# DrorT/demucs

Measured on AMD Instinct MI355X. Metric: real-time factor (audio-sec/wall-sec) htdemucs 4-stem 44.1kHz stereo, 1/8 GPU, higher is better.
Workload: dtype f32

## Files before the change

### demucs_amd/_lib.py

```python
from __future__ import annotations

import ctypes as C
import os
import threading

_HERE = os.path.dirname(os.path.abspath(__file__))
LIB_PATH = os.environ.get("DEMUCS_AMD_LIB") or os.path.join(_HERE, "libdemucs_amd.so")

MI_OK = 0


class MiTensorDesc(C.Structure):
    _fields_ = [("name", C.c_char_p), ("data", C.c_void_p), ("numel", C.c_int64)]


class MiConfig(C.Structure):
    _fields_ = [("n_sources", C.c_int32), ("segment_length", C.c_int32), ("max_batch", C.c_int32),
                ("dtype", C.c_int32)]


class MiProfileRow(C.Structure):
    _fields_ = [("name", C.c_char * 48), ("launches", C.c_int64), ("ms", C.c_double), ("flops", C.c_double),
                ("bytes", C.c_double)]


class MiConvDesc(C.Structure):
    _fields_ = [
        ("wt", C.c_void_p), ("M", C.c_int32), ("Mpad", C.c_int32), ("K", C.c_int32), ("Kpad", C.c_int32),
        ("ktab", C.c_void_p),
        ("x", C.c_void_p), ("x_bstride", C.c_int64),
        ("B", C.c_int32), ("D1", C.c_int32), ("D2", C.c_int32), ("O1", C.c_int32), ("O2", C.c_int32),
        ("S1", C.c_int32), ("S2", C.c_int32),
        ("pro", C.c_int32), ("pro_stats", C.c_void_p), ("pro_w", C.c_void_p), ("pro_b", C.c_void_p),
        ("row_mode", C.c_int32),
        ("epi", C.c_int32), ("flags", C.c_int32),
        ("bias", C.c_void_p), ("scale", C.c_void_p), ("res", C.c_void_p), ("emb", C.c_void_p),
        ("y", C.c_void_p), ("y_bstride", C.c_int64), ("y_cstride", C.c_int64),
        ("stats", C.c_void_p), ("gn_stats", C.c_void_p), ("gn_w", C.c_void_p), ("gn_b", C.c_void_p),
        ("out_len", C.c_int32), ("tile_m", C.c_int32), ("plain", C.c_int32), ("half", C.c_int32),
        ("o2_valid", C.c_int32), ("ktab_len", C.c_int32), ("sink", C.c_void_p), ("wx", C.c_void_p), ("tr_stride", C.c_int32), ("tr_pad", C.c_int32), ("x_ld", C.c_int32), ("x_ld_pad", C.c_int32), ("wh", C.c_void_p),
        ("xh", C.c_void_p), ("xh_n", C.c_int64), ("yh", C.c_void_p), ("yh_n", C.c_int64),
        ("wtap", C.c_void_p), ("ntaps", C.c_int32), ("tap_k2", C.c_int32), ("tap_pad1", C.c_int32), ("tap_pad2", C.c_int32),
        ("tap_dil1", C.c_int32), ("tap_dil2", C.c_int32), ("yh_pq", C.c_int64),
        ("dma_rows", C.c_int32), ("dma_rows_pad", C.c_int32),
        ("dma_time", C.c_int32), ("dma_time_pad", C.c_int32),
    ]


SIGNATURES = {
    "mi_model_create": (C.c_int, [C.POINTER(MiConfig), C.POINTER(MiTensorDesc), C.c_size_t, C.POINTER(C.c_void_p)]),
    "mi_model_destroy": (None, [C.c_void_p]),
    "mi_model_forward": (C.c_int, [C.c_void_p, C.c_void_p, C.c_void_p, C.c_int32, C.c_void_p]),
    "mi_model_forward_core": (C.c_int, [C.c_void_p, C.c_void_p, C.c_void_p, C.c_void_p, C.c_void_p, C.c_int32, C.c_void_p]),
    "mi_model_tap": (C.c_int, [C.c_void_p, C.c_char_p, C.c_void_p, C.c_int32, C.POINTER(C.c_int64), C.c_void_p]),
    "mi_hmodel_create": (C.c_int, [C.POINTER(MiConfig), C.POINTER(MiTensorDesc), C.c_size_t, C.POINTER(C.c_void_p)]),
    "mi_hmodel_destroy": (None, [C.c_void_p]),
    "mi_hmodel_forward": (C.c_int, [C.c_void_p, C.c_void_p, C.c_void_p, C.c_int32, C.c_int32, C.c_void_p]),
    "mi_hmodel_tap": (C.c_int, [C.c_void_p, C.c_char_p, C.c_void_p, C.c_int32, C.POINTER(C.c_int64), C.c_void_p]),
    "mi_hmodel_device_bytes": (C.c_int64, [C.c_void_p]),
    "mi_hmodel_status": (C.c_int, [C.c_void_p, C.c_void_p]),
    "mi_set_two_streams": (C.c_int, [C.c_int32]),
    "mi_set_split_bf16": (C.c_int, [C.c_int32]),
    "mi_set_istft_fused": (C.c_int, [C.c_int32]),
    "mi_set_transpose_tiles": (C.c_int, [C.c_int32]),
    "mi_profile_begin": (C.c_int, [C.c_void_p]),
    "mi_profile_end": (C.c_int, [C.c_void_p, C.POINTER(MiProfileRow), C.c_int32, C.POINTER(C.c_int32), C.c_void_p]),
    "mi_model_device_bytes": (C.c_int64, [C.c_void_p]),
    "mi_segments_gather": (C.c_int, [C.c_void_p, C.c_int64, C.c_int32, C.c_void_p, C.c_int32, C.c_int32, C.c_void_p,
                                     C.c_int64, C.c_void_p]),
    "mi_ola_accumulate": (C.c_int, [C.c_void_p, C.c_int64, C.c_int32, C.c_void_p, C.c_int32, C.c_int64, C.c_void_p, C.c_void_p,
                                    C.c_void_p, C.c_int32, C.c_int64, C.c_int64, C.c_void_p, C.c_int32, C.c_void_p]),
    "mi_ola_finish": (C.c_int, [C.c_void_p, C.c_int64, C.c_int32, C.c_int64, C.c_void_p, C.c_void_p, C.c_int32,
                                C.c_int32, C.c_void_p, C.c_void_p]),
    "mi_segments_gather_packed": (C.c_int, [C.c_void_p, C.c_int64, C.c_int32, C.c_void_p, C.c_int32, C.c_int32, C.c_void_p,
                                            C.c_int64, C.c_void_p]),
    "mi_ola_accumulate_packed": (C.c_int, [C.c_void_p, C.c_int64, C.c_int32, C.c_void_p, C.c_int32, C.c_int64, C.c_void_p, C.c_int32,
                                           C.c_void_p, C.c_int32, C.c_void_p, C.c_int64, C.c_void_p]),
    "mi_ola_finish_packed": (C.c_int, [C.c_void_p, C.c_int64, C.c_int32, C.c_void_p, C.c_int32, C.c_void_p, C.c_int32, C.c_void_p,
                                       C.c_int64, C.c_void_p]),
    "mi_stream_emit": (C.c_int, [C.c_void_p, C.c_int64, C.c_int32, C.c_int32, C.c_void_p, C.c_int32, C.c_void_p, C.c_int32,
                                 C.c_void_p, C.c_int64, C.c_void_p, C.c_int32, C.c_int32, C.c_int32, C.c_void_p, C.c_int64,
                                 C.c_void_p, C.c_int64, C.c_void_p]),
    "mi_streams_emit": (C.c_int, [C.c_void_p, C.c_int64, C.c_int32, C.c_int32, C.c_void_p, C.c_int32, C.c_int64, C.c_void_p,
                                  C.c_int32, C.c_void_p, C.c_int32, C.c_void_p, C.c_int64, C.c_void_p, C.c_int32, C.c_int32,
                                  C.c_int32, C.c_void_p, C.c_int32, C.c_void_p, C.c_int64, C.c_void_p]),
    "mi_streams_append": (C.c_int, [C.c_void_p, C.c_int64, C.c_int32, C.c_void_p, C.c_int32, C.c_int64, C.c_void_p, C.c_int32,
                                    C.c_void_p]),
    "mi_streams_convert_append": (C.c_int, [C.c_void_p, C.c_int64, C.c_int32, C.c_void_p, C.c_int32, C.c_int64, C.c_void_p, C.c_int64,
                                            C.c_void_p, C.c_int64, C.c_void_p, C.c_int32, C.c_int32, C.c_void_p]),
    "mi_pcm_planar": (C.c_int, [C.c_void_p, C.c_int32, C.c_int32, C.c_int64, C.c_int32, C.c_void_p, C.c_void_p, C.c_void_p]),
    "mi_streams_append_pcm": (C.c_int, [C.c_void_p, C.c_int64, C.c_int32, C.c_void_p, C.c_int32, C.c_int64, C.c_void_p, C.c_int32,
                                        C.c_void_p]),
    "mi_streams_convert_append_pcm": (C.c_int, [C.c_void_p, C.c_int64, C.c_int32, C.c_void_p, C.c_int32, C.c_int64, C.c_void_p,
                                                C.c_int64, C.c_void_p, C.c_int64, C.c_void_p, C.c_int32, C.c_int32, C.c_void_p]),
    "mi_streams_compact": (C.c_int, [C.c_void_p, C.c_int64, C.c_void_p, C.c_int64, C.c_void_p, C.c_int32, C.c_int64, C.c_void_p]),
    "mi_mono_stats_scratch_bytes": (C.c_int32, []),
    "mi_mono_stats": (C.c_int, [C.c_void_p, C.c_int32, C.c_int64, C.c_void_p, C.c_void_p, C.c_void_p]),
    "mi_mono_stats_state_bytes": (C.c_int32, []),
    "mi_mono_stats_update": (C.c_int, [C.c_void_p, C.c_int32, C.c_int32, C.c_int64, C.c_int32, C.c_int64, C.c_void_p, C.c_void_p]),
    "mi_mono_stats_finish": (C.c_int, [C.c_void_p, C.c_int64, C.c_void_p, C.c_void_p, C.c_void_p]),
    "mi_sdr_state_bytes": (C.c_int64, [C.c_int32]),
    "mi_sdr_scratch_bytes": (C.c_int64, [C.c_int32]),
    "mi_sdr_update": (C.c_int, [C.c_void_p, C.c_int32, C.c_int32, C.c_int64, C.c_void_p, C.c_int64, C.c_int32, C.c_int32, C.c_int64,
                                C.c_int64, C.c_void_p, C.c_void_p]),
    "mi_sdr_finish": (C.c_int, [C.c_void_p, C.c_int32, C.c_void_p, C.c_void_p, C.c_void_p]),
    "mi_sdr": (C.c_int, [C.c_void_p, C.c_void_p, C.c_int32, C.c_int32, C.c_int32, C.c_int64, C.c_void_p, C.c_void_p, C.c_void_p,
                         C.c_void_p]),
    "mi_track_affine": (C.c_int, [C.c_void_p, C.c_int64, C.c_void_p, C.c_int32, C.c_void_p]),
    "mi_prevent_clip": (C.c_int, [C.c_void_p, C.c_int64, C.c_int32, C.c_void_p, C.c_void_p, C.c_void_p]),
    "mi_two_stems": (C.c_int, [C.c_void_p, C.c_int32, C.c_int32, C.c_void_p, C.c_int32, C.c_int64, C.c_void_p, C.c_void_p]),
    "mi_deliver_peaks": (C.c_int, [C.c_void_p, C.c_int32, C.c_int64, C.c_int32, C.c_int32, C.c_void_p, C.c_int32, C.c_int64, C.c_void_p]),
    "mi_deliver_pcm": (C.c_int, [C.c_void_p, C.c_int32, C.c_int64, C.c_int32, C.c_int32, C.c_void_p, C.c_int32, C.c_void_p, C.c_int64,
                                 C.c_void_p]),
    "mi_deliver_resample_pcm": (C.c_int, [C.c_void_p, C.c_int32, C.c_int64, C.c_int32, C.c_int32, C.c_void_p, C.c_int64, C.c_void_p,
                                          C.c_int64, C.c_int32, C.c_void_p, C.c_int64, C.c_void_p]),
    "mi_deliver_peaks_update": (C.c_int, [C.c_void_p, C.c_int32, C.c_int64, C.c_int32, C.c_int32, C.c_void_p, C.c_int32, C.c_void_p]),
    "mi_deliver_mix_pcm": (C.c_int, [C.c_void_p, C.c_int32, C.c_int64, C.c_int32, C.c_int32, C.c_void_p, C.c_int32, C.c_void_p, C.c_int64,
                                     C.c_void_p]),
    "mi_deliver_mix_peaks": (C.c_int, [C.c_void_p, C.c_int32, C.c_int64, C.c_int32, C.c_int32, C.c_void_p, C.c_int32, C.c_int64,
                                       C.c_void_p]),
    "mi_deliver_mix_peaks_update": (C.c_int, [C.c_void_p, C.c_int32, C.c_int64, C.c_int32, C.c_int32, C.c_void_p, C.c_int32, C.c_void_p]),
    "mi_deliver_mix_auto_pcm": (C.c_int, [C.c_void_p, C.c_int64, C.c_int32, C.c_int64, C.c_int32, C.c_int32, C.c_void_p, C.c_int32,
                                          C.c_void_p, C.c_int64, C.c_void_p]),
    "mi_deliver_mix_auto_peaks": (C.c_int, [C.c_void_p, C.c_int64, C.c_int32, C.c_int64, C.c_int32, C.c_int32, C.c_void_p, C.c_int32,
                                            C.c_int64, C.c_void_p]),
    "mi_loudness_update": (C.c_int, [C.c_void_p, C.c_int32, C.c_int64, C.c_int64, C.c_int32, C.c_int32, C.POINTER(C.c_double), C.c_int64,
                                     C.c_int64, C.c_void_p, C.c_int64, C.c_void_p, C.c_int64, C.c_void_p, C.c_int64, C.c_void_p]),
    "mi_deliver_resample_peaks": (C.c_int, [C.c_void_p, C.c_int32, C.c_int64, C.c_int32, C.c_int32, C.c_void_p, C.c_int64, C.c_void_p,
                                            C.c_int64, C.c_int32, C.c_void_p, C.c_void_p, C.c_int32, C.c_void_p]),
    "mi_deliver_resample_pcm_peaks": (C.c_int, [C.c_void_p, C.c_int32, C.c_int64, C.c_int32, C.c_int32, C.c_void_p, C.c_int64,
                                                C.c_void_p, C.c_int64, C.c_int32, C.c_void_p, C.c_int64, C.c_void_p, C.c_void_p,
                                                C.c_int32, C.c_void_p]),
    "mi_stft_cac": (C.c_int, [C.c_void_p, C.c_int32, C.c_int32, C.c_void_p, C.c_void_p]),
    "mi_istft_cac": (C.c_int, [C.c_void_p, C.c_int32, C.c_int32, C.c_int32, C.c_void_p, C.c_void_p]),
    "mi_stft_norm": (C.c_int, [C.c_void_p, C.c_int32, C.c_int32, C.c_void_p, C.c_int32, C.c_void_p, C.c_void_p, C.c_void_p]),
    "mi_istft_full": (C.c_int, [C.c_void_p, C.c_int32, C.c_int32, C.c_int32, C.c_int32, C.c_void_p, C.c_void_p, C.c_int32, C.c_void_p,
                                C.c_void_p, C.c_void_p]),
    "mi_item_norm": (C.c_int, [C.c_void_p, C.c_int32, C.c_int64, C.c_void_p, C.c_void_p, C.c_void_p, C.c_void_p]),
    "mi_item_denorm": (C.c_int, [C.c_void_p, C.c_int32, C.c_int64, C.c_void_p, C.c_void_p, C.c_void_p]),
    "mi_conv_forward": (C.c_int, [C.POINTER(MiConvDesc), C.c_void_p]),
    "mi_resample_frac": (C.c_int, [C.c_void_p, C.c_int32, C.c_int64, C.c_void_p, C.c_int32, C.c_int32, C.c_int32, C.c_void_p, C.c_int64,
                                   C.c_void_p]),
    "mi_conv_pack_split": (C.c_int, [C.c_void_p, C.c_int32, C.c_int32, C.c_int32, C.c_void_p, C.c_void_p]),
    "mi_conv_pack_half": (C.c_int, [C.c_void_p, C.c_int32, C.c_int32, C.c_int32, C.c_void_p, C.c_void_p]),
    "mi_f32_to_image": (C.c_int, [C.c_void_p, C.c_int32, C.c_int32, C.c_int64, C.c_int32, C.c_void_p, C.c_void_p]),
    "mi_conv_pack_tap": (C.c_int, [C.c_void_p, C.c_int32, C.c_int32, C.c_int32, C.c_int32, C.c_void_p, C.c_void_p]),
    "mi_attention": (C.c_int, [C.c_void_p, C.c_void_p, C.c_void_p, C.c_void_p, C.c_int32, C.c_int32, C.c_int32,
                               C.c_int32, C.c_int64, C.c_int64, C.c_int64, C.c_int32, C.c_void_p]),
    "mi_attention_split": (C.c_int, [C.c_void_p, C.c_void_p, C.c_void_p, C.c_void_p, C.c_int32, C.c_int32, C.c_int32,
                                     C.c_int32, C.c_int64, C.c_int64, C.c_int64, C.c_void_p]),
    "mi_attention_heads": (C.c_int, [C.c_void_p, C.c_void_p, C.c_void_p, C.c_void_p, C.c_int32, C.c_int32, C.c_int32, C.c_int32,
                                     C.c_int32, C.c_int32, C.c_int32, C.c_void_p]),
    "mi_attention_heads_image": (C.c_int, [C.c_void_p, C.c_void_p, C.c_void_p, C.c_void_p, C.c_int64, C.c_int32, C.c_int32, C.c_int32,
                                           C.c_int32, C.c_int32, C.c_int32, C.c_int32, C.c_void_p]),
    "mi_attention_image": (C.c_int, [C.c_void_p, C.c_void_p, C.c_void_p, C.c_void_p, C.c_int64, C.c_int32, C.c_int32, C.c_int32,
                                     C.c_int32, C.c_int64, C.c_int64, C.c_int32, C.c_void_p]),
    "mi_lstm_seq": (C.c_int, [C.c_void_p, C.c_void_p, C.c_int32, C.c_int32, C.c_int32, C.c_void_p, C.c_int32, C.c_void_p]),
    "mi_gn_gelu": (C.c_int, [C.c_void_p, C.c_int32, C.c_int32, C.c_int32, C.c_int32, C.c_int32, C.c_int32, C.c_void_p, C.c_void_p,
                             C.c_void_p, C.c_void_p]),
    "mi_gram_order": (C.c_int32, [C.c_int32]),
    "mi_gn_gelu_gram": (C.c_int, [C.c_void_p, C.c_int32, C.c_int32, C.c_int32, C.c_int32, C.c_int32, C.c_int32, C.c_int32, C.c_void_p,
                                  C.c_void_p, C.c_void_p, C.c_void_p, C.c_int32, C.c_void_p]),
    "mi_dconv_gn_gelu_gram": (C.c_int, [C.c_void_p, C.c_int32, C.c_int32, C.c_int32, C.c_int32, C.c_int32, C.c_int32, C.c_int32,
                                        C.c_void_p, C.c_void_p, C.c_void_p, C.c_void_p, C.c_int32, C.c_void_p]),
    "mi_gram_finalize": (C.c_int, [C.c_void_p, C.c_int32, C.c_int32, C.c_int32, C.c_void_p, C.c_void_p, C.c_double, C.c_double,
                                   C.c_double, C.c_double, C.c_float, C.c_void_p, C.c_void_p]),
    "mi_layernorm_cf": (C.c_int, [C.c_void_p, C.c_int32, C.c_int32, C.c_int32, C.c_void_p, C.c_void_p, C.c_void_p,
                                  C.c_void_p, C.c_void_p]),
    "mi_token_norm": (C.c_int, [C.c_int32, C.c_void_p, C.c_int32, C.c_int32, C.c_int32, C.c_void_p, C.c_void_p, C.c_void_p, C.c_void_p,
                                C.c_void_p, C.c_void_p, C.c_void_p, C.c_int64, C.c_int32, C.c_void_p]),
    "mi_local_attn": (C.c_int, [C.c_void_p, C.c_int32, C.c_int32, C.c_int32, C.c_int32, C.c_void_p, C.c_int32, C.c_void_p]),
    "mi_group_norm_apply": (C.c_int, [C.c_void_p, C.c_int32, C.c_int32, C.c_int32, C.c_int32, C.c_int32, C.c_int32, C.c_void_p,
                                      C.c_void_p, C.c_int32, C.c_int32, C.c_void_p, C.c_void_p, C.c_int32, C.c_void_p, C.c_int32,
                                      C.c_int32, C.c_int32, C.c_int32, C.c_void_p, C.c_void_p, C.c_void_p]),
    "mi_blstm_unfold": (C.c_int, [C.c_void_p, C.c_int32, C.c_int32, C.c_int32, C.c_int32, C.c_int32, C.c_int32, C.c_void_p, C.c_void_p]),
    "mi_blstm_restitch": (C.c_int, [C.c_void_p, C.c_int32, C.c_int32, C.c_int32, C.c_int32, C.c_int32, C.c_int32, C.c_void_p,
                                    C.c_void_p, C.c_void_p]),
    "mi_row_affine_pitch": (C.c_int, [C.c_void_p, C.c_int32, C.c_int32, C.c_int32, C.c_int32, C.c_void_p, C.c_void_p, C.c_void_p]),
    "mi_dconv_row": (C.c_int, [C.c_void_p, C.c_void_p, C.c_int32, C.c_int32, C.c_int32, C.c_int32, C.c_void_p, C.c_int32, C.c_void_p]),
    "mi_dconv_time_layer": (C.c_int, [C.c_void_p, C.c_void_p, C.c_int32, C.c_int32, C.c_int32, C.c_int32, C.c_int32, C.c_void_p,
                                      C.c_void_p, C.c_void_p, C.c_void_p, C.c_void_p, C.c_void_p]),
    "mi_debug_set_post_launch_hook": (None, [C.c_void_p]),
    "mi_debug_last_conv_route": (C.c_int, []),
    "mi_debug_last_conv_tile": (C.c_int, []),
    "mi_debug_conv_staged": (C.c_int, []),
    "mi_debug_conv_route_launches": (C.c_int64, [C.c_int32, C.c_int32]),
    "mi_debug_conv_route": (C.c_int, [C.POINTER(MiConvDesc), C.POINTER(C.c_int)]),
    "mi_debug_switches": (C.c_int, [C.c_char_p, C.c_int32]),
    "mi_last_error": (C.c_char_p, []),
    "mi_version": (C.c_char_p, []),
}

_lib = None
_lock = threading.Lock()


class EngineError(RuntimeError):
    """A libdemucs_amd call returned a non-zero status (the reference convention for this path
# ... 30 lines not shown
```

### demucs_amd/csrc/api.hip

```cpp
#include <new>

#include "hmodel.h"
#include "model.h"

namespace mi {

post_launch_hook_t g_post_launch_hook = nullptr;
int g_last_conv_route = -1;
long long g_conv_route_launches[16][8] = {};
int g_last_conv_tile = -1;

char *last_error_buf() {
    static thread_local char buf[1024] = "";
    return buf;
}

int set_error(int code, const char *fmt, ...) {
    va_list ap;
    va_start(ap, fmt);
    vsnprintf(last_error_buf(), 1024, fmt, ap);
    va_end(ap);
    return code;
}

struct Tables {
    FftTables t{};
    bool ready = false;
};
static int get_tables(FftTables *out) {
    static Tables tb;
    if (!tb.ready) {
        const FftHostTables h = fft_host_tables();
        float *dw, *de; float2 *dt;
        MI_HIP(hipMalloc((void **)&dw, 4096 * 4)); MI_HIP(hipMalloc((void **)&dt, h.twiddle.size() * 8)); MI_HIP(hipMalloc((void **)&de, 1024 * 4));
        MI_HIP(hipMemcpy(dw, h.window.data(), 4096 * 4, hipMemcpyHostToDevice));
        MI_HIP(hipMemcpy(dt, h.twiddle.data(), h.twiddle.size() * 8, hipMemcpyHostToDevice));
        MI_HIP(hipMemcpy(de, h.envelope.data(), 1024 * 4, hipMemcpyHostToDevice));
        tb.t = FftTables{dw, dt, de};
        tb.ready = true;
    }
    *out = tb.t;
    return MI_OK;
}

static size_t dconv_layer_floats(int C) { const size_t h = C / 8; return h * C * 3 + 3 * h + 2 * C * h + 6 * (size_t)C + C; }
struct DConvTestLayer {
    std::vector<void *> bufs;
    DConvTimeLayer l{};
    ~DConvTestLayer() { for (void *p : bufs) (void)hipFree(p); }
    template <typename T> int up(const T *h, size_t n, const T **out) {
        void *p = nullptr;
        MI_HIP(hipMalloc(&p, n * sizeof(T)));
        bufs.push_back(p);
        MI_HIP(hipMemcpy(p, h, n * sizeof(T), hipMemcpyHostToDevice));
        *out = (const T *)p;
        return MI_OK;
    }
    int init(int C, const float *w) {
        const int h = C / 8;
        const float *w0 = w, *b0 = w0 + (size_t)h * C * 3, *g1w = b0 + h, *g1b = g1w + h, *w3 = g1b + h, *b3 = w3 + (size_t)2 * C * h,
                    *g2w = b3 + 2 * C, *g2b = g2w + 2 * C, *ls = g2b + 2 * C;
        const DConvHostPack p = dconv_pack_host(C, h, w0, b0, g1w, g1b, w3, b3);
        MI_TRY(up(p.w0.data(), p.w0.size(), &l.w.w0)); MI_TRY(up(p.b0.data(), p.b0.size(), &l.w.b0));
        MI_TRY(up(p.g1w.data(), p.g1w.size(), &l.w.g1w)); MI_TRY(up(p.g1b.data(), p.g1b.size(), &l.w.g1b));
        MI_TRY(up(p.w3.data(), p.w3.size(), &l.w.w3));
        MI_TRY(up(b3, (size_t)2 * C, &l.w.b3)); MI_TRY(up(g2w, (size_t)2 * C, &l.w.g2w)); MI_TRY(up(g2b, (size_t)2 * C, &l.w.g2b));
        MI_TRY(up(ls, (size_t)C, &l.w.ls));
        MI_TRY(up(p.gram_a.data(), p.gram_a.size(), &l.gram_a)); MI_TRY(up(p.gram_v.data(), p.gram_v.size(), &l.gram_v));
        MI_TRY(up(p.gram_c.data(), p.gram_c.size(), &l.gram_c)); MI_TRY(up(p.gram_e1.data(), p.gram_e1.size(), &l.gram_e1));
        MI_TRY(up(p.gram_e2.data(), p.gram_e2.size(), &l.gram_e2));
        l.sum_b3 = p.sum_b3; l.sum_b3sq = p.sum_b3sq;
        return MI_OK;
    }
};

struct TestScratch {
    std::vector<void *> bufs;
    ~TestScratch() { for (void *p : bufs) (void)hipFree(p); }
    template <typename T> int get(size_t n, T **out) {
        void *p = nullptr;
        MI_HIP(hipMalloc(&p, std::max<size_t>(n, 1) * sizeof(T)));
        bufs.push_back(p);
        *out = (T *)p;
        return MI_OK;
    }
};
static int finish_entry(int r, hipStream_t st, const char *who) {
    const hipError_t e = hipStreamSynchronize(st);
    if (e != hipSuccess && r == MI_OK) r = set_error(MI_EHIP, "%s: hipStreamSynchronize: %s", who, hipGetErrorString(e));
    return r;
}

static int stft_entry(const char *who, const float *mix_dev, int B, int L, float *x_dev, int x_pitch, float *norm_dev, float *denorm_dev,
                      hipStream_t st) {
    FftTables tb;
    MI_TRY(get_tables(&tb));
    const int T = (L + 1023) / 1024;
    TestScratch ws;
    float *zt = nullptr; double *stats = nullptr;
    MI_TRY(ws.get((size_t)B * T * 4 * 2048, &zt));
    MI_TRY(ws.get((size_t)2 * kStatSlots * B, &stats));
    MI_HIP(hipMemsetAsync(stats, 0, sizeof(double) * 2 * kStatSlots * B, st));
    int r = launch_stft_frames(mix_dev, B, L, tb, zt, stats, st);
    if (r == MI_OK && norm_dev) r = launch_finalize_stats(stats, B, 4.0 * 2048 * T, 1e-5f, 1, (float2 *)norm_dev, (float2 *)denorm_dev, st);
    if (r == MI_OK) r = launch_cac_transpose(zt, B, T, (const float2 *)norm_dev, x_dev, st, x_pitch);
    return finish_entry(r, st, who);
}

static const char *const kKindNames[2] = {"htdemucs", "hdemucs"};
template <typename Engine>
static Engine *engine_of(void *handle, EngineKind want, const char *entry) {
    EngineCore *core = static_cast<EngineCore *>(handle);
    if (core->kind != want) {
        set_error(MI_EINVAL, "%s: the handle belongs to the %s engine, this entry takes one of the %s engine", entry, kKindNames[core->kind], kKindNames[want]);
        return nullptr;
    }
    return static_cast<Engine *>(core);
}
constexpr size_t kConvSlack = 128;
int g_conv_staged = 0;
static bool conv_reads_slack(int route) { return route == MI_ROUTE_DMATAP || route == MI_ROUTE_TAP_X6 || route == MI_ROUTE_TIME_X6; }
static bool conv_owns_slack(const float *x, size_t bytes) {
    hipDeviceptr_t base = nullptr;
    size_t size = 0;
    if (hipMemGetAddressRange(&base, &size, (hipDeviceptr_t)x) != hipSuccess) {
        (void)hipGetLastError();
        return false;
    }
    const uintptr_t lo = (uintptr_t)base, hi = lo + size, p = (uintptr_t)x;
    return p >= lo + kConvSlack && p + bytes + kConvSlack <= hi;
}
static int conv_forward_staged(const mi_conv_desc &din, size_t bytes, hipStream_t st) {
    TestScratch ws;
    unsigned char *buf = nullptr;
    MI_TRY(ws.get(bytes + 2 * kConvSlack, &buf));
    MI_HIP(hipMemsetAsync(buf, 0, bytes + 2 * kConvSlack, st));
    MI_HIP(hipMemcpyAsync(buf + kConvSlack, din.x, bytes, hipMemcpyDeviceToDevice, st));
    mi_conv_desc d = din;
    d.x = reinterpret_cast<const float *>(buf + kConvSlack);
    ++g_conv_staged;
    return finish_entry(launch_conv(d, st), st, "mi_conv_forward");
}

static Model *as_model(void *handle, const char *entry) { return engine_of<Model>(handle, ENGINE_HTDEMUCS, entry); }
static HModel *as_hmodel(void *handle, const char *entry) { return engine_of<HModel>(handle, ENGINE_HDEMUCS, entry); }

}

using namespace mi;

extern "C" {

const char *mi_last_error(void) { return last_error_buf(); }
void mi_debug_set_post_launch_hook(void (*hook)(void *stream)) { g_post_launch_hook = hook; }
int mi_debug_last_conv_route(void) { return g_last_conv_route; }
int mi_debug_last_conv_tile(void) { return g_last_conv_tile; }
int mi_debug_conv_staged(void) { return g_conv_staged; }
int64_t mi_debug_conv_route_launches(int32_t route, int32_t epi) {
    if (route < 0 || route >= 16 || epi >= 8) return -1;
    int64_t n = 0;
    for (int e = 0; e < 8; ++e)
        if (epi < 0 || e == epi) n += mi::g_conv_route_launches[route][e];
    return n;
}
int mi_debug_conv_route(const struct mi_conv_desc *desc, int *tile) {
    if (!desc) return -1;
    if (conv_check_tile_m(*desc) != MI_OK) return -1;
    const ConvRoute r = conv_route(*desc);
    if (tile) *tile = r.tile;
    return r.route;
}
const char *mi_version(void) { return "demucs_amd 0.1 gfx950"; }

int mi_model_create(const mi_config *cfg, const mi_tensor_desc *weights, size_t n_weights, void **handle) {
    if (!cfg || !weights || !handle) return set_error(MI_EINVAL, "mi_model_create: null argument");
    *handle = nullptr;
    Model *m = new (std::nothrow) Model();
    if (!m) return set_error(MI_ENOMEM, "mi_model_create: host allocation failed");
    const int r = m->init(*cfg, weights, n_weights);
    if (r != MI_OK) { delete m; return r; }
    *handle = static_cast<EngineCore *>(m);
    return MI_OK;
}

void mi_model_destroy(void *handle) {
    if (!handle) return;
    Model *m = as_model(handle, "mi_model_destroy");
    if (!m) return;
    (void)hipDeviceSynchronize();
    delete m;
}

int mi_model_forward(void *handle, const float *mix_dev, float *out_dev, int32_t B, void *stream) {
    if (!handle) return set_error(MI_EINVAL, "mi_model_forward: null handle");
    Model *m = as_model(handle, "mi_model_forward");
    return m ? m->forward(mix_dev, out_dev, B, (hipStream_t)stream) : MI_EINVAL;
}

int mi_model_tap(void *handle, const char *name, float *dst_dev, int32_t B, int64_t *numel_per_item, void *stream) {
    if (!handle || !name || !numel_per_item) return set_error(MI_EINVAL, "mi_model_tap: null argument");
    Model *m = as_model(handle, "mi_model_tap");
    if (!m) return MI_EINVAL;
    const float *src = nullptr;
    const float **ptr_dev = &src;
    const std::string n(name);
    const int64_t T = m->T, Tf = 8 * T, Tt = m->Lt[4];
    static const int ch[4] = {48, 96, 192, 384}, fr[4] = {512, 128, 32, 8};
    *ptr_dev = nullptr;
    if (n == "x0") { *ptr_dev = m->w_x0; *numel_per_item = 4 * 2048 * T; }
    else if (n == "xt0") { *ptr_dev = m->w_xt0; *numel_per_item = 2 * (int64_t)m->SL; }
    else if (n == "yspec") { *ptr_dev = m->w_yspec; *numel_per_item = 4 * (int64_t)m->S * 2048 * T; }
    else if (n == "ytime") { *ptr_dev = m->w_ytime; *numel_per_item = 2 * (int64_t)m->S * m->SL; }
    else if (n == "tr_f") { *ptr_dev = m->w_tr_x[0][1]; *numel_per_item = 512 * Tf; }
    else if (n == "tr_t") { *ptr_dev = m->w_tr_x[1][1]; *numel_per_item = 512 * Tt; }
    else if (n.size() == 4 && n.compare(0, 3, "enc") == 0 && n[3] >= '0' && n[3] <= '3') {
        const int i = n[3] - '0'; *ptr_dev = m->w_skip[i]; *numel_per_item = (int64_t)ch[i] * fr[i] * T;
    } else if (n.size() == 5 && n.compare(0, 4, "tenc") == 0 && n[4] >= '0' && n[4] <= '3') {
        const int i = n[4] - '0'; *ptr_dev = m->w_skip_t[i]; *numel_per_item = (int64_t)ch[i] * m->Lp[i + 1];
    }
    if (!*ptr_dev) return set_error(MI_EINVAL, "mi_model_tap: unknown tap '%s'", name);
    if (dst_dev) {
        MI_REQUIRE(B >= 1 && B <= m->cfg.max_batch, "mi_model_tap: batch %d out of range", B);
        MI_HIP(hipMemcpyAsync(dst_dev, src, sizeof(float) * (size_t)B * *numel_per_item, hipMemcpyDeviceToDevice, (hipStream_t)stream));
    }
    return MI_OK;
}

int mi_model_forward_core(void *handle, const float *mix_dev, const float *mag_dev, float *spec_out_dev, float *time_out_dev,
                          int32_t B, void *stream) {
    if (!handle) return set_error(MI_EINVAL, "mi_model_forward_core: null handle");
    Model *m = as_model(handle, "mi_model_forward_core");
    return m ? m->forward_core(mix_dev, mag_dev, spec_out_dev, time_out_dev, B, (hipStream_t)stream) : MI_EINVAL;
}

int mi_hmodel_create(const mi_config *cfg, const mi_tensor_desc *weights, size_t n_weights, void **handle) {
    if (!cfg || !weights || !handle) return set_error(MI_EINVAL, "mi_hmodel_create: null argument");
    *handle = nullptr;
    HModel *m = new (std::nothrow) HModel();
    if (!m) return set_error(MI_ENOMEM, "mi_hmodel_create: host allocation failed");
    const int r = m->hinit(*cfg, weights, n_weights);
    if (r != MI_OK) { delete m; return r; }
    *handle = static_cast<EngineCore *>(m);
    return MI_OK;
}

void mi_hmodel_destroy(void *handle) {
    if (!handle) return;
    HModel *m = as_hmodel(handle, "mi_hmodel_destroy");
    if (!m) return;
    (void)hipDeviceSynchronize();
    delete m;
}

int mi_hmodel_forward(void *handle, const float *mix_dev, float *out_dev, int32_t B, int32_t length, void *stream) {
    if (!handle) return set_error(MI_EINVAL, "mi_hmodel_forward: null handle");
    HModel *m = as_hmodel(handle, "mi_hmodel_forward");
    return m ? m->hforward(mix_dev, out_dev, B, length, (hipStream_t)stream) : MI_EINVAL;
}

int mi_hmodel_tap(void *handle, const char *name, float *dst_dev, int32_t B, int64_t *numel_per_item, void *stream) {
    if (!handle || !name || !numel_per_item) return set_error(MI_EINVAL, "mi_hmodel_tap: null argument");
    HModel *m = as_hmodel(handle, "mi_hmodel_tap");
    if (!m) return MI_EINVAL;
    auto it = m->taps.find(name);
    if (it == m->taps.end()) return set_error(MI_EINVAL, "mi_hmodel_tap: unknown tap '%s'", name);
    *numel_per_item = it->second.second;
    if (dst_dev) {
        MI_REQUIRE(B >= 1 && B <= m->cfg.max_batch, "mi_hmodel_tap: batch %d out of range", B);
        MI_HIP(hipMemcpyAsync(dst_dev, it->second.first, sizeof(float) * (size_t)B * it->second.second, hipMemcpyDeviceToDevice, (hipStream_t)stream));
    }
    return MI_OK;
}

int mi_hmodel_status(void *handle, void *stream) {
// ... 355 lines not shown
int mi_deliver_resample_pcm_peaks(const int64_t *table_dev, int32_t n_rows, int64_t max_groups, int32_t n_sources, int32_t channels,
                                  const float *bank_dev, int64_t bank_capacity, float *hist_dev, int64_t hist_capacity, int32_t lds_floats,
                                  void *dst_dev, int64_t dst_capacity, const int32_t *slots_dev, const void *peaks_dev, int32_t n_peaks,
                                  void *stream) {
    MI_REQUIRE(table_dev && dst_dev && n_rows > 0 && n_rows <= 65535 && max_groups >= 1 && max_groups <= INT32_MAX && n_sources > 0 &&
               channels > 0 && bank_capacity >= 0 && (bank_capacity == 0 || bank_dev) && hist_capacity >= 0 &&
               (hist_capacity == 0 || hist_dev) && lds_floats >= 1 && lds_floats <= MI_RATE_LDS_FLOATS && dst_capacity >= 0 &&
               slots_dev && n_peaks >= 0 && (n_peaks == 0 || peaks_dev), "mi_deliver_resample_pcm_peaks: bad argument");
    MI_REQUIRE(((uintptr_t)dst_dev & 3) == 0, "mi_deliver_resample_pcm_peaks: dst_dev must be 4-byte aligned");
    return launch_deliver_resample_pcm_peaks(table_dev, n_rows, max_groups, n_sources, channels, bank_dev, bank_capacity, hist_dev,
                                             hist_capacity, lds_floats, (unsigned char *)dst_dev, dst_capacity, slots_dev,
                                             (const unsigned *)peaks_dev, n_peaks, (hipStream_t)stream);
}

int mi_deliver_mix_pcm(const int64_t *table_dev, int32_t n_rows, int64_t max_n, int32_t n_sources, int32_t channels,
                       const void *peaks_dev, int32_t n_peaks, void *dst_dev, int64_t dst_capacity, void *stream) {
    MI_REQUIRE(table_dev && dst_dev && n_rows > 0 && n_rows <= 65535 && max_n >= 1 && max_n <= (int64_t)INT32_MAX * 1024 &&
               n_sources > 0 && n_sources <= MI_MIX_MAX_SOURCES && channels > 0 && n_peaks >= 0 && (n_peaks == 0 || peaks_dev) &&
               dst_capacity >= 0, "mi_deliver_mix_pcm: bad argument");
    MI_REQUIRE(((uintptr_t)dst_dev & 3) == 0, "mi_deliver_mix_pcm: dst_dev must be 4-byte aligned");
    return launch_deliver_mix_pcm(table_dev, n_rows, max_n, n_sources, channels, (const unsigned *)peaks_dev, n_peaks,
                                  (unsigned char *)dst_dev, dst_capacity, (hipStream_t)stream);
}

int mi_deliver_mix_peaks(const int64_t *table_dev, int32_t n_rows, int64_t max_n, int32_t n_sources, int32_t channels, void *peaks_dev,
                         int32_t n_peaks, int64_t dst_capacity, void *stream) {
    MI_REQUIRE(table_dev && peaks_dev && n_rows > 0 && n_rows <= 65535 && max_n >= 1 && max_n <= (int64_t)INT32_MAX * 1024 &&
               n_sources > 0 && n_sources <= MI_MIX_MAX_SOURCES && channels > 0 && n_peaks > 0 && dst_capacity >= 0,
               "mi_deliver_mix_peaks: bad argument");
    return launch_deliver_mix_peaks(table_dev, n_rows, max_n, n_sources, channels, (unsigned *)peaks_dev, n_peaks, dst_capacity,
                                    (hipStream_t)stream);
}

int mi_deliver_mix_peaks_update(const int64_t *table_dev, int32_t n_rows, int64_t max_n, int32_t n_sources, int32_t channels,
                                void *peaks_dev, int32_t n_peaks, void *stream) {
    MI_REQUIRE(table_dev && peaks_dev && n_rows > 0 && n_rows <= 65535 && max_n >= 1 && max_n <= (int64_t)INT32_MAX * 1024 &&
               n_sources > 0 && n_sources <= MI_MIX_MAX_SOURCES && channels > 0 && n_peaks > 0, "mi_deliver_mix_peaks_update: bad argument");
    return launch_deliver_mix_peaks_update(table_dev, n_rows, max_n, n_sources, channels, (unsigned *)peaks_dev, n_peaks,
                                           (hipStream_t)stream);
}

int mi_deliver_mix_auto_pcm(const int64_t *table_dev, int64_t table_len, int32_t n_rows, int64_t max_n, int32_t n_sources,
                            int32_t channels, const void *peaks_dev, int32_t n_peaks, void *dst_dev, int64_t dst_capacity, void *stream) {
    MI_REQUIRE(table_dev && dst_dev && n_rows > 0 && n_rows <= 65535 && table_len <= INT32_MAX &&
               table_len >= (int64_t)n_rows * MI_AUTO_COLS && max_n >= 1 && max_n <= (int64_t)INT32_MAX * 1024 && n_sources > 0 &&
               n_sources <= MI_MIX_MAX_SOURCES && channels > 0 && n_peaks >= 0 && (n_peaks == 0 || peaks_dev) && dst_capacity >= 0,
               "mi_deliver_mix_auto_pcm: bad argument");
    MI_REQUIRE(((uintptr_t)dst_dev & 3) == 0, "mi_deliver_mix_auto_pcm: dst_dev must be 4-byte aligned");
    return launch_deliver_mix_auto_pcm(table_dev, table_len, n_rows, max_n, n_sources, channels, (const unsigned *)peaks_dev, n_peaks,
                                       (unsigned char *)dst_dev, dst_capacity, (hipStream_t)stream);
}

int mi_deliver_mix_auto_peaks(const int64_t *table_dev, int64_t table_len, int32_t n_rows, int64_t max_n, int32_t n_sources,
                              int32_t channels, void *peaks_dev, int32_t n_peaks, int64_t dst_capacity, void *stream) {
    MI_REQUIRE(table_dev && peaks_dev && n_rows > 0 && n_rows <= 65535 && table_len <= INT32_MAX &&
               table_len >= (int64_t)n_rows * MI_AUTO_COLS && max_n >= 1 && max_n <= (int64_t)INT32_MAX * 1024 && n_sources > 0 &&
               n_sources <= MI_MIX_MAX_SOURCES && channels > 0 && n_peaks > 0 && dst_capacity >= 0,
               "mi_deliver_mix_auto_peaks: bad argument");
    return launch_deliver_mix_auto_peaks(table_dev, table_len, n_rows, max_n, n_sources, channels, (unsigned *)peaks_dev, n_peaks,
                                         dst_capacity, (hipStream_t)stream);
}

int mi_loudness_update(const int64_t *table_dev, int32_t n_rows, int64_t max_n, int64_t max_blocks, int32_t n_sources, int32_t channels,
                       const double *coef, int64_t hop, int64_t warm, float *hist_dev, int64_t hist_capacity, double *energies_dev,
                       int64_t energies_capacity, float *work_dev, int64_t work_capacity, void *stream) {
    MI_REQUIRE(table_dev && coef && energies_dev && work_dev && n_rows > 0 && n_rows <= 65535 && max_n >= 1 &&
               max_n <= (int64_t)INT32_MAX * 256 && max_blocks >= 0 && max_blocks <= (int64_t)INT32_MAX * 64 && n_sources > 0 &&
               n_sources <= MI_MIX_MAX_SOURCES && channels > 0 && channels <= 65535 && hist_capacity >= 0 &&
               (hist_dev || hist_capacity == 0) && energies_capacity >= 0 && work_capacity >= 0,
               "mi_loudness_update: bad argument");
    if (hop < 1 || warm < 0) return MI_OK;
    return launch_loudness_update(table_dev, n_rows, max_n, max_blocks, n_sources, channels, coef, hop, warm, hist_dev, hist_capacity,
                                  energies_dev, energies_capacity, work_dev, work_capacity, (hipStream_t)stream);
}

int mi_stft_cac(const float *mix_dev, int32_t B, int32_t L, float *cac_dev, void *stream) {
    MI_REQUIRE(mix_dev && cac_dev && B > 0 && B <= 16383 && L >= 1, "mi_stft_cac: bad argument");
    return stft_entry("mi_stft_cac", mix_dev, B, L, cac_dev, 0, nullptr, nullptr, (hipStream_t)stream);
}

int mi_stft_norm(const float *mix_dev, int32_t B, int32_t L, float *x_dev, int32_t x_pitch, float *norm_dev, float *denorm_dev, void *stream) {
    MI_REQUIRE(mix_dev && x_dev && norm_dev && denorm_dev, "mi_stft_norm: null argument");
    MI_REQUIRE(B >= 1 && B <= 16383, "mi_stft_norm: B = %d outside [1, 16383] (the transpose's grid holds 4 B planes)", B);
    MI_REQUIRE(L >= 1, "mi_stft_norm: L = %d, at least one sample", L);
    const int T = (L + 1023) / 1024;
    MI_REQUIRE(x_pitch == 0 || x_pitch >= T, "mi_stft_norm: row pitch %d below T = %d", x_pitch, T);
    return stft_entry("mi_stft_norm", mix_dev, B, L, x_dev, x_pitch, norm_dev, denorm_dev, (hipStream_t)stream);
}

int mi_istft_full(const float *y_dev, int32_t B, int32_t S, int32_t L, int32_t y_pitch, const float *denorm_f_dev, const float *xt_dev,
                  int32_t xt_pitch, const float *denorm_t_dev, float *wav_dev, void *stream) {
    MI_REQUIRE(y_dev && wav_dev, "mi_istft_full: null argument");
    MI_REQUIRE(B >= 1 && S >= 1 && (int64_t)B * S <= 16383, "mi_istft_full: B = %d, S = %d: 1 <= B S <= 16383 (the transpose's grid holds 4 B S planes)",
               B, S);
    MI_REQUIRE(L >= 1, "mi_istft_full: L = %d, at least one sample", L);
    const int T = (L + 1023) / 1024;
    MI_REQUIRE(y_pitch == 0 || y_pitch >= T, "mi_istft_full: spectrogram row pitch %d below T = %d", y_pitch, T);
    MI_REQUIRE((xt_dev != nullptr) == (denorm_t_dev != nullptr), "mi_istft_full: xt_dev and denorm_t_dev go together");
    MI_REQUIRE(xt_pitch == 0 || xt_pitch >= L, "mi_istft_full: time-branch row pitch %d below L = %d", xt_pitch, L);
    FftTables tb;
    MI_TRY(get_tables(&tb));
    TestScratch ws;
    float *yt = nullptr, *fr = nullptr;
    MI_TRY(ws.get((size_t)B * S * T * 4 * 2048, &yt));
    MI_TRY(ws.get((size_t)B * S * T * 2 * 4096, &fr));
    hipStream_t st = (hipStream_t)stream;
    const int r = launch_istft(y_dev, B, S, L, (const float2 *)denorm_f_dev, xt_dev, (const float2 *)denorm_t_dev, tb, yt, fr, wav_dev, st,
                               xt_pitch, y_pitch);
    return finish_entry(r, st, "mi_istft_full");
}

int mi_istft_cac(const float *x_dev, int32_t B, int32_t S, int32_t L, float *wav_dev, void *stream) {
    MI_REQUIRE(x_dev && wav_dev && B > 0 && S > 0 && (int64_t)B * S <= 16383 && L >= 1, "mi_istft_cac: bad argument");
    return mi_istft_full(x_dev, B, S, L, 0, nullptr, nullptr, 0, nullptr, wav_dev, stream);
}

int mi_item_norm(const float *x_dev, int32_t rows, int64_t count, float *y_dev, float *norm_dev, float *denorm_dev, void *stream) {
    MI_REQUIRE(x_dev && y_dev && norm_dev && denorm_dev, "mi_item_norm: null argument");
    MI_REQUIRE(rows >= 1 && rows <= 65535, "mi_item_norm: rows = %d outside [1, 65535] (the grid's y range)", rows);
    MI_REQUIRE(count >= 2, "mi_item_norm: count = %lld: the unbiased std divides by count - 1", (long long)count);
    TestScratch ws;
    double *stats = nullptr;
    MI_TRY(ws.get((size_t)2 * kStatSlots * rows, &stats));
    hipStream_t st = (hipStream_t)stream;
    MI_HIP(hipMemsetAsync(stats, 0, sizeof(double) * 2 * kStatSlots * rows, st));
    int r = launch_row_stats(x_dev, rows, count, count, stats, st);
    if (r == MI_OK) r = launch_finalize_stats(stats, rows, (double)count, 1e-5f, 1, (float2 *)norm_dev, (float2 *)denorm_dev, st);
    if (r == MI_OK) r = launch_row_affine(x_dev, rows, count, (const float2 *)norm_dev, y_dev, st);
    return finish_entry(r, st, "mi_item_norm");
}

int mi_item_denorm(const float *x_dev, int32_t rows, int64_t count, const float *denorm_dev, float *y_dev, void *stream) {
    MI_REQUIRE(x_dev && denorm_dev && y_dev, "mi_item_denorm: null argument");
    MI_REQUIRE(rows >= 1 && rows <= 65535 && count >= 1, "mi_item_denorm: rows = %d outside [1, 65535] or count = %lld < 1", rows, (long long)count);
    return launch_row_denorm(x_dev, rows, count, (const float2 *)denorm_dev, y_dev, (hipStream_t)stream);
}

int mi_conv_forward(const struct mi_conv_desc *desc, void *stream) {
    MI_REQUIRE(desc, "mi_conv_forward: null descriptor");
    if (desc->x && desc->B > 0 && desc->x_bstride > 0 && conv_check_tile_m(*desc) == MI_OK && conv_reads_slack(conv_route(*desc).route)) {
        const size_t bytes = (size_t)desc->B * (size_t)desc->x_bstride * sizeof(float);
        if (!conv_owns_slack(desc->x, bytes)) return conv_forward_staged(*desc, bytes, (hipStream_t)stream);
    }
    return launch_conv(*desc, (hipStream_t)stream);
}

int mi_resample_frac(const float *x_dev, int32_t rows, int64_t length, const float *table_dev, int32_t old_sr, int32_t new_sr,
                     int32_t width, float *y_dev, int64_t out_length, void *stream) {
    MI_REQUIRE(x_dev && table_dev && y_dev && old_sr > 0 && new_sr > 0 && width > 0, "mi_resample_frac: bad argument");
    return launch_resample_frac(x_dev, rows, length, table_dev, old_sr, new_sr, width, y_dev, out_length, (hipStream_t)stream);
}

int mi_conv_pack_split(const float *wt_dev, int32_t Kpad, int32_t Mpad, int32_t tile_m, void *wx_dev, void *stream) {
    MI_REQUIRE(wt_dev && wx_dev && Kpad > 0 && Mpad > 0 && (conv_x6_supported(tile_m) || tile_m == 192), "mi_conv_pack_split: bad argument");
    MI_REQUIRE(tile_m != 192 || Mpad % 192 == 0, "mi_conv_pack_split: tile_m 192 needs Mpad %% 192 == 0 (Mpad %d)", Mpad);
    return launch_pack_split(wt_dev, Kpad, Mpad, tile_m == 192 ? 96 : tile_m, wx_dev, (hipStream_t)stream);
}

int mi_conv_pack_tap(const float *wt_dev, int32_t Mpad, int32_t Cin, int32_t ntaps, int32_t dtype, void *wtap_dev, void *stream) {
    MI_REQUIRE(wt_dev && wtap_dev && Mpad > 0 && Cin > 0 && ntaps > 0, "mi_conv_pack_tap: bad argument");
    return launch_pack_tap(wt_dev, Mpad, Cin, ntaps, dtype, wtap_dev, (hipStream_t)stream);
}

int mi_f32_to_image(const float *x_dev, int32_t B, int32_t C, int64_t P, int32_t dtype, void *img_dev, void *stream) {
    MI_REQUIRE(x_dev && img_dev && B > 0 && C > 0 && P > 0, "mi_f32_to_image: bad argument");
    return launch_f32_to_image(x_dev, B, C, P, dtype, img_dev, (hipStream_t)stream);
}

int mi_conv_pack_half(const float *wt_dev, int32_t Kpad, int32_t Mpad, int32_t dtype, void *wh_dev, void *stream) {
    MI_REQUIRE(wt_dev && wh_dev && Kpad > 0 && Mpad > 0, "mi_conv_pack_half: bad argument");
    return launch_pack_half(wt_dev, Kpad, Mpad, dtype, wh_dev, (hipStream_t)stream);
}

int mi_attention(const float *q_dev, const float *k_dev, const float *v_dev, float *o_dev, int32_t B, int32_t heads, int32_t Tq,
                 int32_t Tk, int64_t q_batch_stride, int64_t kv_batch_stride, int64_t o_batch_stride, int32_t dtype, void *stream) {
    MI_REQUIRE(q_dev && k_dev && v_dev && o_dev && B > 0 && heads > 0 && Tq > 0 && Tk > 0, "mi_attention: bad argument");
    return launch_attention(q_dev, k_dev, v_dev, o_dev, B, heads, Tq, Tk, q_batch_stride, kv_batch_stride, o_batch_stride, dtype,
                            (hipStream_t)stream);
}

int mi_attention_split(const float *q_dev, const float *k_dev, const float *v_dev, float *o_dev, int32_t B, int32_t heads, int32_t Tq,
                       int32_t Tk, int64_t q_batch_stride, int64_t kv_batch_stride, int64_t o_batch_stride, void *stream) {
    MI_REQUIRE(q_dev && k_dev && v_dev && o_dev && B > 0 && heads > 0 && Tq > 0 && Tk > 0, "mi_attention_split: bad argument");
    return launch_attention_x6(q_dev, k_dev, v_dev, o_dev, B, heads, Tq, Tk, q_batch_stride, kv_batch_stride, o_batch_stride,
                               (hipStream_t)stream);
}

int mi_attention_heads(const void *q_dev, const void *k_dev, const void *v_dev, float *o_dev, int32_t B, int32_t heads, int32_t Tq, int32_t Tk,
                       int32_t Tq_pitch, int32_t Tk_pitch, int32_t dtype, void *stream) {
    MI_REQUIRE(q_dev && k_dev && v_dev && o_dev && B > 0 && heads > 0 && Tq > 0 && Tk > 0, "mi_attention_heads: bad argument");
    const void *zero = conv_zero_page();
    MI_REQUIRE(zero, "mi_attention_heads: could not allocate the zero page");
    return launch_attention_heads(q_dev, k_dev, v_dev, zero, B, heads, Tq, Tk, Tq_pitch, Tk_pitch, dtype, nullptr, 0, o_dev,
                                  (int64_t)heads * 64 * Tq, (hipStream_t)stream);
}

int mi_attention_heads_image(const void *q_dev, const void *k_dev, const void *v_dev, void *img_dev, int64_t n_img, int32_t B, int32_t heads,
                             int32_t Tq, int32_t Tk, int32_t Tq_pitch, int32_t Tk_pitch, int32_t dtype, void *stream) {
    MI_REQUIRE(q_dev && k_dev && v_dev && img_dev && B > 0 && heads > 0 && Tq > 0 && Tk > 0, "mi_attention_heads_image: bad argument");
    const void *zero = conv_zero_page();
    MI_REQUIRE(zero, "mi_attention_heads_image: could not allocate the zero page");
    return launch_attention_heads(q_dev, k_dev, v_dev, zero, B, heads, Tq, Tk, Tq_pitch, Tk_pitch, dtype, img_dev, n_img, nullptr, 0,
                                  (hipStream_t)stream);
}

int mi_attention_image(const float *q_dev, const float *k_dev, const float *v_dev, void *img_dev, int64_t n_img, int32_t B,
                       int32_t heads, int32_t Tq, int32_t Tk, int64_t q_batch_stride, int64_t kv_batch_stride, int32_t dtype,
                       void *stream) {
    MI_REQUIRE(q_dev && k_dev && v_dev && img_dev && B > 0 && heads > 0 && Tq > 0 && Tk > 0, "mi_attention_image: bad argument");
    MI_REQUIRE(dtype == MI_DTYPE_BF16 || dtype == MI_DTYPE_F16, "mi_attention_image: dtype %d is not a half mode", dtype);
    return launch_attention(q_dev, k_dev, v_dev, nullptr, B, heads, Tq, Tk, q_batch_stride, kv_batch_stride, 0, dtype,
                            (hipStream_t)stream, img_dev, n_img);
}

int mi_gn_gelu(float *x_dev, int32_t B, int32_t C, int32_t C_alloc, int32_t D1, int32_t D2, int32_t row_mode, const float *stats_dev,
               const float *w_dev, const float *b_dev, void *stream) {
    MI_REQUIRE(x_dev && stats_dev && w_dev && b_dev && B > 0 && C > 0 && D1 > 0 && D2 > 0, "mi_gn_gelu: bad argument");
    MI_REQUIRE(C_alloc >= C, "mi_gn_gelu: C_alloc < C");
    return launch_gn_gelu(x_dev, B, C, C_alloc, D1, D2, row_mode, (const float2 *)stats_dev, w_dev, b_dev, (hipStream_t)stream);
}

int32_t mi_gram_order(int32_t h) { return gram_hp(h); }

int mi_lstm_seq(const float *gx_dev, const float *whh_host, int32_t N, int32_t H, int32_t W, float *out_dev, int32_t mode, void *stream) {
    MI_REQUIRE(mode == 0 || mode == 1 || mode == 2, "mi_lstm_seq: mode 0 (one launch per step), 1 (persistent kernel) or 2 (generic small kernel)");
    hipStream_t st = (hipStream_t)stream;
    if (mode == 2) {
        MI_REQUIRE(gx_dev && whh_host && out_dev && N > 0 && N <= 65535 && W > 0 && H >= 1 && H <= 64,
                   "mi_lstm_seq: bad argument (mode 2 needs 1 <= H <= 64)");
        const size_t bytes = (size_t)2 * 4 * H * H * sizeof(float);
        float *wn = nullptr;
        MI_HIP(hipMalloc((void **)&wn, bytes));
        int rs = MI_OK;
        if (hipMemcpyAsync(wn, whh_host, bytes, hipMemcpyHostToDevice, st) != hipSuccess) rs = set_error(MI_EHIP, "mi_lstm_seq: hipMemcpyAsync failed");
        if (rs == MI_OK) rs = launch_lstm_small(gx_dev, wn, N, H, W, out_dev, st);
        const hipError_t es = hipStreamSynchronize(st);
        if (es != hipSuccess && rs == MI_OK) rs = set_error(MI_EHIP, "mi_lstm_seq: hipStreamSynchronize: %s", hipGetErrorString(es));
        (void)hipFree(wn);
        return rs;
    }
    MI_REQUIRE(gx_dev && whh_host && out_dev && N > 0 && W > 0 && (H == 192 || H == 384), "mi_lstm_seq: bad argument (H must be 192 or 384)");
    std::vector<float> packed((size_t)2 * 4 * H * H);
    pack_lstm_whh(whh_host, H, packed.data());
    float *wd = nullptr, *state = nullptr;
    void *scratch = nullptr;
    unsigned *flag = nullptr;
    int r = MI_OK;
    auto fail = [&](hipError_t e, const char *what) { if (e != hipSuccess && r == MI_OK) r = set_error(MI_EHIP, "mi_lstm_seq: %s: %s", what, hipGetErrorString(e)); };
    fail(hipMalloc((void **)&wd, packed.size() * sizeof(float)), "hipMalloc");
    fail(hipMalloc((void **)&state, (size_t)6 * N * H * sizeof(float)), "hipMalloc");
    fail(hipMalloc(&scratch, lstm_persist_scratch_bytes()), "hipMalloc");
    fail(hipHostMalloc((void **)&flag, 64, hipHostMallocMapped), "hipHostMalloc");
    if (r == MI_OK) {
        *flag = 0;
        fail(hipMemcpyAsync(wd, packed.data(), packed.size() * sizeof(float), hipMemcpyHostToDevice, st), "hipMemcpyAsync");
        if (r == MI_OK) r = mode ? launch_lstm_persist(gx_dev, wd, N, H, W, out_dev, scratch, flag, st) : launch_lstm_seq(gx_dev, wd, N, H, W, out_dev, state, st);
        fail(hipStreamSynchronize(st), "hipStreamSynchronize");
        if (r == MI_OK && *(volatile unsigned *)flag) r = set_error(MI_EHIP, "mi_lstm_seq: the persistent kernel timed out waiting for its hidden-state exchange");
        if (r == MI_OK && mode && switches().lstm_debug) {
                        unsigned dbg[16] = {};
            (void)hipMemcpy(dbg, (char *)scratch + lstm_persist_ctl_offset(), sizeof(dbg), hipMemcpyDeviceToHost);
            fprintf(stderr, "[lstm] H %d N %d W %d: block 0 / wave 1 spent %.1f us gathering h in %u poll passes (%.2f us, %.2f passes per step); "
                    "%s stores\n", H, N, W, dbg[2] * 0.01, dbg[3], dbg[2] * 0.01 / std::max(1, W - 1), (double)dbg[3] / std::max(1, W - 1),
                    dbg[4] ? "same-XCD plain" : "write-through");
            fprintf(stderr, "[lstm]   shader cycles per step: gather %.0f, issue + products %.0f, LDS write + barrier %.0f, gate stage %.0f; whole step %.0f\n",
                    (double)dbg[8] / W, (double)dbg[9] / W, (double)dbg[10] / W, (double)dbg[11] / W, (double)dbg[12] / W);
        }
    }
    if (wd) (void)hipFree(wd);
    if (state) (void)hipFree(state);
    if (scratch) (void)hipFree(scratch);
    if (flag) (void)hipHostFree(flag);
    return r;
}

int mi_gn_gelu_gram(float *x_dev, int32_t B, int32_t h, int32_t C_alloc, int32_t D1, int32_t D2, int32_t pitch, int32_t row_mode,
                    const float *stats_dev, const float *w_dev, const float *b_dev, double *gram_dev, int32_t slots, void *stream) {
    MI_REQUIRE(x_dev && stats_dev && w_dev && b_dev && gram_dev && B > 0 && h > 0 && D1 > 0 && D2 > 0 && slots > 0, "mi_gn_gelu_gram: bad argument");
    MI_REQUIRE(C_alloc >= h && pitch >= D2, "mi_gn_gelu_gram: C_alloc < h or pitch < D2");
    return launch_gn_gelu_gram(x_dev, B, h, C_alloc, D1, D2, pitch, row_mode, (const float2 *)stats_dev, w_dev, b_dev, gram_dev, slots,
                               false, (hipStream_t)stream);
}

int mi_dconv_gn_gelu_gram(float *x_dev, int32_t B, int32_t h, int32_t C_alloc, int32_t D1, int32_t D2, int32_t pitch, int32_t row_mode,
                          const float *stats_dev, const float *w_dev, const float *b_dev, double *gram_dev, int32_t slots, void *stream) {
    MI_REQUIRE(x_dev && stats_dev && w_dev && b_dev && gram_dev && B > 0 && h > 0 && D1 > 0 && D2 > 0 && slots > 0, "mi_dconv_gn_gelu_gram: bad argument");
    MI_REQUIRE(C_alloc >= h && C_alloc <= gram_hp(h) && pitch >= D2, "mi_dconv_gn_gelu_gram: C_alloc outside [h, mi_gram_order(h)] or pitch < D2");
    return launch_gn_gelu_gram(x_dev, B, h, C_alloc, D1, D2, pitch, row_mode, (const float2 *)stats_dev, w_dev, b_dev, gram_dev, slots,
                               true, (hipStream_t)stream);
}

int mi_gram_finalize(double *gram_dev, int32_t rows, int32_t h, int32_t slots, const double *wt_dev, const double *ct_dev, double sum_b,
                     double sum_bsq, double cols, double count, float eps, float *stats_out_dev, void *stream) {
    MI_REQUIRE(gram_dev && wt_dev && ct_dev && stats_out_dev && rows > 0 && h > 0 && slots > 0 && count > 0.0, "mi_gram_finalize: bad argument");
    return launch_gram_finalize(gram_dev, rows, h, slots, wt_dev, ct_dev, sum_b, sum_bsq, cols, count, eps, (float2 *)stats_out_dev,
                                (hipStream_t)stream);
}

int mi_layernorm_cf(const float *x_dev, int32_t B, int32_t C, int32_t T, const float *w_dev, const float *b_dev,
                    const float *add_dev, float *y_dev, void *stream) {
    MI_REQUIRE(x_dev && w_dev && b_dev && y_dev, "mi_layernorm_cf: null argument");
    return launch_layernorm_cf(x_dev, B, C, T, w_dev, b_dev, add_dev, y_dev, nullptr, (hipStream_t)stream);
}

int mi_token_norm(int32_t mode, const float *x_dev, int32_t B, int32_t C, int32_t T, const float *w_dev, const float *b_dev,
                  const float *pe_dev, const float *gstat_dev, float *y_dev, float *ostat_dev, void *img_dev, int64_t img_n,
                  int32_t img_dtype, void *stream) {
// ... 104 lines not shown
```

### demucs_amd/csrc/conv_route.hip

```cpp
#include "common.h"
#include "kernels.h"

namespace mi {

int g_split_bf16 = 1;

int conv_pick_tile(int M) {
    if (M <= 32) return 32;
    if (M <= 64) return 64;
    if (M % 128 == 0) return 128;
    if (M % 96 == 0) return 96;
    if (M <= 96) return 96;
    return 128;
}

static bool under_filled(const mi_conv_desc &d, int tile = 128) {
    return (int64_t)(d.Mpad / tile) * ceil_div((int64_t)d.B * d.O1 * d.O2, BN) < 200;
}

static bool dmatap_eligible(const mi_conv_desc &d, int tile, bool has_image, bool split = false) {
    const bool off = switches().no_dma_tap;
    const int ld = d.x_ld ? d.x_ld : d.D2;
    if (switches().no_dma_dconv && d.epi == MI_EPI_BIAS_STATS) return false;
    const int dil = d.tap_dil2 ? d.tap_dil2 : 1;
    const bool kind = (d.epi == MI_EPI_GLU && (tile == 96 || tile == 128) && (d.ntaps == 9 || d.ntaps == 3) && dil == 1) ||
                      (d.epi == MI_EPI_BIAS_STATS && (tile == 32 || tile == 64) && d.ntaps == 3 && (dil == 1 || dil == 2) && d.flags == 0);
    return !off && !d.half && (split ? has_image && d.epi == MI_EPI_GLU : !has_image) && kind && d.tap_k2 == 3 && d.Mpad % tile == 0 &&
           d.K % d.ntaps == 0 && d.S1 == 1 && d.S2 == 1 && d.O1 == d.D1 && d.O2 == ld && ld % 4 == 0 && d.tap_pad2 == dil &&
           d.tap_pad1 == (d.ntaps / 3 - 1) / 2 && !(d.flags & (MI_FLAG_IMG | MI_FLAG_IMG4)) && d.x_bstride == (int64_t)(d.K / d.ntaps) * d.D1 * ld;
}
static bool dmarow_eligible(const mi_conv_desc &d, int tile, bool plain, bool has_image, bool split = false) {
    const bool off = switches().no_dma_rows;
    const int ld = d.x_ld ? d.x_ld : d.D2;
    const int lf = d.flags & (MI_FLAG_GELU | MI_FLAG_SCALE | MI_FLAG_RES | MI_FLAG_LN | MI_FLAG_STATS | MI_FLAG_IMG | MI_FLAG_IMG4 | MI_FLAG_HEADS);
    const bool epi_ok = (d.epi == MI_EPI_LINEAR && lf == MI_FLAG_GELU && !plain) || d.epi == MI_EPI_CONVTR ||
                        ((d.epi == MI_EPI_GLU || d.epi == MI_EPI_GN_GLU) && plain && tile == 128 && !(d.flags & (MI_FLAG_IMG | MI_FLAG_IMG4)));
    if (split && (d.epi == MI_EPI_GN_GLU || tile == 64)) return false;
    return !off && !d.half && (split ? has_image : !has_image) && d.ktab && epi_ok && (plain || d.dma_rows) && (tile == 64 || tile == 96 || tile == 128) &&
           d.Mpad % tile == 0 && d.S2 == 1 && d.O2 == ld && ld % 4 == 0 && ((uintptr_t)d.x & 3) == 0 && ((uintptr_t)d.ktab & 63) == 0 &&
           (d.epi == MI_EPI_CONVTR || tile != 64 || d.epi == MI_EPI_LINEAR);
}

static bool dmatime_eligible(const mi_conv_desc &d, int tile, bool plain, bool has_image) {
    const int ld = d.x_ld ? d.x_ld : d.D2, o2v = d.o2_valid ? d.o2_valid : d.O2;
    const int lf = d.flags & (MI_FLAG_GELU | MI_FLAG_SCALE | MI_FLAG_RES | MI_FLAG_LN | MI_FLAG_STATS | MI_FLAG_IMG | MI_FLAG_IMG4 | MI_FLAG_HEADS);
    const bool tr = d.epi == MI_EPI_CONVTR && !(d.flags & (MI_FLAG_TR_FREQ | MI_FLAG_IMG)) && d.K % 2 == 0 && d.S2 == 1 && d.O2 % 4 == 0 &&
                    d.o2_valid == d.D2 + 1 && d.o2_valid <= d.O2 && d.x_bstride == (int64_t)(d.K / 2) * ld;
    const bool enc = d.epi == MI_EPI_LINEAR && lf == MI_FLAG_GELU && d.K % 8 == 0 && d.S2 == 4 && 4 * (int64_t)o2v <= (int64_t)d.D2 + 3 &&
                     d.x_bstride == (int64_t)(d.K / 8) * ld;
    return d.dma_time && !d.half && has_image && !plain && (tr || enc) && (tile == 96 || tile == 128) && d.Mpad % tile == 0 && d.D1 == 1 &&
           d.O1 == 1 && d.S1 == 1 && ld >= d.D2 && ((uintptr_t)d.x & 3) == 0;
}

int conv_check_tile_m(const mi_conv_desc &d) {
    MI_REQUIRE(d.tile_m != 192 || (d.M > 0 && d.M % 192 == 0 && d.Mpad == d.M), "conv: tile_m 192 needs M %% 192 == 0 and no M padding (M %d, Mpad %d)", d.M, d.Mpad);
    return MI_OK;
}

static bool conv_plain(const mi_conv_desc &d) {
    const int64_t P = (int64_t)d.O1 * d.O2;
    return d.plain && (d.xh || (d.K == d.Kpad && P % 4 == 0 && d.x_bstride % 4 == 0 && ((uintptr_t)d.x & 15) == 0)) &&
           d.S1 == 1 && d.S2 == 1 && d.D1 == d.O1 && (d.x_ld ? d.x_ld : d.D2) == d.O2;
}

static bool half_img256_only(int f) { return f == (MI_FLAG_LN | MI_FLAG_HEADS) || f == (MI_FLAG_LN | MI_FLAG_GELU | MI_FLAG_IMG); }
static int half_linear_flags(const mi_conv_desc &d) {
    return d.flags & (MI_FLAG_GELU | MI_FLAG_SCALE | MI_FLAG_RES | MI_FLAG_LN | MI_FLAG_IMG | MI_FLAG_HEADS | MI_FLAG_STATS);
}

int conv_validate(const mi_conv_desc &d) {
    MI_TRY(conv_check_tile_m(d));
    MI_REQUIRE((int64_t)d.Mpad * d.y_cstride < (1ll << 31), "conv: output channel stride too large for 32-bit row offsets");
    MI_REQUIRE(d.Kpad % BK == 0 && d.Kpad >= BK, "conv: Kpad %d must be a positive multiple of %d", d.Kpad, BK);
    MI_REQUIRE(d.Mpad % 4 == 0, "conv: Mpad %d must be a multiple of 4", d.Mpad);
    MI_REQUIRE(d.O2 >= 32 || d.row_mode == 0 || (d.epi != MI_EPI_BIAS_STATS && d.epi != MI_EPI_STATS_ONLY),
               "conv: statistics epilogue with rows (b, o1) (row_mode 1) needs O2 >= 32");
    MI_REQUIRE(d.pro == 0, "conv: the fused GroupNorm+GELU prologue was replaced by launch_gn_gelu");
    MI_REQUIRE(!(d.flags & MI_FLAG_IMG4) || (d.epi == MI_EPI_GLU && d.half && d.yh && d.yh_pq > 0 && d.yh_n >= (int64_t)d.B * d.yh_pq && d.M % 32 == 0 &&
                                             ((uintptr_t)d.yh & 15) == 0),
               "conv: MI_FLAG_IMG4 needs a half-mode GLU layer with M %% 32 == 0 and an aligned phase image of >= B * yh_pq positions per plane");
    MI_REQUIRE(!(d.flags & MI_FLAG_STATS) || (d.epi == MI_EPI_LINEAR && d.stats && d.O2 >= 32 && d.row_mode == 0),
               "conv: MI_FLAG_STATS needs a LINEAR layer, a statistics buffer and O2 >= 32");
    MI_REQUIRE(!(d.flags & MI_FLAG_LN) || (d.pro_stats && d.scale && d.epi == MI_EPI_LINEAR), "conv: MI_FLAG_LN needs pro_stats and scale");
    const int64_t P = (int64_t)d.O1 * d.O2;
    MI_REQUIRE(!(d.flags & MI_FLAG_IMG) || d.epi == MI_EPI_CONVTR ||
               (d.half && d.yh && d.epi == MI_EPI_LINEAR && d.M % 8 == 0 && d.yh_n >= (int64_t)d.B * P && ((uintptr_t)d.yh & 15) == 0) ||
               (d.half && d.yh && d.epi == MI_EPI_GLU && d.M % 32 == 0 && !(d.flags & (MI_FLAG_IMG4 | MI_FLAG_EMB)) && d.yh_n >= (int64_t)d.B * P &&
                ((uintptr_t)d.yh & 15) == 0),
               "conv: MI_FLAG_IMG needs a half-precision LINEAR layer with M %% 8 == 0 (or GLU layer with M %% 32 == 0) and an aligned "
               "output image of >= B * P columns");
    MI_REQUIRE(d.epi != MI_EPI_CONVTR || ((int64_t)d.Mpad * d.y_cstride < (1ll << 30) && (d.tr_stride == 0 || d.tr_stride == 2 || d.tr_stride == 4) &&
                                          d.M % (d.tr_stride == 2 ? 2 : 4) == 0),
               "conv: transposed conv needs stride 2 or 4, M a multiple of it and 30-bit output offsets per item");
    {
        const int f = d.flags & (MI_FLAG_GELU | MI_FLAG_RES | MI_FLAG_IMG);
        MI_REQUIRE(d.epi != MI_EPI_CONVTR || f == 0 || (d.tr_stride != 2 && (f == (MI_FLAG_GELU | MI_FLAG_RES) || f == (MI_FLAG_GELU | MI_FLAG_RES | MI_FLAG_IMG))),
                   "conv: transposed conv epilogue supports no flags, GELU|RES or GELU|RES|IMG (stride 2: no flags), got %d", d.flags);
    }
    MI_REQUIRE(!(d.flags & MI_FLAG_IMG) || d.epi != MI_EPI_CONVTR ||
               (d.half && d.yh && d.yh_n >= (int64_t)d.B * d.y_cstride && ((uintptr_t)d.yh & 15) == 0),
               "conv: MI_FLAG_IMG on a transposed conv needs a half mode and an output image of >= B * y_cstride positions");
    MI_REQUIRE(!d.wtap || (d.half && d.xh), "conv: tap-ordered weights need a half mode and an operand-image input");
    MI_REQUIRE(d.wtap || !(d.flags & MI_FLAG_HEADS) || (d.half && d.yh && d.epi == MI_EPI_LINEAR && d.M % 512 == 0 && d.O1 == 1 && d.yh_n >= d.O2 &&
                                                        ((uintptr_t)d.yh & 15) == 0 && !(d.flags & MI_FLAG_IMG)),
               "conv: MI_FLAG_HEADS needs a half-precision LINEAR layer on tokens (O1 = 1) with M %% 512 == 0 and an aligned output");
    MI_REQUIRE(!d.xh || d.half, "conv: an operand-image input needs a half-precision layer");
    if (d.xh && !d.wtap) {
        const int f = half_linear_flags(d);
        MI_REQUIRE(d.epi == MI_EPI_LINEAR && conv_plain(d), "conv: an operand-image input needs a plain LINEAR layer");
        MI_REQUIRE(f == (MI_FLAG_SCALE | MI_FLAG_RES) || f == (MI_FLAG_SCALE | MI_FLAG_RES | MI_FLAG_STATS) || half_img256_only(f),
                   "conv: an operand-image input is not instantiated for LINEAR flags %d", d.flags);
    }
    return MI_OK;
}

bool conv_stats_per_item(const mi_conv_desc &d) {
    return (d.epi == MI_EPI_BIAS_STATS || d.epi == MI_EPI_STATS_ONLY) && d.row_mode == 0 && d.B > 2 && (int64_t)d.O1 * d.O2 < 32;
}

ConvRoute conv_route(const mi_conv_desc &d) {
    const bool image = d.wx && g_split_bf16;
    const Switches &sw = switches();
    const int tile = d.tile_m && d.tile_m != 192 ? d.tile_m : conv_pick_tile(d.M);
    const bool plain = conv_plain(d);
    if (d.wtap) return {MI_ROUTE_TAP_HALF, tile, plain};
    if (d.half && d.xh) {
        const int f = half_linear_flags(d);
        const bool wide = d.Mpad % 256 == 0;
        if (half_img256_only(f) || (f == (MI_FLAG_SCALE | MI_FLAG_RES) && sw.img256 && wide)) return {MI_ROUTE_HALF_IMG256, 256, plain};
        return {MI_ROUTE_HALF_IMG, wide ? 256 : 128, plain};
    }
    if (d.half) return {MI_ROUTE_HALF, sw.half_tile256 && plain && tile == 128 && d.epi == MI_EPI_LINEAR && d.Mpad % 256 == 0 ? 256 : tile, plain};
    const bool t192 = d.tile_m == 192 && image;
    const bool small = sw.small_tile && tile == 128 && !t192 && under_filled(d), small_linear = small && plain && d.epi == MI_EPI_LINEAR;
    const int lf = d.flags & (MI_FLAG_GELU | MI_FLAG_SCALE | MI_FLAG_RES | MI_FLAG_LN | MI_FLAG_STATS);
    auto split_tile = [&](int ntaps) {
        if (!t192) return small ? 64 : tile;
        const bool filled = !(sw.small_tile && under_filled(d, 192));
        return filled && conv_x6_tile192(d.epi, d.epi == MI_EPI_LINEAR ? lf : 0, plain, ntaps) ? 192 : 96;
    };
    if (!plain && !sw.x6_plain_only && dmatap_eligible(d, tile, image, true)) return {MI_ROUTE_TAP_X6, split_tile(d.ntaps), plain};
    if (!sw.x6_plain_only && dmarow_eligible(d, tile, plain, image, true)) return {MI_ROUTE_ROWS_X6, split_tile(kRowTaps), plain};
    if (!sw.x6_plain_only && dmatime_eligible(d, tile, plain, image))
        return {MI_ROUTE_TIME_X6, split_tile(d.epi == MI_EPI_CONVTR ? kTimeTr : kTimeEnc), plain};
    const int ktile = small && !plain && d.epi == MI_EPI_GLU && d.Mpad % 96 == 0 ? 96 : tile;
    if (!plain && dmatap_eligible(d, ktile, image)) return {MI_ROUTE_DMATAP, ktile, plain};
    if (dmarow_eligible(d, tile, plain, image)) return {MI_ROUTE_DMAROW, tile, plain};
    if (image && conv_x6_supported(tile) && (!sw.x6_plain_only || plain)) return {MI_ROUTE_X6, t192 ? split_tile(0) : small_linear ? 64 : tile, plain};
    const int ntile = small_linear && d.Mpad % 64 == 0 ? 64 : tile;
    const bool dma = plain && ntile == 128 && d.epi == MI_EPI_LINEAR && !sw.no_dma;
    return {dma ? MI_ROUTE_DMA : MI_ROUTE_TABLE, ntile, plain, sw.mgroups};
}

}
```

### demucs_amd/csrc/engine_core.h

```cpp
#pragma once
#include <algorithm>
#include <cstring>
#include <map>
#include <string>
#include <vector>

#include "common.h"
#include "gemm_conv.h"
#include "kernels.h"

namespace mi {

extern int g_two_streams;

struct DeviceArena {
    int64_t bytes = 0;
    DeviceArena() = default;
    DeviceArena(const DeviceArena &) = delete;
    DeviceArena &operator=(const DeviceArena &) = delete;
    int alloc(void **p, size_t n);
    void release(void *p);
    ~DeviceArena();

   private:
    std::map<void *, size_t> sizes;
};

struct PackedConv {
    float *wt = nullptr, *bias = nullptr;
    void *wx = nullptr;
    void *wh = nullptr;
    void *wtap = nullptr;
    int ntaps = 0;
    int M = 0, Mpad = 0, K = 0, Kpad = 0, tile = 0, half = 0;
};

struct DConvLayerW {
    PackedConv conv3, conv1;
    mi_ktab_entry *ktab3 = nullptr, *ktab1 = nullptr;
    float *gn1_w = nullptr, *gn1_b = nullptr, *gn2_w = nullptr, *gn2_b = nullptr, *ls = nullptr;
    double *gram_wt = nullptr, *gram_ct = nullptr, sum_b = 0.0, sum_bsq = 0.0;
};
struct DConvW {
    DConvLayerW l[2];
    int h = 0;
    bool has_row = false;
    DConvRowLayer row[2];
    bool has_time = false;
    DConvTimeLayer tl[2];
};

struct ProfRow {
    int cls = 0;
    char name[48] = "";
    long long launches = 0;
    double ms = 0.0, flops = 0.0, bytes = 0.0;
};
struct Profiler {
    bool on = false;
    struct Pending { int cls; hipEvent_t a, b; double flops, bytes; long long launches = 1; };
    std::vector<Pending> pending;
    std::vector<hipEvent_t> pool;
    ProfRow rows[128];
    hipEvent_t get();
    template <typename Fn>
    int timed(int cls, const char *name, double flops, double bytes, hipStream_t st, Fn &&fn, long long launches = 1) {
        if (!on) return fn();
        Pending p{cls, get(), get(), flops, bytes, launches};
        MI_HIP(hipEventRecord(p.a, st));
        const int r = fn();
        MI_HIP(hipEventRecord(p.b, st));
        pending.push_back(p);
        if (name) snprintf(rows[cls].name, sizeof(rows[cls].name), "%s", name);
        return r;
    }
    void begin();
    int end(hipStream_t st);
    ~Profiler();
};

enum SplitScope {
    SPLIT_OPT_IN,
    SPLIT_DEFAULT,
    SPLIT_ROWS,
    SPLIT_TIME,
};

struct WeightTable {
    std::map<std::string, std::pair<const float *, int64_t>> t;
    int get(const std::string &name, int64_t numel, const float **out) const {
        auto it = t.find(name);
        if (it == t.end()) return set_error(MI_EWEIGHT, "missing tensor '%s'", name.c_str());
        if (it->second.second != numel)
            return set_error(MI_EWEIGHT, "tensor '%s' has %lld elements, expected %lld", name.c_str(),
                             (long long)it->second.second, (long long)numel);
        *out = it->second.first;
        return MI_OK;
    }
};

static inline int round_up(int v, int m) { return (v + m - 1) / m * m; }

struct Gather {
    int Cin, K1, K2, dil1, dil2, pad1, pad2;
    int64_t chan_stride;
    int D2;
};

static inline std::vector<mi_ktab_entry> build_ktab(const Gather &g, int Kpad) {
    std::vector<mi_ktab_entry> tab(Kpad);
    const int K = g.Cin * g.K1 * g.K2;
    for (int k = 0; k < Kpad; ++k) {
        mi_ktab_entry e;
        if (k < K) {
            const int ci = k / (g.K1 * g.K2), r = k % (g.K1 * g.K2), k1 = r / g.K2, k2 = r % g.K2;
            e.d1 = k1 * g.dil1 - g.pad1;
            e.d2 = k2 * g.dil2 - g.pad2;
            e.off = (int32_t)(ci * g.chan_stride + (int64_t)e.d1 * g.D2 + e.d2);
            e.ci = ci;
        } else {
            e.d1 = -(1 << 29); e.d2 = -(1 << 29); e.off = 0; e.ci = 0;
        }
        tab[k] = e;
    }
    return tab;
}

struct Geo {
    int B, D1, D2;
    int row_mode;
    int ld;
    int pitch() const { return ld ? ld : D2; }
};

static inline mi_conv_desc base_desc(const PackedConv &pc, const mi_ktab_entry *ktab, const float *x, int64_t x_bs, const Geo &g) {
    mi_conv_desc d;
    memset(&d, 0, sizeof(d));
    d.wt = pc.wt; d.M = pc.M; d.Mpad = pc.Mpad; d.K = pc.K; d.Kpad = pc.Kpad; d.ktab = ktab; d.bias = pc.bias; d.tile_m = pc.tile; d.wx = pc.wx;
    d.wh = pc.wh; d.half = pc.wh ? pc.half : 0; d.ktab_len = round_up(pc.Kpad, 32);
    d.x = x; d.x_bstride = x_bs; d.B = g.B; d.D1 = g.D1; d.D2 = g.D2; d.O1 = g.D1; d.O2 = g.pitch(); d.S1 = 1; d.S2 = 1;
    d.o2_valid = g.pitch() != g.D2 ? g.D2 : 0;
    d.x_ld = g.pitch() != g.D2 ? g.pitch() : 0;
    d.row_mode = g.row_mode;
    return d;
}

enum EngineKind { ENGINE_HTDEMUCS, ENGINE_HDEMUCS };

struct EngineCore {
    const EngineKind kind;
    mi_config cfg{};
    Profiler prof;
    int conv(const mi_conv_desc &d, hipStream_t st);
    DeviceArena weights;
    FftTables fft{};

    hipStream_t side_st = nullptr;
    hipEvent_t ev_main = nullptr, ev_side = nullptr;
    int side_streams();

   protected:
    explicit EngineCore(EngineKind k) : kind(k) {}
    ~EngineCore();
    template <typename T> int upload(const std::vector<T> &h, T **dptr) {
        void *p = nullptr;
        MI_TRY(weights.alloc(&p, std::max<size_t>(h.size(), 1) * sizeof(T)));
        MI_HIP(hipMemcpy(p, h.data(), h.size() * sizeof(T), hipMemcpyHostToDevice));
        *dptr = (T *)p;
        return MI_OK;
    }
    int upload_fft_tables();
    int pack_split(PackedConv *pc, SplitScope scope);
    int pack_half(PackedConv *pc);
    int pack_conv(const float *W, const float *bias, int M, int K, bool glu, PackedConv *pc, int ntaps = 0, SplitScope scope = SPLIT_OPT_IN);
    int pack_tap(PackedConv *pc, int ntaps);
    int pack_enc_tap(const float *W, int Cin, PackedConv *pc);
    int pack_convtr(const float *W, const float *bias, int Cin, int Cout, PackedConv *pc, int stride = 4, SplitScope scope = SPLIT_OPT_IN);
    int pack_vec(const float *v, int n, int npad, bool glu, float **out);
    int pack_linear_ln(const float *W, const float *bias, const float *ln_w, const float *ln_b, int M, int K, PackedConv *pc,
                       float **c1, SplitScope scope);
    int make_ktab(const Gather &g, int Kpad, mi_ktab_entry **out);
    int load_dconv(const WeightTable &wt, const std::string &prefix, int C, int64_t chan_stride, int D2, bool freq, DConvW *dw, int comp = 8);
    double *dconv_gram = nullptr;
    double *dconv_gram2 = nullptr;
    size_t dconv_gram2_bytes = 0;
    bool dconv_tap_dma = false;
    int run_dconv(const DConvW &w, int C, const Geo &g, float *x, float *tmp, float *hidden, double *stats, float2 *st1, float2 *st2,
                  hipStream_t st, double *gram2 = nullptr, size_t gram2_cap = 0);
};

}
```

### demucs_amd/csrc/engine_core.hip

```cpp
#include <cmath>
#include <string>
#include <vector>

#include "engine_core.h"

namespace mi {

int DeviceArena::alloc(void **p, size_t n) {
    n = (n + 255) & ~(size_t)255;
    hipError_t e = hipMalloc(p, n);
    if (e != hipSuccess) return set_error(MI_ENOMEM, "hipMalloc(%zu) failed: %s", n, hipGetErrorString(e));
    sizes[*p] = n;
    bytes += (int64_t)n;
    return MI_OK;
}
void DeviceArena::release(void *p) {
    auto it = sizes.find(p);
    if (it == sizes.end()) return;
    (void)hipFree(p);
    bytes -= (int64_t)it->second;
    sizes.erase(it);
}
DeviceArena::~DeviceArena() {
    for (auto &a : sizes) (void)hipFree(a.first);
}

int EngineCore::upload_fft_tables() {
    const FftHostTables h = fft_host_tables();
    float *dw, *de; float2 *dt;
    MI_TRY(upload(h.window, &dw)); MI_TRY(upload(h.twiddle, &dt)); MI_TRY(upload(h.envelope, &de));
    fft = FftTables{dw, dt, de};
    return MI_OK;
}

EngineCore::~EngineCore() {
    if (side_st) (void)hipStreamDestroy(side_st);
    if (ev_main) (void)hipEventDestroy(ev_main);
    if (ev_side) (void)hipEventDestroy(ev_side);
}

int g_two_streams = 1;

int EngineCore::side_streams() {
    if (side_st) return MI_OK;
    const int prio = switches().side_prio;
    if (prio) {
        int least = 0, greatest = 0;
        MI_HIP(hipDeviceGetStreamPriorityRange(&least, &greatest));
        MI_HIP(hipStreamCreateWithPriority(&side_st, hipStreamNonBlocking, prio < 0 ? least : greatest));
    } else
        MI_HIP(hipStreamCreateWithFlags(&side_st, hipStreamNonBlocking));
    MI_HIP(hipEventCreateWithFlags(&ev_main, hipEventDisableTiming));
    MI_HIP(hipEventCreateWithFlags(&ev_side, hipEventDisableTiming));
    return MI_OK;
}

hipEvent_t Profiler::get() {
    if (!pool.empty()) { hipEvent_t e = pool.back(); pool.pop_back(); return e; }
    hipEvent_t e;
    (void)hipEventCreate(&e);
    return e;
}
void Profiler::begin() {
    for (auto &r : rows) r = ProfRow();
    on = true;
}
int Profiler::end(hipStream_t st) {
    on = false;
    MI_HIP(hipStreamSynchronize(st));
    for (auto &p : pending) {
        float ms = 0.f;
        MI_HIP(hipEventElapsedTime(&ms, p.a, p.b));
        ProfRow &r = rows[p.cls];
        r.cls = p.cls; r.launches += p.launches; r.ms += ms; r.flops += p.flops; r.bytes += p.bytes;
        pool.push_back(p.a); pool.push_back(p.b);
    }
    pending.clear();
    return MI_OK;
}
Profiler::~Profiler() {
    for (auto &p : pending) { (void)hipEventDestroy(p.a); (void)hipEventDestroy(p.b); }
    for (auto e : pool) (void)hipEventDestroy(e);
}

static const char *kEpiNames[6] = {"linear", "glu", "bias_stats", "stats_only", "gn_glu", "convtr"};

int EngineCore::conv(const mi_conv_desc &d, hipStream_t st) {
    if (!prof.on) return launch_conv(d, st);
    const int route = conv_route(d).route;
    const int tile = d.tile_m && d.tile_m != 192 ? d.tile_m : conv_pick_tile(d.M), ti = tile == 32 ? 0 : tile == 64 ? 1 : tile == 96 ? 2 : 3;
    const bool tap_x6 = route == MI_ROUTE_TAP_X6, rows_x6 = route == MI_ROUTE_ROWS_X6, time_x6 = route == MI_ROUTE_TIME_X6;
    const int cls = tap_x6    ? 105 + (d.ntaps == 9 ? 2 : 0) + (tile == 128 ? 1 : 0)
                    : rows_x6 ? 109 + (d.epi == MI_EPI_CONVTR ? 4 : d.epi == MI_EPI_GLU ? 2 : 0) + (tile == 128 ? 1 : 0)
                              : (route >= MI_ROUTE_X6 && !time_x6 ? 48 : 0) + d.epi * 8 + ti * 2 + (d.plain ? 1 : 0);
    const double N = (double)d.B * d.O1 * d.O2;
    const double in_bytes = 4.0 * (double)d.B * (double)d.x_bstride;
    double out_rows = d.M;
    if (d.epi == MI_EPI_GLU || d.epi == MI_EPI_GN_GLU) out_rows = d.M / 2;
    if (d.epi == MI_EPI_CONVTR) out_rows = d.M;
    if (d.epi == MI_EPI_STATS_ONLY) out_rows = 0;
    double bytes = in_bytes + 4.0 * out_rows * N + 4.0 * (double)d.M * d.K;
    if (d.flags & MI_FLAG_RES || d.epi == MI_EPI_GN_GLU) bytes += 4.0 * out_rows * N;
    char name[sizeof(ProfRow::name)];
    const bool unnamed = !prof.rows[cls].name[0];
    if (unnamed && tap_x6)
        snprintf(name, sizeof(name), "conv_tap_x6<%s,tile%d,taps%d>", kEpiNames[d.epi], tile, d.ntaps);
    else if (unnamed && rows_x6)
        snprintf(name, sizeof(name), "conv_rows_x6<%s,tile%d>", kEpiNames[d.epi], tile);
    else if (unnamed)
        snprintf(name, sizeof(name), "conv_gemm%s<%s,tile%d%s>", d.half == MI_DTYPE_BF16 ? "_bf16" : d.half == MI_DTYPE_F16 ? "_f16" : cls >= 48 ? "_x6" : "",
                 kEpiNames[d.epi], tile, d.plain ? ",1x1" : "");
    return prof.timed(cls, unnamed ? name : nullptr, 2.0 * d.M * (double)d.K * N, bytes, st, [&] { return launch_conv(d, st); });
}

int EngineCore::pack_split(PackedConv *pc, SplitScope scope) {
    const Switches &sw = switches();
    const bool in_default = scope == SPLIT_DEFAULT || scope == SPLIT_TIME || (scope == SPLIT_ROWS && !sw.no_dma_rows);
    const bool want = sw.x6_scope == 2 || (sw.x6_scope == 1 && in_default && cfg.dtype == MI_DTYPE_F32);
    if (!want || !conv_x6_supported(pc->tile)) return MI_OK;
    const bool t192 = pc->M % 192 == 0 && pc->Mpad == pc->M;
    MI_TRY(weights.alloc(&pc->wx, (size_t)6 * pc->Kpad * pc->Mpad));
    MI_TRY(launch_pack_split(pc->wt, pc->Kpad, pc->Mpad, t192 ? 96 : pc->tile, pc->wx, nullptr));
    MI_HIP(hipStreamSynchronize(nullptr));
    if (t192) pc->tile = 192;
    return MI_OK;
}

int EngineCore::pack_half(PackedConv *pc) {
    if (cfg.dtype == MI_DTYPE_F32) return MI_OK;
    const int Kh = round_up(pc->Kpad, 32);
    MI_TRY(weights.alloc(&pc->wh, (size_t)2 * Kh * pc->Mpad));
    pc->half = cfg.dtype;
    MI_TRY(launch_pack_half(pc->wt, pc->Kpad, pc->Mpad, cfg.dtype, pc->wh, nullptr));
    MI_HIP(hipStreamSynchronize(nullptr));
    return MI_OK;
}

int EngineCore::pack_tap(PackedConv *pc, int ntaps) {
    if (cfg.dtype == MI_DTYPE_F32 || switches().no_tap_image || ntaps < 2 || pc->K % ntaps || (pc->K / ntaps) % 8) return MI_OK;
    const int Cin = pc->K / ntaps;
    MI_TRY(weights.alloc(&pc->wtap, (size_t)16 * conv_tap_pairs_pad(Cin, ntaps) * pc->Mpad));
    pc->ntaps = ntaps;
    MI_TRY(launch_pack_tap(pc->wt, pc->Mpad, Cin, ntaps, cfg.dtype, pc->wtap, nullptr));
    MI_HIP(hipStreamSynchronize(nullptr));
    return MI_OK;
}

int EngineCore::pack_enc_tap(const float *W , int Cin, PackedConv *pc) {
    if (cfg.dtype == MI_DTYPE_F32 || switches().no_enc_image || switches().no_tap_image || Cin % 8) return MI_OK;
    const int M = pc->M, K = 8 * Cin;
    std::vector<float> wt((size_t)K * pc->Mpad, 0.f);
    for (int m = 0; m < M; ++m)
        for (int ci = 0; ci < Cin; ++ci)
            for (int rho = 0; rho < 4; ++rho)
                for (int j = 0; j < 2; ++j) {
                    const int tau = 4 * (j - (rho >= 2)) + rho + 2, ce = ((ci >> 3) * 4 + rho) * 8 + (ci & 7);
                    wt[(size_t)(ce * 2 + j) * pc->Mpad + m] = W[((size_t)m * Cin + ci) * 8 + tau];
                }
    float *tmp = nullptr;
    MI_HIP(hipMalloc((void **)&tmp, wt.size() * sizeof(float)));
    MI_HIP(hipMemcpy(tmp, wt.data(), wt.size() * sizeof(float), hipMemcpyHostToDevice));
    int r = weights.alloc(&pc->wtap, (size_t)16 * conv_tap_pairs_pad(4 * Cin, 2) * pc->Mpad);
    if (r == MI_OK) r = launch_pack_tap(tmp, pc->Mpad, 4 * Cin, 2, cfg.dtype, pc->wtap, nullptr);
    (void)hipStreamSynchronize(nullptr);
    (void)hipFree(tmp);
    if (r == MI_OK) pc->ntaps = 2;
    return r;
}

int EngineCore::pack_conv(const float *W, const float *bias, int M, int K, bool glu, PackedConv *pc, int ntaps, SplitScope scope) {
    const int tile = conv_pick_tile(M);
    pc->M = M; pc->K = K; pc->Mpad = round_up(M, tile); pc->Kpad = round_up(K, 16); pc->tile = tile;
    std::vector<float> wt((size_t)pc->Kpad * pc->Mpad, 0.f), b(pc->Mpad, 0.f);
    for (int m = 0; m < M; ++m) {
        const int src = glu ? ((m & 1) ? (m >> 1) + M / 2 : (m >> 1)) : m;
        for (int k = 0; k < K; ++k) wt[(size_t)k * pc->Mpad + m] = W[(size_t)src * K + k];
        b[m] = bias ? bias[src] : 0.f;
    }
    MI_TRY(upload(wt, &pc->wt));
    MI_TRY(upload(b, &pc->bias));
    MI_TRY(pack_half(pc));
    MI_TRY(pack_tap(pc, ntaps));
    return pack_split(pc, scope);
}

int EngineCore::pack_convtr(const float *W, const float *bias, int Cin, int Cout, PackedConv *pc, int stride, SplitScope scope) {
    const int M = stride * Cout, K = 2 * Cin, ks = 2 * stride;
    const int tile = conv_pick_tile(M);
    pc->M = M; pc->K = K; pc->Mpad = round_up(M, tile); pc->Kpad = round_up(K, 16); pc->tile = tile;
    std::vector<float> wt((size_t)pc->Kpad * pc->Mpad, 0.f), b(pc->Mpad, 0.f);
    for (int ci = 0; ci < Cin; ++ci)
        for (int co = 0; co < Cout; ++co)
            for (int r = 0; r < stride; ++r)
                for (int j = 0; j < 2; ++j)
                    wt[(size_t)(2 * ci + j) * pc->Mpad + stride * co + r] = W[((size_t)ci * Cout + co) * ks + r + stride * j];
    for (int co = 0; co < Cout; ++co)
        for (int r = 0; r < stride; ++r) b[stride * co + r] = bias[co];
    MI_TRY(upload(wt, &pc->wt));
    MI_TRY(upload(b, &pc->bias));
    MI_TRY(pack_half(pc));
    MI_TRY(pack_tap(pc, 2));
    return pack_split(pc, scope);
}

int EngineCore::pack_linear_ln(const float *W, const float *bias, const float *ln_w, const float *ln_b, int M, int K, PackedConv *pc,
                               float **c1, SplitScope scope) {
    std::vector<float> wf((size_t)M * K), c2(M), c1h(M);
    for (int m = 0; m < M; ++m) {
        double s1 = 0.0, s2 = bias ? (double)bias[m] : 0.0;
        for (int k = 0; k < K; ++k) {
            const float wp = W[(size_t)m * K + k] * ln_w[k];
            wf[(size_t)m * K + k] = wp;
            s1 += (double)wp;
            s2 += (double)W[(size_t)m * K + k] * (double)ln_b[k];
        }
        c1h[m] = (float)s1; c2[m] = (float)s2;
    }
    MI_TRY(pack_conv(wf.data(), c2.data(), M, K, false, pc, 0, scope));
    return pack_vec(c1h.data(), M, pc->Mpad, false, c1);
}

int EngineCore::pack_vec(const float *v, int n, int npad, bool glu, float **out) {
    std::vector<float> h(npad, 0.f);
    for (int m = 0; m < n; ++m) h[m] = v[glu ? ((m & 1) ? (m >> 1) + n / 2 : (m >> 1)) : m];
    return upload(h, out);
}

int EngineCore::make_ktab(const Gather &g, int Kpad, mi_ktab_entry **out) {
    return upload(build_ktab(g, round_up(Kpad, 32)), out);
}

int EngineCore::load_dconv(const WeightTable &wt, const std::string &prefix, int C, int64_t chan_stride, int D2, bool freq, DConvW *dw, int comp) {
    const int h = C / comp;
    dw->h = h;
    dw->has_row = comp == 8 && freq && dconv_row_supported(C, D2);
    dw->has_time = comp == 8 && !freq && !switches().no_dconv_time && dconv_time_supported(C, D2);
    for (int d = 0; d < 2; ++d) {
        DConvLayerW &l = dw->l[d];
        const std::string p = prefix + ".dconv.layers." + std::to_string(d);
        const float *w0, *b0, *g1w, *g1b, *w3, *b3, *g2w, *g2b, *ls;
        MI_TRY(wt.get(p + ".0.weight", (int64_t)h * C * 3, &w0));
        MI_TRY(wt.get(p + ".0.bias", h, &b0));
        MI_TRY(wt.get(p + ".1.weight", h, &g1w));
        MI_TRY(wt.get(p + ".1.bias", h, &g1b));
        MI_TRY(wt.get(p + ".3.weight", (int64_t)2 * C * h, &w3));
        MI_TRY(wt.get(p + ".3.bias", 2 * C, &b3));
        MI_TRY(wt.get(p + ".4.weight", 2 * C, &g2w));
        MI_TRY(wt.get(p + ".4.bias", 2 * C, &g2b));
        MI_TRY(wt.get(p + ".6.scale", C, &ls));
        MI_TRY(pack_conv(w0, b0, h, 3 * C, false, &l.conv3));
        const int dil = 1 << d;
        MI_TRY(make_ktab(Gather{C, 1, 3, 1, dil, 0, dil, chan_stride, D2}, l.conv3.Kpad, &l.ktab3));
        const int hp = round_up(h, 16);
        std::vector<float> w3p((size_t)2 * C * hp, 0.f);
        for (int m = 0; m < 2 * C; ++m)
            for (int k = 0; k < h; ++k) w3p[(size_t)m * hp + k] = w3[(size_t)m * h + k];
        MI_TRY(pack_conv(w3p.data(), b3, 2 * C, hp, true, &l.conv1));
        MI_TRY(make_ktab(Gather{hp, 1, 1, 1, 1, 0, 0, chan_stride, D2}, l.conv1.Kpad, &l.ktab1));
        MI_TRY(pack_vec(g1w, h, h, false, &l.gn1_w));
        MI_TRY(pack_vec(g1b, h, h, false, &l.gn1_b));
        MI_TRY(pack_vec(g2w, 2 * C, l.conv1.Mpad, true, &l.gn2_w));
        MI_TRY(pack_vec(g2b, 2 * C, l.conv1.Mpad, true, &l.gn2_b));
        MI_TRY(pack_vec(ls, C, C, false, &l.ls));
        {
            const int HP = gram_hp(h);
            std::vector<double> gw((size_t)HP * HP, 0.0), gc(HP, 0.0);
            double sb = 0.0, sbq = 0.0;
            for (int m = 0; m < 2 * C; ++m) { sb += (double)b3[m]; sbq += (double)b3[m] * (double)b3[m]; }
            for (int i = 0; i < h; ++i) {
                for (int k = 0; k < h; ++k) {
                    if ((k >> 5) < (i >> 5)) continue;
                    double a = 0.0;
                    for (int m = 0; m < 2 * C; ++m) a += (double)w3[(size_t)m * h + i] * (double)w3[(size_t)m * h + k];
                    gw[(size_t)i * HP + k] = (k >> 5) > (i >> 5) ? 2.0 * a : a;
                }
                double v = 0.0, c1 = 0.0;
                for (int m = 0; m < 2 * C; ++m) { v += 2.0 * (double)w3[(size_t)m * h + i] * (double)b3[m]; c1 += (double)w3[(size_t)m * h + i]; }
                gw[(size_t)i * HP + h] = v;
                gc[i] = c1;
            }
            MI_TRY(upload(gw, &l.gram_wt)); MI_TRY(upload(gc, &l.gram_ct));
            l.sum_b = sb; l.sum_bsq = sbq;
        }
        if (dw->has_row || dw->has_time) {
            const DConvHostPack pk = dconv_pack_host(C, h, w0, b0, g1w, g1b, w3, b3);
            float *p0, *p1, *p2, *p3, *p4, *p5, *p6, *p7;
            MI_TRY(upload(pk.w0, &p0)); MI_TRY(upload(pk.b0, &p1)); MI_TRY(upload(pk.g1w, &p2)); MI_TRY(upload(pk.g1b, &p3));
            MI_TRY(upload(pk.w3, &p4));
            MI_TRY(pack_vec(b3, 2 * C, 2 * C, false, &p5)); MI_TRY(pack_vec(g2w, 2 * C, 2 * C, false, &p6));
            MI_TRY(pack_vec(g2b, 2 * C, 2 * C, false, &p7));
            dw->row[d] = DConvRowLayer{p0, p1, p2, p3, p4, p5, p6, p7, l.ls};
            double *da, *dv, *dc, *de1, *de2;
            MI_TRY(upload(pk.gram_a, &da)); MI_TRY(upload(pk.gram_v, &dv)); MI_TRY(upload(pk.gram_c, &dc));
            MI_TRY(upload(pk.gram_e1, &de1)); MI_TRY(upload(pk.gram_e2, &de2));
            dw->tl[d] = DConvTimeLayer{dw->row[d], da, dv, dc, de1, de2, pk.sum_b3, pk.sum_b3sq};
        }
    }
    return MI_OK;
}

int EngineCore::run_dconv(const DConvW &w, int C, const Geo &g, float *x, float *tmp, float *hidden, double *stats, float2 *st1,
                          float2 *st2, hipStream_t st, double *gram2, size_t gram2_cap) {
    if (!gram2) { gram2 = dconv_gram2; gram2_cap = dconv_gram2_bytes; }
    const int h = w.h, hp = round_up(h, 16);
    const int64_t P = (int64_t)g.D1 * g.pitch();
    const int rows = g.row_mode ? g.B * g.D1 : g.B;
    if (w.has_row && g.row_mode == 1) {
        DConvRowArgs a{{w.tl[0], w.tl[1]}, x, x, g.D1, g.D2};
        return prof.timed(101, "dconv_row_kernel", 2.0 * 2.0 * (3.0 * C * h + 2.0 * 2 * C * h) * (double)rows * g.D2,
                          2.0 * 4.0 * C * (double)rows * g.D2, st, [&] { return launch_dconv_row(a, C, rows, switches().dconv_row_lds, st); });
    }
    if (w.has_time && g.row_mode == 0 && g.D1 == 1) {
        MI_REQUIRE(dconv_gram, "dconv: the engine set no Gram buffer for the time kernels");
        return prof.timed(102, "dconv_time_kernels", 2.0 * 2.0 * (3.0 * C * h + 2.0 * C * h) * (double)g.B * g.D2, 2.0 * 4.0 * C * (double)g.B * g.D2, st, [&] {
            float *s = x, *dd = tmp;
            for (int dlayer = 0; dlayer < 2; ++dlayer) {
                MI_TRY(launch_dconv_time_layer(w.tl[dlayer], C, 1 << dlayer, g.B, g.D2, g.pitch(), s, dd, hidden, stats, dconv_gram, st1, st2, st));
                std::swap(s, dd);
            }
            return (int)MI_OK;
        });
    }
    const double cnt_row = g.row_mode ? (double)g.D2 : (double)g.D1 * g.D2;
    float *src = x, *dst = tmp;
    for (int dlayer = 0; dlayer < 2; ++dlayer) {
        const DConvLayerW &l = w.l[dlayer];
        mi_conv_desc d = base_desc(l.conv3, l.ktab3, src, (int64_t)C * P, g);
        d.epi = MI_EPI_BIAS_STATS; d.y = hidden; d.y_bstride = (int64_t)hp * P; d.y_cstride = P; d.stats = stats;
        if (dconv_tap_dma) {
            d.ntaps = 3; d.tap_k2 = 3; d.tap_pad1 = 0; d.tap_pad2 = 1 << dlayer; d.tap_dil2 = 1 << dlayer;
        }
        MI_TRY(conv(d, st));
        MI_TRY(launch_finalize_stats(stats, rows, cnt_row * h, 1e-5f, 0, st1, nullptr, st));
        const int gslots = g.row_mode ? 1 : 8, HP = gram_hp(h);
        MI_REQUIRE((size_t)rows * gslots * HP * HP * sizeof(double) <= gram2_cap, "dconv: Gram accumulators need %zu bytes, workspace has %zu",
                   (size_t)rows * gslots * HP * HP * sizeof(double), gram2_cap);
        MI_TRY(launch_gn_gelu_gram(hidden, g.B, h, hp, g.D1, g.D2, g.pitch(), g.row_mode, st1, l.gn1_w, l.gn1_b, gram2, gslots, true, st));
        MI_TRY(launch_gram_finalize(gram2, rows, h, gslots, l.gram_wt, l.gram_ct, l.sum_b, l.sum_bsq, cnt_row, cnt_row * 2 * C, 1e-5f, st2, st));
        mi_conv_desc e = base_desc(l.conv1, l.ktab1, hidden, (int64_t)hp * P, g);
        e.plain = 1;
        e.epi = MI_EPI_GN_GLU; e.stats = nullptr; e.gn_stats = (const float *)st2; e.gn_w = l.gn2_w; e.gn_b = l.gn2_b;
        e.scale = l.ls; e.res = src; e.y = dst; e.y_bstride = (int64_t)C * P; e.y_cstride = P;
        MI_TRY(conv(e, st));
        std::swap(src, dst);
    }
    return MI_OK;
}

}
```

### demucs_amd/csrc/gemm_conv.h

```cpp
#pragma once
#include <stdint.h>

#ifdef __cplusplus
extern "C" {
#endif

enum mi_epilogue {
    MI_EPI_LINEAR = 0,
    MI_EPI_GLU = 1,
    MI_EPI_BIAS_STATS = 2,
    MI_EPI_STATS_ONLY = 3,
    MI_EPI_GN_GLU = 4,
    MI_EPI_CONVTR = 5
};

#define MI_FLAG_GELU 1
#define MI_FLAG_SCALE 2
#define MI_FLAG_RES 4
#define MI_FLAG_EMB 8
#define MI_FLAG_TR_FREQ 16
#define MI_FLAG_LN 32
#define MI_FLAG_IMG 64
#define MI_FLAG_HEADS 128
#define MI_FLAG_STATS 256
#define MI_FLAG_IMG4 512

#define MI_SINK_FLOATS 256
#define MI_ZERO_PAGE_FLOATS 64

typedef struct mi_ktab_entry {
    int32_t off;
    int32_t d1;
    int32_t d2;
    int32_t ci;
} mi_ktab_entry;

typedef struct mi_conv_desc {
    const float *wt;
    int32_t M, Mpad, K, Kpad;
    const mi_ktab_entry *ktab;
    const float *x;
    int64_t x_bstride;
    int32_t B, D1, D2, O1, O2, S1, S2;
    int32_t pro;
    const float *pro_stats;
    const float *pro_w, *pro_b;
    int32_t row_mode;
    int32_t epi, flags;
    const float *bias;
    const float *scale;
    const float *res;
    const float *emb;
    float *y;
    int64_t y_bstride, y_cstride;
    double *stats;
    const float *gn_stats;
    const float *gn_w, *gn_b;
    int32_t out_len;
    int32_t tile_m;
    int32_t plain;
    int32_t half;
    int32_t o2_valid;
    int32_t ktab_len;
    float *sink;
    const void *wx;
    int32_t tr_stride;
    int32_t tr_pad;
    int32_t x_ld;
    int32_t x_ld_pad;
    const void *wh;
    const void *xh;
    int64_t xh_n;
    void *yh;
    int64_t yh_n;
    const void *wtap;
    int32_t ntaps, tap_k2, tap_pad1, tap_pad2;
    int32_t tap_dil1, tap_dil2;
    int64_t yh_pq;
    int32_t dma_rows;
    int32_t dma_rows_pad;
    int32_t dma_time;
    int32_t dma_time_pad;
} mi_conv_desc;

#ifdef __cplusplus
}
#endif
```

### demucs_amd/csrc/gemm_conv.hip

```cpp
#include "gemm_loop.h"

namespace mi {

template <int WM, int WN, int TM, int TN, int EPI, int LFLAGS, bool PLAIN>
__global__ __launch_bounds__(256, (TM * TN == 4 ? 3 : 4)) void conv_gemm_kernel(const mi_conv_desc d, const int N, const int MT, const int Gm) {
    constexpr int BM = WM * TM * 32;
    static_assert(WN * TN * 32 == BN, "block N tile is 128");
    static_assert(WM * WN == 4, "4 waves");
    __shared__ float As[2][BK][BM];
    __shared__ float Bs[2][BK][BN];
    Wg w;
    if (!wg_tile<WN, BM>(d, MT, Gm, N, w)) return;
    const int tid = w.tid;

    constexpr int A_F4 = BK * BM / 4, A_FULL = A_F4 / 256, A_REM = A_F4 % 256;
    constexpr int A_SLOTS = A_FULL + (A_REM ? 1 : 0);
    static_assert(A_SLOTS <= 2, "A tile fits two float4 per thread");
    const int aidx0 = tid < A_F4 ? tid : 0, aidx1 = (tid + 256 < A_F4) ? tid + 256 : 0;
    const int ar0 = aidx0 / (BM / 4), ac0 = (aidx0 % (BM / 4)) * 4;
    const int ar1 = aidx1 / (BM / 4), ac1 = (aidx1 % (BM / 4)) * 4;
    const bool a_on0 = tid < A_F4, a_on1 = tid + 256 < A_F4;
    const float *ap0 = d.wt + (size_t)ar0 * d.Mpad + w.m0 + ac0;
    const float *ap1 = d.wt + (size_t)ar1 * d.Mpad + w.m0 + ac1;
    const size_t a_step = (size_t)BK * d.Mpad;
// ... 40 lines not shown
        if (A_SLOTS >= 2 && a_on1) *reinterpret_cast<float4 *>(&As[buf][ar1][ac1]) = areg1;           \
    } while (0)

    f32x16 acc[TM][TN];
    zero_acc(acc);

    const int nk = d.Kpad / BK;
    MI_LOAD_TILE(0);
    MI_STORE_TILE(0);
    __syncthreads();
    int cur = 0;
    for (int kt = 0; kt < nk; ++kt) {
        if (kt + 1 < nk) MI_LOAD_TILE(kt + 1);
        fp32_kstep<TM, TN, BM>(&As[cur][0][0], &Bs[cur][0][0], w, acc);
        if (kt + 1 < nk) MI_STORE_TILE(cur ^ 1);
        __syncthreads();
        cur ^= 1;
    }
#undef MI_LOAD_TILE
#undef MI_STORE_TILE

    conv_epilogue<TM, TN, EPI, LFLAGS>(d, acc, w.m0, w.n0, w.wm, w.wn, N, w.P, w.o2v);
}

template <int BM, int EPI, int LFLAGS, int NT, int DIL, bool ROWPAIRS>
__device__ __forceinline__ void conv_dma_body(const mi_conv_desc &d, const int N, const int MT, const int Gm) {
    constexpr int WM = BM == 128 ? 2 : 1, WN = 4 / WM, TM = BM / (32 * WM), TN = BN / (32 * WN);
    constexpr int SS = BK * (BM + BN);
    __shared__ __attribute__((aligned(16))) float smem[3 * SS];
    Wg w;
    if (!wg_tile<WN, BM>(d, MT, Gm, N, w)) return;
    const AImagePlan<BM, ROWPAIRS> A(d, w);
    BLoader<NT, DIL> B(d, w, N, (int64_t)d.D1 * (d.x_ld ? d.x_ld : d.D2));
    const auto brows = [&](int stage) { return smem + stage * SS + BK * BM + (4 * w.wave) * BN; };
    f32x16 acc[TM][TN];
    zero_acc(acc);
    dma_ring3(
        d.Kpad / BK, kBInFlight + A.in_flight(), [&](int kt) { B.prefetch(kt); },
        [&](int kt, int stage) {
            A.issue(kt, smem + stage * SS);
            B.issue(d, kt, brows(stage));
        },
        [&](int kt, int stage) {
            if constexpr (NT > 0) {
                B.fix(d, kt, brows(stage));
                asm volatile("s_waitcnt lgkmcnt(0)" ::: "memory");
            }
        },
        [&](int stage) { fp32_kstep<TM, TN, BM>(smem + stage * SS, smem + stage * SS + BK * BM, w, acc); });
    conv_epilogue<TM, TN, EPI, LFLAGS>(d, acc, w.m0, w.n0, w.wm, w.wn, N, w.P, w.o2v);
}

template <int EPI, int LFLAGS>
__global__ __launch_bounds__(256, 3) void conv_gemm_dma_kernel(const mi_conv_desc d, const int N, const int MT, const int Gm) {
    conv_dma_body<128, EPI, LFLAGS, 0, 1, true>(d, N, MT, Gm);
}

template <int BMT, int EPI, int NT, int DIL = 1>
__global__ __launch_bounds__(256, 3) void conv_gemm_dmatap_kernel(const mi_conv_desc d, const int N, const int MT, const int Gm) {
    conv_dma_body<BMT, EPI, 0, NT, DIL, true>(d, N, MT, Gm);
}

template <int EPI>
static int launch_dmatap(const mi_conv_desc &d, int tile, hipStream_t st) {
    ConvGeom g;
    MI_TRY(conv_geom(d, "conv: DMA tap route", tile, tile, g));
    if constexpr (EPI == MI_EPI_BIAS_STATS) {
        const bool d2 = d.tap_dil2 == 2;
        if (tile == 64 && d2) MI_LAUNCH_TILES((conv_gemm_dmatap_kernel<64, EPI, 3, 2>), d, g, 1, st);
        else if (tile == 64) MI_LAUNCH_TILES((conv_gemm_dmatap_kernel<64, EPI, 3, 1>), d, g, 1, st);
        else if (d2) MI_LAUNCH_TILES((conv_gemm_dmatap_kernel<32, EPI, 3, 2>), d, g, 1, st);
        else MI_LAUNCH_TILES((conv_gemm_dmatap_kernel<32, EPI, 3, 1>), d, g, 1, st);
    } else if (tile == 128 && d.ntaps == 9) MI_LAUNCH_TILES((conv_gemm_dmatap_kernel<128, EPI, 9>), d, g, 1, st);
    else if (tile == 128) MI_LAUNCH_TILES((conv_gemm_dmatap_kernel<128, EPI, 3>), d, g, 1, st);
    else if (d.ntaps == 9) MI_LAUNCH_TILES((conv_gemm_dmatap_kernel<96, EPI, 9>), d, g, 1, st);
    else MI_LAUNCH_TILES((conv_gemm_dmatap_kernel<96, EPI, 3>), d, g, 1, st);
    return MI_OK;
}

template <int BMT, int EPI, int LFLAGS>
__global__ __launch_bounds__(256, 3) void conv_gemm_dmarow_kernel(const mi_conv_desc d, const int N, const int MT, const int Gm) {
    conv_dma_body<BMT, EPI, LFLAGS, kRowTaps, 1, false>(d, N, MT, Gm);
}

template <int EPI, int LFLAGS>
static int launch_dmarow(const mi_conv_desc &d, int tile, hipStream_t st) {
    ConvGeom g;
    MI_TRY(conv_geom(d, "conv: DMA row route", tile, tile, g));
    if (tile == 128) MI_LAUNCH_TILES((conv_gemm_dmarow_kernel<128, EPI, LFLAGS>), d, g, 1, st);
    else if constexpr (EPI == MI_EPI_LINEAR || EPI == MI_EPI_CONVTR) {
        if (tile == 96) MI_LAUNCH_TILES((conv_gemm_dmarow_kernel<96, EPI, LFLAGS>), d, g, 1, st);
        else MI_LAUNCH_TILES((conv_gemm_dmarow_kernel<64, EPI, LFLAGS>), d, g, 1, st);
    } else return set_error(MI_EINVAL, "conv: DMA row route has no %d-row tile for epilogue %d", tile, EPI);
    return MI_OK;
}

template <int WM, int WN, int TM, int TN, int EPI, int LFLAGS, bool PLAIN>
static int launch_cfg(const mi_conv_desc &d, const ConvRoute &r, hipStream_t st) {
    constexpr int BM = WM * TM * 32;
    const bool dma = r.route == MI_ROUTE_DMA;
    ConvGeom g;
    MI_TRY(conv_geom(d, "conv", BM, BM, g));
    const int Gm = r.mgroups ? pick_m_groups(g.MT, (size_t)d.Kpad * d.Mpad * 4) : 1;
    if constexpr (PLAIN && BM == 128 && EPI == MI_EPI_LINEAR) {
        if (dma) {
            MI_LAUNCH_TILES((conv_gemm_dma_kernel<EPI, LFLAGS>), d, g, Gm, st);
            return MI_OK;
        }
    }
    MI_REQUIRE(!dma, "conv: the LDS-DMA linear tile takes a plain LINEAR layer on the 128-row tile");
    MI_LAUNCH_TILES((conv_gemm_kernel<WM, WN, TM, TN, EPI, LFLAGS, PLAIN>), d, g, Gm, st);
    return MI_OK;
}

template <int EPI, int LFLAGS, bool PLAIN>
static int launch_tile(const mi_conv_desc &d, const ConvRoute &r, hipStream_t st) {
    switch (r.tile) {
        case 128: return launch_cfg<2, 2, 2, 2, EPI, LFLAGS, PLAIN>(d, r, st);
        case 96: return launch_cfg<1, 4, 3, 1, EPI, LFLAGS, PLAIN>(d, r, st);
        case 64: return launch_cfg<1, 4, 2, 1, EPI, LFLAGS, PLAIN>(d, r, st);
        case 32: return launch_cfg<1, 4, 1, 1, EPI, LFLAGS, PLAIN>(d, r, st);
    }
    return set_error(MI_EINVAL, "conv: unsupported tile_m %d", r.tile);
}

static float *conv_sink() {
    static float *p = nullptr;
    if (!p) {
        if (hipMalloc((void **)&p, (MI_SINK_FLOATS + MI_ZERO_PAGE_FLOATS) * sizeof(float)) != hipSuccess) { p = nullptr; return nullptr; }
        (void)hipMemset(p, 0, (MI_SINK_FLOATS + MI_ZERO_PAGE_FLOATS) * sizeof(float));
    }
    return p;
}

const void *conv_zero_page() {
    float *p = conv_sink();
    return p ? p + MI_SINK_FLOATS : nullptr;
}

static int launch_routed(const mi_conv_desc &d, hipStream_t st) {
    const ConvRoute r = conv_route(d);
    const int image_tile = d.tile_m == 192 ? 96 : d.tile_m ? d.tile_m : conv_pick_tile(d.M);
    g_last_conv_route = r.route;
    g_last_conv_tile = r.tile;
    if ((unsigned)r.route < 16u && (unsigned)d.epi < 8u) ++g_conv_route_launches[r.route][d.epi];
    switch (r.route) {
        case MI_ROUTE_TAP_HALF: return launch_conv_tap(d, r.tile, st);
        case MI_ROUTE_HALF:
        case MI_ROUTE_HALF_IMG:
        case MI_ROUTE_HALF_IMG256: return launch_conv_half(d, r, st);
        case MI_ROUTE_TAP_X6: return launch_conv_tap_x6(d, r.tile, image_tile, st);
        case MI_ROUTE_ROWS_X6: return launch_conv_rows_x6(d, r.tile, image_tile, st);
        case MI_ROUTE_TIME_X6: return launch_conv_time_x6(d, r.tile, image_tile, st);
        case MI_ROUTE_X6: return launch_conv_x6(d, r.tile, image_tile, r.plain, st);
        case MI_ROUTE_DMATAP:
            return d.epi == MI_EPI_GLU ? launch_dmatap<MI_EPI_GLU>(d, r.tile, st) : launch_dmatap<MI_EPI_BIAS_STATS>(d, r.tile, st);
        case MI_ROUTE_DMAROW:
            switch (d.epi) {
                case MI_EPI_LINEAR: return launch_dmarow<MI_EPI_LINEAR, MI_FLAG_GELU>(d, r.tile, st);
                case MI_EPI_CONVTR: return launch_dmarow<MI_EPI_CONVTR, 0>(d, r.tile, st);
                case MI_EPI_GLU: return launch_dmarow<MI_EPI_GLU, 0>(d, r.tile, st);
                case MI_EPI_GN_GLU: return launch_dmarow<MI_EPI_GN_GLU, 0>(d, r.tile, st);
            }
            return set_error(MI_EINVAL, "conv: DMA row route has no epilogue %d", d.epi);
    }
    return dispatch_epilogue(d, [&](auto epi, auto lflags) {
        constexpr int E = decltype(epi)::value, F = decltype(lflags)::value;
        return r.plain ? launch_tile<E, F, true>(d, r, st) : launch_tile<E, F, false>(d, r, st);
    });
}

int launch_conv(const mi_conv_desc &din, hipStream_t st) {
    mi_conv_desc d = din;
    if (!d.sink) d.sink = conv_sink();
    MI_REQUIRE(d.sink && ((uintptr_t)d.sink & 15) == 0, "conv: the store sink could not be allocated or is not 16-byte aligned");
    MI_TRY(conv_validate(d));
    if (!conv_stats_per_item(d)) return launch_routed(d, st);
    mi_conv_desc e = d;
    e.B = 1;
    for (int b = 0; b < d.B; ++b) {
        e.x = d.x + (size_t)b * d.x_bstride;
        e.y = d.y ? d.y + (size_t)b * d.y_bstride : nullptr;
        e.res = d.res ? d.res + (size_t)b * d.y_bstride : nullptr;
        e.stats = d.stats ? d.stats + (size_t)b * kStatSlots * 2 : nullptr;
        MI_TRY(launch_routed(e, st));
    }
    return MI_OK;
}

}
```

### demucs_amd/csrc/gemm_x6.hip

```cpp
#include "gemm_loop.h"
#include "split_bf16.h"

namespace mi {

__global__ void pack_split_kernel(const float *__restrict__ wt, int Kpad, int Mpad, int BM, __bf16 *__restrict__ wx) {
    const size_t idx = blockIdx.x * (size_t)blockDim.x + threadIdx.x;
    if (idx >= (size_t)Kpad * Mpad) return;
    const int k = (int)(idx / Mpad), m = (int)(idx % Mpad);
    const int mt = m / BM, mi = m % BM, kt = k / BK, h = (k % BK) / 8, j = k % 8, nk = Kpad / BK;
    const float x = wt[idx];
    const __bf16 a = (__bf16)x;
    const float r = x - (float)a;
    const __bf16 b = (__bf16)r;
    const __bf16 c = (__bf16)(r - (float)b);
    __bf16 *img = wx + ((size_t)mt * nk + kt) * ((size_t)BM * 48);
    img[((0 * 2 + h) * BM + mi) * 8 + j] = a;
    img[((1 * 2 + h) * BM + mi) * 8 + j] = b;
    img[((2 * 2 + h) * BM + mi) * 8 + j] = c;
}

int launch_pack_split(const float *wt, int Kpad, int Mpad, int tile_m, void *wx, hipStream_t st) {
    MI_REQUIRE(Kpad % BK == 0 && Mpad % tile_m == 0, "pack_split: Kpad %d / Mpad %d do not fit tile %d", Kpad, Mpad, tile_m);
    const size_t n = (size_t)Kpad * Mpad;
    hipLaunchKernelGGL(pack_split_kernel, dim3((unsigned)((n + 255) / 256)), dim3(256), 0, st, wt, Kpad, Mpad, tile_m, (__bf16 *)wx);
    MI_CHECK_LAUNCH();
    return MI_OK;
}

template <int WM, int WN, int TM, int TN, int EPI, int LFLAGS, bool PLAIN, bool HALF_IMG, int NT>
__device__ __forceinline__ void conv_x6_body(const mi_conv_desc &d, const int N, const int MT, const int Gm) {
    constexpr int BM = WM * TM * 32;
    constexpr bool RAW = PLAIN || NT != 0;
    constexpr bool ROWS = NT == kRowTaps;
    static_assert(NT <= 0 || (!PLAIN && EPI == MI_EPI_GLU), "tap loader: GLU rewrite convs");
    static_assert(!ROWS || (!PLAIN && (EPI == MI_EPI_LINEAR || EPI == MI_EPI_CONVTR || EPI == MI_EPI_GLU)),
                  "row-tap loader: encoder / transposed convs, 1 x 1 + GLU rewrites");
    static_assert(NT != kTimeTr || (!PLAIN && EPI == MI_EPI_CONVTR), "time-axis two-tap loader: transposed convs");
    static_assert(NT != kTimeEnc || (!PLAIN && EPI == MI_EPI_LINEAR && LFLAGS == MI_FLAG_GELU), "time-axis strided loader: encoder convs");
    static_assert(NT >= kTimeEnc, "NT: taps, 0, kRowTaps, kTimeTr or kTimeEnc");
    static_assert(WN * TN * 32 == BN, "block N tile is 128");
    static_assert(WM * WN == 4, "4 waves");
    constexpr int A_BYTES = BM * 96, B_BYTES = BN * 96, STAGE = A_BYTES + B_BYTES;
    constexpr int A_CHUNKS = A_BYTES / 1024;
    static_assert(!HALF_IMG || BM == 64, "HALF_IMG: 64-row tile of a 128-row image");
    constexpr bool PAIR = BM == 192;
    static_assert(!PAIR || (WM == 2 && TM == 3), "192-row tile: two wave rows of 96 rows");
    constexpr int IMG_ROWS = PAIR ? 96 : BM, IMG_BYTES = IMG_ROWS * 96, IMG_CHUNKS = IMG_BYTES / 1024;
    constexpr int A_KSTEP = HALF_IMG ? 2 * A_BYTES : IMG_BYTES, A_CHUNK_STRIDE = HALF_IMG ? 2048 : 1024;
    __shared__ __attribute__((aligned(16))) unsigned char smem[2 * STAGE];
    __shared__ __attribute__((aligned(16))) float braw[RAW ? 2 * BK * BN : 4];

    agpr_anchor();
    Wg w;
    if (!wg_tile<WN, BM>(d, MT, Gm, N, w)) return;
    const int nk = d.Kpad / BK;

    const unsigned char *aimg = reinterpret_cast<const unsigned char *>(d.wx) + (size_t)(HALF_IMG ? w.mt >> 1 : PAIR ? 2 * w.mt : w.mt) * nk * A_KSTEP +
                                (HALF_IMG ? (w.mt & 1) * 1024 : 0) + w.lane * 16;
#define MI_A_DMA(kt, stage)                                                                                         \
    do {                                                                                                            \
        _Pragma("unroll") for (int c = 0; c < (A_CHUNKS + 3) / 4; ++c) {                                             \
            const int chunk = c * 4 + w.wave, img = PAIR ? chunk / IMG_CHUNKS : 0, ic = chunk - img * IMG_CHUNKS;      \
            if (chunk < A_CHUNKS)                                                                                   \
                lds_dma16_tracked(aimg + ((size_t)img * nk + (kt)) * A_KSTEP + ic * A_CHUNK_STRIDE,                    \
                                  smem + (stage) * STAGE + chunk * 1024);                                          \
        }                                                                                                           \
    } while (0)

    const int bn = w.tid & 127;
    const int bh = __builtin_amdgcn_readfirstlane(w.tid >> 7);
    const ColInfo lc = decompose(w.n0 + bn, N, w.P, d.O2, PLAIN ? d.O2 : w.o2v);
    const int i1b = lc.o1 * d.S1, i2b = lc.o2 * d.S2;
    const float *xcol = d.x + (size_t)lc.b * d.x_bstride + (PLAIN ? (size_t)lc.p : (size_t)i1b * (d.x_ld ? d.x_ld : d.D2) + i2b);
    const float *bp = lc.valid ? xcol + (size_t)(8 * bh) * w.P : d.sink + MI_SINK_FLOATS;
    const size_t b_row = lc.valid ? (size_t)w.P : 0, b_step = lc.valid ? (size_t)BK * w.P : 0;
    float breg[8];
    BLoader<NT> L(d, w, N, w.P);
    constexpr bool OWN_STAGE = NT == kTimeEnc;
#define MI_BRAW_DMA(kt, rs) L.issue(d, (kt), braw + (rs) * (BK * BN) + (OWN_STAGE ? 0 : 4 * w.wave) * BN)
#define MI_BRAW_FIX(kt, rs) L.fix(d, (kt), braw + (rs) * (BK * BN) + (OWN_STAGE ? 0 : 4 * w.wave) * BN)
#define MI_BRAW_READ(rs)                                                                                            \
    do {                                                                                                            \
        if constexpr (OWN_STAGE) {                                                                                  \
            L.read(braw + (rs) * (BK * BN), bn, bh, breg);                                                          \
        } else {                                                                                                    \
            _Pragma("unroll") for (int j = 0; j < 8; ++j) breg[j] = braw[(rs) * (BK * BN) + (8 * bh + j) * BN + bn]; \
        }                                                                                                           \
    } while (0)

#define MI_B_LOAD(kt)                                                                                               \
    do {                                                                                                            \
        if (PLAIN) {                                                                                                \
            _Pragma("unroll") for (int j = 0; j < 8; ++j) breg[j] = bp[(size_t)(kt) * b_step + j * b_row];           \
        } else {                                                                                                    \
            mi_ktab_entry ke[8];                                                                                    \
            _Pragma("unroll") for (int j = 0; j < 8; ++j) ke[j] = d.ktab[(kt) * BK + 8 * bh + j];                    \
            _Pragma("unroll") for (int j = 0; j < 8; ++j) {                                                          \
                bool ok;                                                                                            \
                const float v = gather_b(d, ke[j], xcol, i1b, i2b, lc.valid, ok);                                   \
                breg[j] = ok ? v : 0.f;                                                                             \
            }                                                                                                       \
        }                                                                                                           \
    } while (0)

#define MI_B_STORE(stage)                                                                                           \
    do {                                                                                                            \
        unsigned ph[4], pm[4], pl[4];                                                                               \
        _Pragma("unroll") for (int j = 0; j < 4; ++j) split3(breg[2 * j], breg[2 * j + 1], ph[j], pm[j], pl[j]);    \
        unsigned char *bs = smem + (stage) * STAGE + A_BYTES + (bh * BN + bn) * 16;                                 \
        *reinterpret_cast<uint4 *>(bs) = make_uint4(ph[0], ph[1], ph[2], ph[3]);                                    \
        *reinterpret_cast<uint4 *>(bs + 2 * BN * 16) = make_uint4(pm[0], pm[1], pm[2], pm[3]);                      \
        *reinterpret_cast<uint4 *>(bs + 4 * BN * 16) = make_uint4(pl[0], pl[1], pl[2], pl[3]);                      \
    } while (0)

    f32x16 acc[TM][TN];
    zero_acc(acc);

    constexpr int PA[6] = {2, 0, 1, 1, 0, 0}, PB[6] = {0, 2, 1, 0, 1, 0};
    MI_A_DMA(0, 0);
    if constexpr (RAW) {
        L.prefetch(0);
        MI_BRAW_DMA(0, 0);
        if (nk > 1) {
            L.prefetch(1);
            MI_BRAW_DMA(1, 1);
        }
        if (nk > 2) L.prefetch(2);
        asm volatile("s_waitcnt vmcnt(0)" ::: "memory");
        MI_BRAW_FIX(0, 0);
        if (nk > 1) MI_BRAW_FIX(1, 1);
        __syncthreads();
        MI_BRAW_READ(0);
    } else {
        MI_B_LOAD(0);
    }
    MI_B_STORE(0);
    asm volatile("s_waitcnt vmcnt(0)" ::: "memory");
    __syncthreads();
    int cur = 0;
    for (int kt = 0; kt < nk; ++kt) {
        const unsigned char *As = smem + cur * STAGE, *Bs = As + A_BYTES;
        bf16x8 af[TM][3], bf[TN][3];
#pragma unroll
        for (int p = 0; p < 3; ++p) {
#pragma unroll
            for (int a = 0; a < TM; ++a)
                af[a][p] = *reinterpret_cast<const bf16x8 *>(As + (PAIR ? w.wm * IMG_BYTES : 0) +
                                                             (((p * 2 + w.lh) * IMG_ROWS) + ((PAIR ? 0 : w.wm * TM) + a) * 32 + w.li) * 16);
#pragma unroll
            for (int b = 0; b < TN; ++b)
                bf[b][p] = *reinterpret_cast<const bf16x8 *>(Bs + (((p * 2 + w.lh) * BN) + (w.wn * TN + b) * 32 + w.li) * 16);
        }
        __builtin_amdgcn_sched_barrier(0);
        if (kt + 1 < nk) {
            MI_A_DMA(kt + 1, cur ^ 1);
            if constexpr (RAW) {
                if (kt + 2 < nk) MI_BRAW_DMA(kt + 2, kt & 1);
            } else {
                MI_B_LOAD(kt + 1);
            }
        }
        if constexpr (RAW) {
            MI_BRAW_READ((kt + 1) & 1);
        }
        __builtin_amdgcn_sched_barrier(0);
#pragma unroll
        for (int q = 0; q < 6; ++q)
#pragma unroll
            for (int a = 0; a < TM; ++a)
#pragma unroll
                for (int b = 0; b < TN; ++b)
                    acc[a][b] = __builtin_amdgcn_mfma_f32_32x32x16_bf16(af[a][PA[q]], bf[b][PB[q]], acc[a][b], 0, 0, 0);
        if (RAW || kt + 1 < nk) MI_B_STORE(cur ^ 1);
        if constexpr (RAW) {
#pragma unroll
            for (int i = 0; i < 6 * TM * TN; ++i) {
                __builtin_amdgcn_sched_group_barrier(0x008, 1, 0);
                __builtin_amdgcn_sched_group_barrier(0x002, (72 + 6 * TM * TN - 1) / (6 * TM * TN), 0);
            }
        }
        if constexpr (ROWS) {
            if (kt + 3 < nk) L.template prefetch<true>(kt + 3);
            else asm volatile("s_waitcnt vmcnt(0)" ::: "memory");
        } else {
            asm volatile("s_waitcnt vmcnt(0)" ::: "memory");
        }
        if (kt + 2 < nk) MI_BRAW_FIX(kt + 2, kt & 1);
        __syncthreads();
        cur ^= 1;
    }
#undef MI_A_DMA
#undef MI_B_LOAD
#undef MI_BRAW_DMA
#undef MI_BRAW_FIX
#undef MI_BRAW_READ
#undef MI_B_STORE

    conv_epilogue<TM, TN, EPI, LFLAGS>(d, acc, w.m0, w.n0, w.wm, w.wn, N, w.P, w.o2v);
}

template <int WM, int WN, int TM, int TN, int EPI, int LFLAGS, bool PLAIN, bool HALF_IMG = false>
__global__ __launch_bounds__(256, 2) void conv_gemm_x6_kernel(const mi_conv_desc d, const int N, const int MT, const int Gm) {
    conv_x6_body<WM, WN, TM, TN, EPI, LFLAGS, PLAIN, HALF_IMG, 0>(d, N, MT, Gm);
}

template <int WM, int WN, int TM, int TN, bool HALF_IMG, int NT>
__global__ __launch_bounds__(256, 2) void conv_tap_x6_kernel(const mi_conv_desc d, const int N, const int MT, const int Gm) {
    conv_x6_body<WM, WN, TM, TN, MI_EPI_GLU, 0, false, HALF_IMG, NT>(d, N, MT, Gm);
}

template <int WM, int WN, int TM, int TN, int EPI, int LFLAGS, bool HALF_IMG>
__global__ __launch_bounds__(256, 2) void conv_rows_x6_kernel(const mi_conv_desc d, const int N, const int MT, const int Gm) {
    conv_x6_body<WM, WN, TM, TN, EPI, LFLAGS, false, HALF_IMG, kRowTaps>(d, N, MT, Gm);
}

template <int WM, int WN, int TM, int TN, bool HALF_IMG>
__global__ __launch_bounds__(256, 2) void conv_time_tr_x6_kernel(const mi_conv_desc d, const int N, const int MT, const int Gm) {
    conv_x6_body<WM, WN, TM, TN, MI_EPI_CONVTR, 0, false, HALF_IMG, kTimeTr>(d, N, MT, Gm);
}

template <int WM, int WN, int TM, int TN, bool HALF_IMG>
__global__ __launch_bounds__(256, 2) void conv_time_enc_x6_kernel(const mi_conv_desc d, const int N, const int MT, const int Gm) {
    conv_x6_body<WM, WN, TM, TN, MI_EPI_LINEAR, MI_FLAG_GELU, false, HALF_IMG, kTimeEnc>(d, N, MT, Gm);
}

template <int WM, int WN, int TM, int TN, int EPI, int LFLAGS, bool PLAIN, bool HALF_IMG = false, int NTAPS = 0>
static int launch_cfg_x6(const mi_conv_desc &d, hipStream_t st) {
    constexpr int BM = WM * TM * 32;
    ConvGeom g;
    MI_TRY(conv_geom(d, "conv", BM, HALF_IMG ? 2 * BM : BM, g));
    const int Gm = pick_m_groups(g.MT, (size_t)d.Kpad * d.Mpad * 6);
    if constexpr (NTAPS > 0) MI_LAUNCH_TILES((conv_tap_x6_kernel<WM, WN, TM, TN, HALF_IMG, NTAPS>), d, g, Gm, st);
    else if constexpr (NTAPS == kRowTaps) MI_LAUNCH_TILES((conv_rows_x6_kernel<WM, WN, TM, TN, EPI, LFLAGS, HALF_IMG>), d, g, Gm, st);
    else if constexpr (NTAPS == kTimeTr) MI_LAUNCH_TILES((conv_time_tr_x6_kernel<WM, WN, TM, TN, HALF_IMG>), d, g, Gm, st);
    else if constexpr (NTAPS == kTimeEnc) MI_LAUNCH_TILES((conv_time_enc_x6_kernel<WM, WN, TM, TN, HALF_IMG>), d, g, Gm, st);
    else MI_LAUNCH_TILES((conv_gemm_x6_kernel<WM, WN, TM, TN, EPI, LFLAGS, PLAIN, HALF_IMG>), d, g, Gm, st);
    return MI_OK;
}

template <int EPI, int LFLAGS, bool PLAIN, int NTAPS>
static int launch_tile_x6(const mi_conv_desc &d, int tile, int image_tile, hipStream_t st) {
    if (tile != image_tile) {
        if constexpr (NTAPS != 0 || (PLAIN && EPI == MI_EPI_LINEAR)) {
            if (tile == 64 && image_tile == 128) return launch_cfg_x6<1, 4, 2, 1, EPI, LFLAGS, PLAIN, true, NTAPS>(d, st);
        }
        if constexpr (conv_x6_tile192(EPI, LFLAGS, PLAIN, NTAPS)) {
            if (tile == 192 && image_tile == 96) return launch_cfg_x6<2, 2, 3, 2, EPI, LFLAGS, PLAIN, false, NTAPS>(d, st);
        }
        return set_error(MI_EINVAL, "conv x6: no %d-row tile on a %d-row image for epilogue %d", tile, image_tile, EPI);
    }
    switch (tile) {
        case 128: return launch_cfg_x6<2, 2, 2, 2, EPI, LFLAGS, PLAIN, false, NTAPS>(d, st);
        case 96: return launch_cfg_x6<1, 4, 3, 1, EPI, LFLAGS, PLAIN, false, NTAPS>(d, st);
        case 64:
            if constexpr (NTAPS == 0) return launch_cfg_x6<1, 4, 2, 1, EPI, LFLAGS, PLAIN>(d, st);
    }
    return set_error(MI_EINVAL, "conv x6: unsupported tile_m %d", tile);
}

int launch_conv_tap_x6(const mi_conv_desc &d, int tile, int image_tile, hipStream_t st) {
    MI_REQUIRE(d.wx && ((uintptr_t)d.wx & 15) == 0, "conv tap x6: split weight image missing or misaligned");
    MI_REQUIRE(d.epi == MI_EPI_GLU && (image_tile == 96 || image_tile == 128) && (d.ntaps == 9 || d.ntaps == 3),
               "conv tap x6: GLU layer with 9 or 3 taps on a 96- or 128-row tile (epi %d, tile %d, ntaps %d)", d.epi, image_tile, d.ntaps);
    return d.ntaps == 9 ? launch_tile_x6<MI_EPI_GLU, 0, false, 9>(d, tile, image_tile, st) : launch_tile_x6<MI_EPI_GLU, 0, false, 3>(d, tile, image_tile, st);
}

int launch_conv_rows_x6(const mi_conv_desc &d, int tile, int image_tile, hipStream_t st) {
    MI_REQUIRE(d.wx && ((uintptr_t)d.wx & 15) == 0, "conv rows x6: split weight image missing or misaligned");
    MI_REQUIRE(d.ktab && ((uintptr_t)d.ktab & 63) == 0, "conv rows x6: gather table missing or misaligned");
    MI_REQUIRE(image_tile == 96 || image_tile == 128, "conv rows x6: 96- or 128-row tile (tile %d)", image_tile);
    if (d.epi == MI_EPI_CONVTR) return launch_tile_x6<MI_EPI_CONVTR, 0, false, kRowTaps>(d, tile, image_tile, st);
    if (d.epi == MI_EPI_GLU) {
        MI_REQUIRE(image_tile == 128 || d.tile_m == 192, "conv rows x6: GLU on a 128-row tile or a 192-row layer (tile %d)", image_tile);
        return launch_tile_x6<MI_EPI_GLU, 0, false, kRowTaps>(d, tile, image_tile, st);
    }
    MI_REQUIRE(d.epi == MI_EPI_LINEAR && (d.flags & (MI_FLAG_GELU | MI_FLAG_SCALE | MI_FLAG_RES | MI_FLAG_LN | MI_FLAG_STATS)) == MI_FLAG_GELU,
               "conv rows x6: LINEAR + GELU, CONVTR or GLU (epi %d, flags %d)", d.epi, d.flags);
    return launch_tile_x6<MI_EPI_LINEAR, MI_FLAG_GELU, false, kRowTaps>(d, tile, image_tile, st);
}

int launch_conv_time_x6(const mi_conv_desc &d, int tile, int image_tile, hipStream_t st) {
    MI_REQUIRE(d.wx && ((uintptr_t)d.wx & 15) == 0, "conv time x6: split weight image missing or misaligned");
    MI_REQUIRE((image_tile == 96 || image_tile == 128) && d.D1 == 1 && d.O1 == 1, "conv time x6: a 1-D layer on a 96- or 128-row tile (tile %d)", image_tile);
    if (d.epi == MI_EPI_CONVTR) {
        MI_REQUIRE(d.O2 % 4 == 0 && d.o2_valid == d.D2 + 1 && d.o2_valid <= d.O2 && d.K % 2 == 0,
                   "conv time x6: columns 0 .. D2 on a pitch that is a multiple of 4 (D2 %d, O2 %d, o2_valid %d)", d.D2, d.O2, d.o2_valid);
        return launch_tile_x6<MI_EPI_CONVTR, 0, false, kTimeTr>(d, tile, image_tile, st);
    }
    MI_REQUIRE(d.epi == MI_EPI_LINEAR && (d.flags & (MI_FLAG_GELU | MI_FLAG_SCALE | MI_FLAG_RES | MI_FLAG_LN | MI_FLAG_STATS)) == MI_FLAG_GELU &&
               d.S2 == 4 && d.K % 8 == 0, "conv time x6: CONVTR, or LINEAR + GELU with k = 8, s = 4 (epi %d, flags %d, S2 %d)", d.epi, d.flags, d.S2);
    return launch_tile_x6<MI_EPI_LINEAR, MI_FLAG_GELU, false, kTimeEnc>(d, tile, image_tile, st);
}

int launch_conv_x6(const mi_conv_desc &d, int tile, int image_tile, bool plain, hipStream_t st) {
    MI_REQUIRE(d.wx && ((uintptr_t)d.wx & 15) == 0, "conv x6: split weight image missing or misaligned");
    return dispatch_epilogue(d, [&](auto epi, auto lflags) {
        constexpr int E = decltype(epi)::value, F = decltype(lflags)::value;
        return plain ? launch_tile_x6<E, F, true, 0>(d, tile, image_tile, st) : launch_tile_x6<E, F, false, 0>(d, tile, image_tile, st);
    });
}

}
```

### demucs_amd/csrc/kernels.h

```cpp
#pragma once
#include <cmath>
#include <vector>
#include <hip/hip_runtime.h>
#include <stdint.h>

#include "gemm_conv.h"

namespace mi {

struct FftTables {
    const float *window;
    const float2 *twiddle;
    const float *envelope;
};
struct FftHostTables {
    std::vector<float> window, envelope;
    std::vector<float2> twiddle;
};
static inline FftHostTables fft_host_tables() {
    FftHostTables t{std::vector<float>(4096), std::vector<float>(1024), std::vector<float2>(2048)};
    for (int i = 0; i < 4096; ++i) t.window[i] = 0.5f - 0.5f * cosf((float)i * (float)(2.0 * M_PI / 4096.0));
    for (int r = 0; r < 1024; ++r) {
        float e = 0.f;
        for (int j = 3; j >= 0; --j) e += t.window[r + 1024 * j] * t.window[r + 1024 * j];
        t.envelope[r] = e;
    }
    for (int i = 0; i < 2048; ++i) { const double a = -2.0 * M_PI * i / 4096.0; t.twiddle[i] = make_float2((float)cos(a), (float)sin(a)); }
    return t;
}

int launch_stft_frames(const float *mix, int B, int L, const FftTables &tb, float *zt, double *stats, hipStream_t st);
int launch_cac_transpose(const float *zt, int B, int T, const float2 *norm, float *x, hipStream_t st, int x_pitch = 0 );
int launch_istft(const float *y, int B, int S, int L, const float2 *denorm, const float *xt, const float2 *denorm_t,
                 const FftTables &tb, float *yt, float *fr, float *out, hipStream_t st, int xt_pitch = 0 ,
                 int y_pitch = 0 );

extern int g_transpose_tiles;
extern int g_istft_fused;

int launch_row_stats(const float *x, int rows, int64_t count, int64_t row_stride, double *stats, hipStream_t st);
int launch_finalize_stats(double *stats, int rows, double count, float eps, int mode, float2 *out_a, float2 *out_b,
                          hipStream_t st);
int launch_row_affine(const float *x, int rows, int64_t count, const float2 *norm, float *y, hipStream_t st);
int launch_row_denorm(const float *x, int rows, int64_t count, const float2 *denorm, float *y, hipStream_t st);
int launch_layernorm_cf(const float *x, int B, int C, int T, const float *w, const float *b, const float *pe, float *y,
                        float2 *ostat, hipStream_t st, void *img = nullptr, int64_t img_n = 0, int img_dtype = 0);
int launch_token_stats(const float *x, int B, int C, int T, float2 *ostat, hipStream_t st, void *img = nullptr, int64_t img_n = 0,
                       int img_dtype = 0);
int launch_gn_apply_tokstats(const float *x, int B, int C, int T, const float2 *gstat, const float *w, const float *b, float *y,
                             float2 *ostat, hipStream_t st, void *img = nullptr, int64_t img_n = 0, int img_dtype = 0);

int gram_hp(int h);
int launch_gn_gelu_gram(float *x, int B, int h, int Cs, int D1, int D2 , int pitch, int row_mode, const float2 *stats, const float *w,
                        const float *b, double *gram , int slots, bool zero_pad, hipStream_t st);
int launch_gram_finalize(double *gram, int rows, int h, int slots, const double *wt , const double *ct , double sum_b,
                         double sum_bsq, double cols, double count, float eps, float2 *out, hipStream_t st);
int launch_gn_gelu(float *x, int B, int C, int Cs, int D1, int D2, int row_mode, const float2 *stats, const float *w, const float *b,
                   hipStream_t st);

struct DConvRowLayer {
    const float *w0;
    const float *b0;
    const float *g1w, *g1b;
    const float *w3;
    const float *b3, *g2w, *g2b;
    const float *ls;
};
struct DConvTimeLayer {
    DConvRowLayer w;
    const double *gram_a;
    const double *gram_v;
    const double *gram_c;
    const double *gram_e1, *gram_e2;
    double sum_b3, sum_b3sq;
};
struct DConvRowArgs {
    DConvTimeLayer l[2];
    const float *x;
    float *y;
    int Fr, T;
};
struct DConvHostPack {
    std::vector<float> w0, b0, g1w, g1b, w3;
    std::vector<double> gram_a, gram_v, gram_c, gram_e1, gram_e2;
    double sum_b3, sum_b3sq;
};
DConvHostPack dconv_pack_host(int C, int h, const float *w0, const float *b0, const float *g1w, const float *g1b, const float *w3,
                              const float *b3);
bool dconv_row_supported(int C, int T);
bool dconv_row_lds_supported(int C, int T);
int launch_dconv_row(const DConvRowArgs &a, int C, int rows, bool lds_row, hipStream_t st);

bool dconv_time_supported(int C, int Lp);
int launch_dconv_time_layer(const DConvTimeLayer &l, int C, int dil, int B, int Lv, int Lp, const float *x, float *y, float *hbuf,
                            double *stats, double *gram, float2 *st1, float2 *st2, hipStream_t st);

int launch_conv(const mi_conv_desc &d, hipStream_t st);

constexpr int BK = 16;
constexpr int BN = 128;
int conv_pick_tile(int M);
int conv_check_tile_m(const mi_conv_desc &d);
int conv_validate(const mi_conv_desc &d);
bool conv_stats_per_item(const mi_conv_desc &d);
extern int g_split_bf16;
struct ConvRoute { int route; int tile; bool plain; bool mgroups; };
ConvRoute conv_route(const mi_conv_desc &d);
struct Switches {
    bool no_dma;
    bool no_dma_tap;
    bool no_dma_rows;
    bool no_dma_dconv;
    bool small_tile;
    bool mgroups;
    bool x6_plain_only;
    bool img256;
    bool half_tile256;
    int x6_scope;
    bool no_tap_image;
    bool no_enc_image;
    bool no_dconv_time;
    bool no_lin2_stats;
    bool no_ffn_image;
    bool no_qkv_heads;
    bool no_input_image;
    bool one_stream;
    bool debug_sync;
    int side_prio;
    bool h_no_deep_tap;
    bool h_no_last_tap;
    bool h_one_stream;
    bool lstm_steps;
    bool lstm_write_through;
    bool lstm_debug;
    int transpose_tiles;
    bool istft_split;
    bool dconv_row_lds;
};
const Switches &switches();
constexpr bool conv_x6_supported(int tile) { return tile == 128 || tile == 96 || tile == 64; }
constexpr int kRowTaps = -1;
constexpr int kTimeTr = -2;
constexpr int kTimeEnc = -3;
constexpr bool conv_x6_tile192(int epi, int lflags, bool plain, int ntaps) {
    if (ntaps > 0) return epi == MI_EPI_GLU;
    if (ntaps == kTimeTr) return epi == MI_EPI_CONVTR;
    if (ntaps == kTimeEnc) return epi == MI_EPI_LINEAR && lflags == MI_FLAG_GELU;
    if (ntaps == kRowTaps) return (epi == MI_EPI_LINEAR && lflags == MI_FLAG_GELU) || epi == MI_EPI_CONVTR || epi == MI_EPI_GLU;
    return plain && epi == MI_EPI_LINEAR && lflags == MI_FLAG_LN;
}
int launch_conv_x6(const mi_conv_desc &d, int tile, int image_tile, bool plain, hipStream_t st);
int launch_conv_tap_x6(const mi_conv_desc &d, int tile, int image_tile, hipStream_t st);
int launch_conv_rows_x6(const mi_conv_desc &d, int tile, int image_tile, hipStream_t st);
int launch_conv_time_x6(const mi_conv_desc &d, int tile, int image_tile, hipStream_t st);
int launch_pack_split(const float *wt, int Kpad, int Mpad, int tile_m, void *wx, hipStream_t st);

int launch_conv_half(const mi_conv_desc &d, const ConvRoute &r, hipStream_t st);
int launch_pack_half(const float *wt, int Kpad, int Mpad, int dtype, void *wh, hipStream_t st);
int conv_tap_pairs_pad(int Cin, int ntaps);
int launch_pack_tap(const float *wt, int Mpad, int Cin, int ntaps, int dtype, void *out, hipStream_t st);
int launch_conv_tap(const mi_conv_desc &d, int tile, hipStream_t st);
int launch_f32_to_image(const float *x, int B, int C, int64_t P, int dtype, void *img, hipStream_t st);

int launch_row_affine_pitch(const float *x, int B, int C, int L, int out_pitch, const float2 *norm, float *y, hipStream_t st);
int launch_gn_apply(const float *x, int B, int Cin, int G, int in_pitch, int off, const float2 *stats, const float *w, const float *bias,
                    int glu, int gelu, const float *scale, const float *res, int res_pitch, float *y, int Cout, int out_len,
                    int out_pitch, hipStream_t st, int chan_div = 1);
int launch_unfold_frames(const float *x, int B, int C, int T, int F, int W, int S, float *fr, hipStream_t st);
int launch_restitch_frames(const float *fr, int B, int C, int T, int F, int W, int S, const float *skip, float *y, hipStream_t st);
void pack_lstm_whh(const float *whh , int H, float *packed);
int launch_lstm_seq(const float *gx, const float *whh , int N, int H, int W, float *out, float *state , hipStream_t st);
size_t lstm_persist_scratch_bytes();
size_t lstm_persist_ctl_offset();
int launch_lstm_persist(const float *gx, const float *whh , int N, int H, int W, float *out, void *scratch, unsigned *ctl_host,
                        hipStream_t st);
int launch_lstm_small(const float *gx, const float *whh_natural , int N, int H, int W, float *out, hipStream_t st);
int launch_local_attn(const float *qkc, int B, int C, int T, int ld , float *out, int ld_o, hipStream_t st);

int launch_attention(const float *q, const float *k, const float *v, float *o, int B, int heads, int Tq, int Tk, int64_t q_bs,
                     int64_t kv_bs, int64_t o_bs, int dtype, hipStream_t st, void *oh = nullptr, int64_t oh_n = 0);
int launch_attention_x6(const float *q, const float *k, const float *v, float *o, int B, int heads, int Tq, int Tk, int64_t q_bs,
                        int64_t kv_bs, int64_t o_bs, hipStream_t st);

int launch_segments_gather(const float *track, int64_t track_len, int channels, const int64_t *starts_dev, int B, int valid,
                           float *seg, hipStream_t st);
int launch_ola_accumulate(float *acc, int64_t acc_len, int rows, const float *model_out, int valid, const int64_t *offs_dev,
                          const int32_t *lens_dev, const int32_t *trim_dev, int B, int64_t span_lo, int64_t span_hi,
                          const float *weight, int weight_len, hipStream_t st);
int launch_ola_finish(float *acc, int64_t acc_len, int rows, int64_t acc_off0, const int64_t *offs_dev, const int32_t *lens_dev,
                      int n_segments, int max_len, const float *weight, hipStream_t st);

int launch_segments_gather_packed(const float *tracks, int64_t tracks_cap, int channels, const int64_t *items_dev, int B, int valid,
                                  float *seg, hipStream_t st);
int launch_ola_accumulate_packed(float *acc, int64_t acc_cap, int rows, const float *model_out, int valid, const int64_t *items_dev,
                                 int B, const int64_t *tiles_dev, int n_tiles, const float *weights, int64_t weights_cap,
                                 hipStream_t st);
int launch_ola_finish_packed(float *acc, int64_t acc_cap, int rows, const int64_t *tiles_dev, int n_tiles, const int64_t *segs_dev,
                             int n_segs, const float *weights, int64_t weights_cap, hipStream_t st);

int launch_resample_frac(const float *x, int rows, int64_t L, const float *table, int old_sr, int new_sr, int width, float *y,
                         int64_t Lout, hipStream_t st);

int launch_streams_convert_append(float *win, int64_t win_cap, int channels, const int64_t *table, int n_streams, int64_t max_groups,
                                  const float *bank, int64_t bank_cap, float *hist, int64_t hist_cap, const float *stats, int n_stats,
                                  int lds_floats, hipStream_t st);
int launch_streams_convert_append_pcm(float *win, int64_t win_cap, int channels, const int64_t *table, int n_streams,
                                      int64_t max_groups, const float *bank, int64_t bank_cap, float *hist, int64_t hist_cap,
                                      const float *stats, int n_stats, int lds_floats, hipStream_t st);

int launch_pcm_planar(const unsigned char *src, int fmt, int src_ch, int64_t n, int channels, const float *stats, float *dst,
                      hipStream_t st);
int launch_streams_append_pcm(float *win, int64_t win_cap, int channels, const int64_t *table, int n_streams, int64_t max_bytes,
                              const float *stats, int n_stats, hipStream_t st);

int mono_stats_state_bytes();
int launch_mono_stats_update(const unsigned char *src, int fmt, int src_ch, int64_t n, int channels, int64_t before, double *state,
                             hipStream_t st);
int launch_mono_stats_finish(const double *state, int64_t length, double *scratch, float *stats, hipStream_t st);

int64_t sdr_state_bytes(int n_sources);
int64_t sdr_scratch_bytes(int n_sources);
int launch_sdr_update(const void *const *refs, int fmt, int src_ch, int64_t ref_stride, const float *est, int64_t est_stride, int n_sources,
                      int channels, int64_t n, int64_t before, double *state, hipStream_t st);
int launch_sdr_finish(const double *state, int n_sources, double *scratch, double *sums, hipStream_t st);
int launch_sdr(const float *ref, const float *est, int B, int n_sources, int channels, int64_t length, double *state, double *scratch,
               double *sums, hipStream_t st);

const void *conv_zero_page();
int launch_attention_heads(const void *q, const void *k, const void *v, const void *zero_page, int B, int heads, int Tq, int Tk, int Tq_pitch,
                           int Tk_pitch, int dtype, void *oh, int64_t oh_n, float *o, int64_t o_bs, hipStream_t st);

int post_stats_scratch_bytes();
int launch_mono_stats(const float *wav, int channels, int64_t length, double *scratch, float *stats, hipStream_t st);
int launch_mono_stats_final(const double *scratch, int64_t length, float *stats, hipStream_t st);
int launch_stream_emit(const float *acc, int64_t acc_cap, int n_sources, int channels, const int64_t *passes, int n_passes,
                       const int64_t *segs, int n_segs, const float *weights, int64_t weights_cap, const float *scales, int n_members,
                       int shifts, int bag, const float *stats, int64_t n, float *out, hipStream_t st);
int launch_streams_emit(const float *acc, int64_t acc_cap, int n_sources, int channels, const int64_t *streams, int n_streams, int64_t max_n,
                        const int64_t *passes, int n_passes, const int64_t *segs, int n_segs, const float *weights, int64_t weights_cap,
                        const float *scales, int n_members, int shifts, int bag, const float *stats, int n_stats, float *out,
                        int64_t out_cap, hipStream_t st);
int launch_streams_append(float *win, int64_t win_cap, int channels, const int64_t *table, int n_streams, int64_t max_n,
                          const float *stats, int n_stats, hipStream_t st);
int launch_streams_compact(float *dst, int64_t dst_cap, const float *src, int64_t src_cap, const int64_t *table, int n_rows, int64_t max_len,
                           hipStream_t st);
int launch_track_affine(float *x, int64_t n, const float *stats, int mode, hipStream_t st);
int launch_prevent_clip(const float *x, int64_t n, int mode, unsigned *peak, float *y, hipStream_t st);
int launch_two_stems(const float *const *stems, int S, int sel, const float *origin, int mode, int64_t n, float *y, hipStream_t st);

int launch_deliver_peaks(const int64_t *table, int n_rows, int64_t max_n, int n_sources, int channels, unsigned *peaks, int n_peaks,
                         int64_t dst_cap, hipStream_t st);
int launch_deliver_pcm(const int64_t *table, int n_rows, int64_t max_n, int n_sources, int channels, const unsigned *peaks, int n_peaks,
                       unsigned char *dst, int64_t dst_cap, hipStream_t st);

int launch_deliver_mix_pcm(const int64_t *table, int n_rows, int64_t max_n, int n_sources, int channels, const unsigned *peaks,
                           int n_peaks, unsigned char *dst, int64_t dst_cap, hipStream_t st);
int launch_deliver_mix_peaks(const int64_t *table, int n_rows, int64_t max_n, int n_sources, int channels, unsigned *peaks, int n_peaks,
                             int64_t dst_cap, hipStream_t st);
int launch_deliver_mix_peaks_update(const int64_t *table, int n_rows, int64_t max_n, int n_sources, int channels, unsigned *peaks,
                                    int n_peaks, hipStream_t st);

int launch_deliver_mix_auto_pcm(const int64_t *table, int64_t table_len, int n_rows, int64_t max_n, int n_sources, int channels,
                                const unsigned *peaks, int n_peaks, unsigned char *dst, int64_t dst_cap, hipStream_t st);
int launch_deliver_mix_auto_peaks(const int64_t *table, int64_t table_len, int n_rows, int64_t max_n, int n_sources, int channels,
                                  unsigned *peaks, int n_peaks, int64_t dst_cap, hipStream_t st);

int launch_deliver_resample_pcm(const int64_t *table, int n_rows, int64_t max_groups, int n_sources, int channels, const float *bank,
                                int64_t bank_cap, float *hist, int64_t hist_cap, int lds_floats, unsigned char *dst, int64_t dst_cap,
                                hipStream_t st);

int launch_deliver_peaks_update(const int64_t *table, int n_rows, int64_t max_n, int n_sources, int channels, unsigned *peaks,
                                int n_peaks, hipStream_t st);
int launch_deliver_resample_peaks(const int64_t *table, int n_rows, int64_t max_groups, int n_sources, int channels, const float *bank,
                                  int64_t bank_cap, float *hist, int64_t hist_cap, int lds_floats, const int32_t *slots, unsigned *peaks,
                                  int n_peaks, hipStream_t st);
int launch_deliver_resample_pcm_peaks(const int64_t *table, int n_rows, int64_t max_groups, int n_sources, int channels,
                                      const float *bank, int64_t bank_cap, float *hist, int64_t hist_cap, int lds_floats, unsigned char *dst,
                                      int64_t dst_cap, const int32_t *slots, const unsigned *peaks, int n_peaks, hipStream_t st);

int launch_loudness_update(const int64_t *table, int n_rows, int64_t max_n, int64_t max_blocks, int n_sources, int channels,
                           const double *coef, int64_t hop, int64_t warm, float *hist, int64_t hist_cap, double *energies, int64_t e_cap,
                           float *work, int64_t work_cap, hipStream_t st);

}
```

### demucs_amd/csrc/model.hip

```cpp
#include <cmath>
#include <map>
#include <memory>
#include <mutex>
#include <string>
#include <vector>

#include "model.h"

namespace mi {

int Model::attn(const float *q, const float *k, const float *v, float *o, int B, int Tq, int Tk, int64_t q_bs, int64_t kv_bs,
                int64_t o_bs, hipStream_t st, bool image) {
    void *oh = image ? (void *)o : nullptr;
    const int64_t oh_n = (int64_t)B * Tq;
    const bool x6 = cfg.dtype == MI_DTYPE_F32 && !image && g_split_bf16 && switches().x6_scope != 0;
    auto launch = [&]() {
        return x6 ? launch_attention_x6(q, k, v, o, B, 8, Tq, Tk, q_bs, kv_bs, o_bs, st)
                  : launch_attention(q, k, v, o, B, 8, Tq, Tk, q_bs, kv_bs, o_bs, cfg.dtype, st, oh, oh_n);
    };
    const int cls = x6 ? 104 : 100;
    const char *name = x6 ? "attention_x6_kernel" : cfg.dtype == MI_DTYPE_BF16 ? "attention_bf16_kernel" : cfg.dtype == MI_DTYPE_F16 ? "attention_f16_kernel" : "attention_kernel";
    return prof.timed(cls, name, 4.0 * B * 8 * (double)Tq * Tk * 64.0, 4.0 * B * 512.0 * (2.0 * Tq + 2.0 * Tk), st, launch);
}

int Model::attn_heads(const void *q, const void *k, const void *v, float *o, int B, int Tq, int Tk, hipStream_t st) {
    const int64_t oh_n = (int64_t)B * Tq;
    const void *zero = conv_zero_page();
    MI_REQUIRE(zero, "attention: could not allocate the zero page");
    return prof.timed(100, cfg.dtype == MI_DTYPE_BF16 ? "attention_heads_bf16_kernel" : "attention_heads_f16_kernel",
                      4.0 * B * 8 * (double)Tq * Tk * 64.0, 2.0 * B * 512.0 * (2.0 * Tq + 2.0 * Tk), st,
                      [&] { return launch_attention_heads(q, k, v, zero, B, 8, Tq, Tk, Tq, Tk, cfg.dtype, o, oh_n, nullptr, 0, st); });
}

static const int kFr[5] = {2048, 512, 128, 32, 8};
static const int kCh[4] = {48, 96, 192, 384};

int Model::init(const mi_config &c, const mi_tensor_desc *weights, size_t n) {
    cfg = c;
    MI_REQUIRE(c.n_sources >= 1 && c.n_sources <= 8, "n_sources %d unsupported", c.n_sources);
    MI_REQUIRE(c.max_batch >= 1 && c.max_batch <= 64, "max_batch %d out of range [1, 64]", c.max_batch);
    MI_REQUIRE(c.dtype == MI_DTYPE_F32 || c.dtype == MI_DTYPE_BF16 || c.dtype == MI_DTYPE_F16, "unknown compute dtype %d", c.dtype);
    MI_REQUIRE(c.segment_length > 4096 && c.segment_length % 4 == 0, "segment_length %d unsupported", c.segment_length);
    S = c.n_sources; SL = c.segment_length; T = (SL + 1023) / 1024;
    MI_REQUIRE(T % 4 == 0, "segment_length %d gives %d STFT frames; the engine needs a multiple of 4", SL, T);
    Lt[0] = SL;
    for (int i = 0; i < 4; ++i) Lt[i + 1] = (Lt[i] + 3) / 4;
    for (int i = 0; i < 5; ++i) Lp[i] = round_up(Lt[i], 4);
    MI_REQUIRE(Lt[4] % 4 == 0, "time branch bottleneck length %d must be a multiple of 4", Lt[4]);
    WeightTable wt;
    for (size_t i = 0; i < n; ++i) wt.t[weights[i].name] = {weights[i].data, weights[i].numel};

    MI_TRY(upload_fft_tables());

    for (int i = 0; i < 4; ++i) {
        const int Cin = i ? kCh[i - 1] : 4, C = kCh[i];
        const std::string p = "encoder." + std::to_string(i);
        const float *w, *b, *rw, *rb;
        MI_TRY(wt.get(p + ".conv.weight", (int64_t)C * Cin * 8, &w));
        MI_TRY(wt.get(p + ".conv.bias", C, &b));
        MI_TRY(wt.get(p + ".rewrite.weight", (int64_t)2 * C * C, &rw));
        MI_TRY(wt.get(p + ".rewrite.bias", 2 * C, &rb));
        EncW &e = enc[i];
        MI_TRY(pack_conv(w, b, C, Cin * 8, false, &e.conv, 0, i > 0 ? SPLIT_ROWS : SPLIT_OPT_IN));
        if (i) MI_TRY(pack_enc_tap(w, Cin, &e.conv));
        MI_TRY(make_ktab(Gather{Cin, 8, 1, 1, 1, 2, 0, (int64_t)kFr[i] * T, T}, e.conv.Kpad, &e.ktab_conv));
        MI_TRY(pack_conv(rw, rb, 2 * C, C, true, &e.rewrite, 0, i >= 2 ? SPLIT_ROWS : SPLIT_OPT_IN));
        MI_TRY(make_ktab(Gather{C, 1, 1, 1, 1, 0, 0, (int64_t)kFr[i + 1] * T, T}, e.rewrite.Kpad, &e.ktab_rw));
        MI_TRY(load_dconv(wt, p, C, (int64_t)kFr[i + 1] * T, T, true, &e.dconv));

        const int Cint = i ? kCh[i - 1] : 2;
        const std::string pt = "tencoder." + std::to_string(i);
        MI_TRY(wt.get(pt + ".conv.weight", (int64_t)C * Cint * 8, &w));
        MI_TRY(wt.get(pt + ".conv.bias", C, &b));
        MI_TRY(wt.get(pt + ".rewrite.weight", (int64_t)2 * C * C, &rw));
        MI_TRY(wt.get(pt + ".rewrite.bias", 2 * C, &rb));
        EncW &te = tenc[i];
        MI_TRY(pack_conv(w, b, C, Cint * 8, false, &te.conv, 0, i > 0 ? SPLIT_TIME : SPLIT_OPT_IN));
        if (i) MI_TRY(pack_enc_tap(w, Cint, &te.conv));
        MI_TRY(make_ktab(Gather{Cint, 1, 8, 1, 1, 0, 2, (int64_t)Lp[i], Lp[i]}, te.conv.Kpad, &te.ktab_conv));
        MI_TRY(pack_conv(rw, rb, 2 * C, C, true, &te.rewrite, 0, i >= 2 ? SPLIT_ROWS : SPLIT_OPT_IN));
        MI_TRY(make_ktab(Gather{C, 1, 1, 1, 1, 0, 0, (int64_t)Lp[i + 1], Lp[i + 1]}, te.rewrite.Kpad, &te.ktab_rw));
        MI_TRY(load_dconv(wt, pt, C, (int64_t)Lp[i + 1], Lp[i + 1], false, &te.dconv));
    }
    {
        const float *ew;
        MI_TRY(wt.get("freq_emb.embedding.weight", 512 * 48, &ew));
        std::vector<float> emb(48 * 512);
        for (int f = 0; f < 512; ++f)
            for (int ch = 0; ch < 48; ++ch) emb[ch * 512 + f] = 0.2f * (ew[f * 48 + ch] * 10.0f);
        MI_TRY(upload(emb, &freq_emb));
    }
    for (int j = 0; j < 4; ++j) {
        const int C = kCh[3 - j], Fr = kFr[4 - j];
        const int Cout = j < 3 ? kCh[2 - j] : 4 * S, Coutt = j < 3 ? kCh[2 - j] : 2 * S;
        const std::string p = "decoder." + std::to_string(j);
        const float *w, *b, *rw, *rb;
        MI_TRY(wt.get(p + ".conv_tr.weight", (int64_t)C * Cout * 8, &w));
        MI_TRY(wt.get(p + ".conv_tr.bias", Cout, &b));
        MI_TRY(wt.get(p + ".rewrite.weight", (int64_t)2 * C * C * 9, &rw));
        MI_TRY(wt.get(p + ".rewrite.bias", 2 * C, &rb));
        DecW &dd = dec[j];
        MI_TRY(pack_conv(rw, rb, 2 * C, C * 9, true, &dd.rewrite, 9, SPLIT_DEFAULT));
        MI_TRY(make_ktab(Gather{C, 3, 3, 1, 1, 1, 1, (int64_t)Fr * T, T}, dd.rewrite.Kpad, &dd.ktab_rw));
        MI_TRY(load_dconv(wt, p, C, (int64_t)Fr * T, T, true, &dd.dconv));
        MI_TRY(pack_convtr(w, b, C, Cout, &dd.convtr, 4, j < 3 ? SPLIT_ROWS : SPLIT_OPT_IN));
        MI_TRY(make_ktab(Gather{C, 2, 1, -1, 1, 0, 0, (int64_t)Fr * T, T}, dd.convtr.Kpad, &dd.ktab_tr));

        const int L = Lp[4 - j];
        const std::string pt = "tdecoder." + std::to_string(j);
        MI_TRY(wt.get(pt + ".conv_tr.weight", (int64_t)C * Coutt * 8, &w));
        MI_TRY(wt.get(pt + ".conv_tr.bias", Coutt, &b));
        MI_TRY(wt.get(pt + ".rewrite.weight", (int64_t)2 * C * C * 3, &rw));
        MI_TRY(wt.get(pt + ".rewrite.bias", 2 * C, &rb));
        DecW &td = tdec[j];
        MI_TRY(pack_conv(rw, rb, 2 * C, C * 3, true, &td.rewrite, 3, SPLIT_DEFAULT));
        MI_TRY(make_ktab(Gather{C, 1, 3, 1, 1, 0, 1, (int64_t)L, L}, td.rewrite.Kpad, &td.ktab_rw));
        MI_TRY(load_dconv(wt, pt, C, (int64_t)L, L, false, &td.dconv));
        MI_TRY(pack_convtr(w, b, C, Coutt, &td.convtr, 4, j < 3 ? SPLIT_TIME : SPLIT_OPT_IN));
        MI_TRY(make_ktab(Gather{C, 1, 2, 1, -1, 0, 0, (int64_t)L, L}, td.convtr.Kpad, &td.ktab_tr));
    }
    const int Tf = 8 * T, Tt = Lt[4];
    {
        const char *names[4] = {"channel_upsampler", "channel_upsampler_t", "channel_downsampler", "channel_downsampler_t"};
        for (int i = 0; i < 4; ++i) {
            const int M = i < 2 ? 512 : 384, K = i < 2 ? 384 : 512, P = (i & 1) ? Tt : Tf;
            const float *w, *b;
            MI_TRY(wt.get(std::string(names[i]) + ".weight", (int64_t)M * K, &w));
            MI_TRY(wt.get(std::string(names[i]) + ".bias", M, &b));
            MI_TRY(pack_conv(w, b, M, K, false, &chan[i]));
            MI_TRY(make_ktab(Gather{K, 1, 1, 1, 1, 0, 0, (int64_t)P, P}, chan[i].Kpad, &chan_ktab[i]));
        }
        for (int br = 0; br < 2; ++br) {
            const int P = br ? Tt : Tf;
            MI_TRY(make_ktab(Gather{512, 1, 1, 1, 1, 0, 0, (int64_t)P, P}, 512, &tr_ktab512[br]));
            MI_TRY(make_ktab(Gather{2048, 1, 1, 1, 1, 0, 0, (int64_t)P, P}, 2048, &tr_ktab2048[br]));
        }
    }
    for (int br = 0; br < 2; ++br) {
        const std::string ni = br ? "crosstransformer.norm_in_t" : "crosstransformer.norm_in";
        const float *w, *b;
        MI_TRY(wt.get(ni + ".weight", 512, &w)); MI_TRY(wt.get(ni + ".bias", 512, &b));
        MI_TRY(pack_vec(w, 512, 512, false, &norm_in_w[br])); MI_TRY(pack_vec(b, 512, 512, false, &norm_in_b[br]));
        for (int k = 0; k < 5; ++k) {
            const std::string p = std::string("crosstransformer.") + (br ? "layers_t." : "layers.") + std::to_string(k);
            const bool cross = k & 1;
            const std::string at = p + (cross ? ".cross_attn" : ".self_attn");
            TrLayerW &l = tr[br][k];
            const float *ipw, *ipb, *ow, *ob, *w1, *b1, *w2, *b2;
            MI_TRY(wt.get(at + ".in_proj_weight", 1536 * 512, &ipw));
            MI_TRY(wt.get(at + ".in_proj_bias", 1536, &ipb));
            MI_TRY(wt.get(at + ".out_proj.weight", 512 * 512, &ow));
            MI_TRY(wt.get(at + ".out_proj.bias", 512, &ob));
            MI_TRY(wt.get(p + ".linear1.weight", 2048 * 512, &w1)); MI_TRY(wt.get(p + ".linear1.bias", 2048, &b1));
            MI_TRY(wt.get(p + ".linear2.weight", 512 * 2048, &w2)); MI_TRY(wt.get(p + ".linear2.bias", 512, &b2));
            const float *nw[4] = {}, *nb[4] = {};
            const char *nn[4] = {".norm1", ".norm2", ".norm3", ".norm_out"};
            for (int q = 0; q < 4; ++q) {
                if (q == 2 && !cross) continue;
                MI_TRY(wt.get(p + nn[q] + ".weight", 512, &nw[q])); MI_TRY(wt.get(p + nn[q] + ".bias", 512, &nb[q]));
            }
            MI_TRY(pack_vec(nw[3], 512, 512, false, &l.norm_w[3])); MI_TRY(pack_vec(nb[3], 512, 512, false, &l.norm_b[3]));
            if (cross) {
                MI_TRY(pack_linear_ln(ipw, ipb, nw[0], nb[0], 512, 512, &l.q_proj, &l.q_c1, SPLIT_DEFAULT));
                MI_TRY(pack_linear_ln(ipw + 512 * 512, ipb + 512, nw[1], nb[1], 1024, 512, &l.kv_proj, &l.kv_c1, SPLIT_DEFAULT));
                MI_TRY(pack_linear_ln(w1, b1, nw[2], nb[2], 2048, 512, &l.lin1, &l.lin1_c1, SPLIT_DEFAULT));
            } else {
                MI_TRY(pack_linear_ln(ipw, ipb, nw[0], nb[0], 1536, 512, &l.qkv_proj, &l.qkv_c1, SPLIT_DEFAULT));
                MI_TRY(pack_linear_ln(w1, b1, nw[1], nb[1], 2048, 512, &l.lin1, &l.lin1_c1, SPLIT_DEFAULT));
            }
            MI_TRY(pack_conv(ow, ob, 512, 512, false, &l.out_proj, 0, SPLIT_DEFAULT));
            MI_TRY(pack_conv(w2, b2, 512, 2048, false, &l.lin2, 0, SPLIT_DEFAULT));
            MI_TRY(wt.get(p + ".gamma_1.scale", 512, &w)); MI_TRY(pack_vec(w, 512, 512, false, &l.gamma1));
            MI_TRY(wt.get(p + ".gamma_2.scale", 512, &w)); MI_TRY(pack_vec(w, 512, 512, false, &l.gamma2));
        }
    }
    {
        std::vector<float> pe2((size_t)512 * Tf), pe1((size_t)512 * Tt);
        for (int i = 0; i < 128; ++i) {
            const float div = expf((float)(2 * i) * (float)(-(log(10000.0) / 256.0)));
            for (int fr = 0; fr < 8; ++fr)
                for (int t1 = 0; t1 < T; ++t1) {
                    const size_t tok = (size_t)fr * T + t1;
                    pe2[(size_t)(2 * i) * Tf + tok] = sinf((float)t1 * div);
                    pe2[(size_t)(2 * i + 1) * Tf + tok] = cosf((float)t1 * div);
                    pe2[(size_t)(256 + 2 * i) * Tf + tok] = sinf((float)fr * div);
                    pe2[(size_t)(256 + 2 * i + 1) * Tf + tok] = cosf((float)fr * div);
                }
        }
        for (int i = 0; i < 256; ++i) {
            const float den = powf(10000.0f, (float)i / 255.0f);
            for (int t2 = 0; t2 < Tt; ++t2) {
                const float ph = (float)t2 / den;
                pe1[(size_t)i * Tt + t2] = cosf(ph);
                pe1[(size_t)(256 + i) * Tt + t2] = sinf(ph);
            }
        }
        MI_TRY(upload(pe2, &pos_emb[0])); MI_TRY(upload(pe1, &pos_emb[1]));
    }
    MI_TRY(alloc_workspace());
    {
        const Switches &sw = switches();
        const bool half = cfg.dtype != MI_DTYPE_F32;
        plan.ffn_img = half && !sw.no_ffn_image;
        plan.qkv_heads = plan.ffn_img && !sw.no_qkv_heads;
        plan.in_img = plan.qkv_heads && !sw.no_input_image;
        plan.lin2_stats = !sw.no_lin2_stats;
        plan.tap_img = half && dec[0].rewrite.wtap && tdec[0].rewrite.wtap;
        for (int i = 1; i < 4; ++i) {
            plan.enc_img[0][i] = enc[i].conv.wtap && w_eimg[0][i - 1];
            plan.enc_img[1][i] = tenc[i].conv.wtap && w_eimg[1][i - 1];
        }
    }
    MI_HIP(hipDeviceSynchronize());
    return MI_OK;
}

static std::mutex g_ws_mutex;
static std::map<std::string, std::weak_ptr<Workspace>> g_ws;

int Model::alloc_workspace() {
    int dev = 0;
    MI_HIP(hipGetDevice(&dev));
    char key[128];
    snprintf(key, sizeof(key), "htdemucs dev%d S%d SL%d B%d %s", dev, S, SL, cfg.max_batch, cfg.dtype == MI_DTYPE_F32 ? "f32" : "half");
    std::lock_guard<std::mutex> lock(g_ws_mutex);
    auto it = g_ws.find(key);
    if (it != g_ws.end()) ws = it->second.lock();
    if (!ws) {
        auto w = std::make_shared<Workspace>();
        w->key = key;
        MI_TRY(fill_workspace(*w));
        g_ws[key] = w;
        ws = w;
    }
    static_cast<WorkspacePtrs &>(*this) = *ws;
    dconv_gram = w_gram; dconv_gram2 = w_gram2; dconv_gram2_bytes = gram2_bytes;
    dconv_tap_dma = true;
    return MI_OK;
}

int Model::fill_workspace(Workspace &w) {
    const size_t B = cfg.max_batch;
    auto A = [&](float **p, size_t per_item) { return w.mem.alloc((void **)p, per_item * B * sizeof(float)); };
    auto dev_alloc = [&](void **p, size_t n) { return w.mem.alloc(p, n); };
    MI_TRY(A(&w.w_xt0, (size_t)2 * SL));
    MI_TRY(A(&w.w_zt, (size_t)4 * 2048 * T));
    MI_TRY(A(&w.w_x0, (size_t)4 * 2048 * T));
    size_t big = 0;
    for (int i = 0; i < 4; ++i) {
        const size_t nf = (size_t)kCh[i] * kFr[i + 1] * T, nt = (size_t)kCh[i] * Lp[i + 1];
        MI_TRY(A(&w.w_skip[i], nf));
        MI_TRY(w.mem.alloc((void **)&w.w_skip_t[i], (nt * B + 64) * sizeof(float)));
        w.w_skip_t[i] += 32;
        big = std::max(big, std::max(nf, nt));
    }
    if (cfg.dtype != MI_DTYPE_F32)
        for (int i = 0; i < 3; ++i) {
            const size_t pqf = (size_t)(kFr[i + 1] / 4 + 1) * T, pqt = round_up(ceil_div(Lt[i + 1], 4) + 1, 4);
            float *pf = nullptr, *pt = nullptr;
            MI_TRY(A(&pf, 2 * kCh[i] * pqf)); MI_TRY(A(&pt, 2 * kCh[i] * pqt));
            MI_HIP(hipMemset(pf, 0, 2 * kCh[i] * pqf * B * sizeof(float)));
            MI_HIP(hipMemset(pt, 0, 2 * kCh[i] * pqt * B * sizeof(float)));
            w.w_eimg[0][i] = pf; w.w_eimg[1][i] = pt;
        }
    MI_TRY(A(&w.w_h, big / 2)); MI_TRY(A(&w.w_th, big / 2));
    for (float **p : {&w.w_a, &w.w_b, &w.w_ta, &w.w_tb, &w.w_c, &w.w_tc}) {
        MI_TRY(w.mem.alloc((void **)p, (big * B + 64) * sizeof(float)));
        *p += 32;
    }
    MI_HIP(hipMemset(w.w_h, 0, (big / 2) * B * sizeof(float)));
    MI_HIP(hipMemset(w.w_th, 0, (big / 2) * B * sizeof(float)));
    const size_t Tf = 8 * (size_t)T, Tt = Lt[4];
    for (int br = 0; br < 2; ++br) {
        const size_t P = br ? Tt : Tf;
        MI_TRY(A(&w.w_tr_x[br][0], 512 * P)); MI_TRY(A(&w.w_tr_x[br][1], 512 * P));
        if (cfg.dtype != MI_DTYPE_F32) {
            MI_TRY(A(&w.w_tr_ximg[br][0], 256 * P)); MI_TRY(A(&w.w_tr_ximg[br][1], 256 * P)); MI_TRY(A(&w.w_tr_x1img[br], 256 * P));
        }
        for (int q = 0; q < 2; ++q) MI_TRY(dev_alloc((void **)&w.w_tr_stat[br][q], B * P * sizeof(float2)));
        MI_TRY(dev_alloc((void **)&w.w_tr_stat1[br], B * P * sizeof(float2)));
        MI_TRY(A(&w.w_tr_qkv[br], 1536 * Tf)) ; MI_TRY(A(&w.w_tr_att[br], 512 * P));
        MI_TRY(A(&w.w_tr_x1[br], 512 * P)); MI_TRY(A(&w.w_tr_x2[br], 512 * P)); MI_TRY(A(&w.w_tr_ffh[br], 2048 * P));
// ... 329 lines not shown
```

### include/demucs_amd.h

```cpp
#ifndef DEMUCS_AMD_H
#define DEMUCS_AMD_H

#include <stddef.h>
#include <stdint.h>

#ifdef __cplusplus
extern "C" {
#endif

#define MI_OK 0
#define MI_EINVAL (-1)
#define MI_EHIP (-2)
#define MI_ENOMEM (-3)
#define MI_EWEIGHT (-4)

typedef struct mi_tensor_desc {
    const char *name;
    const float *data;
    int64_t numel;
} mi_tensor_desc;

typedef struct mi_config {
    int32_t n_sources;
    int32_t segment_length;
// ... 261 lines not shown
#define MI_MIX_CLIP 11
#define MI_MIX_PEAK 12
#define MI_MIX_FMT 13
#define MI_MIX_DST_OFF 14
#define MI_MIX_COLS 15
#define MI_MIX_MAX_SOURCES 8
int mi_deliver_mix_pcm(const int64_t *table_dev, int32_t n_rows, int64_t max_n, int32_t n_sources, int32_t channels,
                       const void *peaks_dev, int32_t n_peaks, void *dst_dev, int64_t dst_capacity, void *stream);
int mi_deliver_mix_peaks(const int64_t *table_dev, int32_t n_rows, int64_t max_n, int32_t n_sources, int32_t channels, void *peaks_dev,
                         int32_t n_peaks, int64_t dst_capacity, void *stream);
int mi_deliver_mix_peaks_update(const int64_t *table_dev, int32_t n_rows, int64_t max_n, int32_t n_sources, int32_t channels,
                                void *peaks_dev, int32_t n_peaks, void *stream);

#define MI_AUTO_SRC 0
#define MI_AUTO_N 1
#define MI_AUTO_ORIGIN 2
#define MI_AUTO_ORIGIN_PITCH 3
#define MI_AUTO_ORIGIN_AFFINE 4
#define MI_AUTO_AFFINE_ON 5
#define MI_AUTO_GAINS 6
#define MI_AUTO_CLIP 11
#define MI_AUTO_PEAK 12
#define MI_AUTO_FMT 13
#define MI_AUTO_DST_OFF 14
#define MI_AUTO_T0 15
#define MI_AUTO_CHG_OFF 16
#define MI_AUTO_CHG_N 17
#define MI_AUTO_COLS 18
#define MI_AUTO_CHG_AT 0
#define MI_AUTO_CHG_RAMP 1
#define MI_AUTO_CHG_GAINS 2
#define MI_AUTO_CHG_COLS 7
int mi_deliver_mix_auto_pcm(const int64_t *table_dev, int64_t table_len, int32_t n_rows, int64_t max_n, int32_t n_sources,
                            int32_t channels, const void *peaks_dev, int32_t n_peaks, void *dst_dev, int64_t dst_capacity, void *stream);
int mi_deliver_mix_auto_peaks(const int64_t *table_dev, int64_t table_len, int32_t n_rows, int64_t max_n, int32_t n_sources,
                              int32_t channels, void *peaks_dev, int32_t n_peaks, int64_t dst_capacity, void *stream);

#define MI_LOUD_SRC 0
#define MI_LOUD_N 1
#define MI_LOUD_ORIGIN 2
#define MI_LOUD_ORIGIN_PITCH 3
#define MI_LOUD_ORIGIN_AFFINE 4
#define MI_LOUD_AFFINE_ON 5
#define MI_LOUD_GAINS 6
#define MI_LOUD_SRC_PITCH 11
#define MI_LOUD_BEFORE 12
#define MI_LOUD_HIST_LEN 13
#define MI_LOUD_HIST_RD 14
#define MI_LOUD_HIST_WR 15
#define MI_LOUD_HIST_START 16
#define MI_LOUD_HIST_NEXT 17
#define MI_LOUD_E_OFF 18
#define MI_LOUD_E_PITCH 19
#define MI_LOUD_WORK_OFF 20
#define MI_LOUD_WORK_PITCH 21
#define MI_LOUD_COLS 22
int mi_loudness_update(const int64_t *table_dev, int32_t n_rows, int64_t max_n, int64_t max_blocks, int32_t n_sources, int32_t channels,
                       const double *coef, int64_t hop, int64_t warm, float *hist_dev, int64_t hist_capacity, double *energies_dev,
                       int64_t energies_capacity, float *work_dev, int64_t work_capacity, void *stream);

int mi_stft_cac(const float *mix_dev, int32_t B, int32_t L, float *cac_dev, void *stream);
int mi_istft_cac(const float *x_dev, int32_t B, int32_t S, int32_t L, float *wav_dev, void *stream);

int mi_stft_norm(const float *mix_dev, int32_t B, int32_t L, float *x_dev, int32_t x_pitch, float *norm_dev, float *denorm_dev, void *stream);
int mi_istft_full(const float *y_dev, int32_t B, int32_t S, int32_t L, int32_t y_pitch, const float *denorm_f_dev, const float *xt_dev,
                  int32_t xt_pitch, const float *denorm_t_dev, float *wav_dev, void *stream);
int mi_item_norm(const float *x_dev, int32_t rows, int64_t count, float *y_dev, float *norm_dev, float *denorm_dev, void *stream);
int mi_item_denorm(const float *x_dev, int32_t rows, int64_t count, const float *denorm_dev, float *y_dev, void *stream);

struct mi_conv_desc;
int mi_conv_forward(const struct mi_conv_desc *desc, void *stream);

int mi_conv_pack_split(const float *wt_dev, int32_t Kpad, int32_t Mpad, int32_t tile_m, void *wx_dev, void *stream);

int mi_conv_pack_tap(const float *wt_dev, int32_t Mpad, int32_t Cin, int32_t ntaps, int32_t dtype, void *wtap_dev, void *stream);
int mi_f32_to_image(const float *x_dev, int32_t B, int32_t C, int64_t P, int32_t dtype, void *img_dev, void *stream);

int mi_conv_pack_half(const float *wt_dev, int32_t Kpad, int32_t Mpad, int32_t dtype, void *wh_dev, void *stream);

int mi_attention(const float *q_dev, const float *k_dev, const float *v_dev, float *o_dev, int32_t B, int32_t heads,
                 int32_t Tq, int32_t Tk, int64_t q_batch_stride, int64_t kv_batch_stride, int64_t o_batch_stride,
                 int32_t dtype, void *stream);

int mi_attention_split(const float *q_dev, const float *k_dev, const float *v_dev, float *o_dev, int32_t B, int32_t heads,
                       int32_t Tq, int32_t Tk, int64_t q_batch_stride, int64_t kv_batch_stride, int64_t o_batch_stride,
                       void *stream);

int mi_attention_heads(const void *q_dev, const void *k_dev, const void *v_dev, float *o_dev, int32_t B, int32_t heads, int32_t Tq, int32_t Tk,
                       int32_t Tq_pitch, int32_t Tk_pitch, int32_t dtype, void *stream);

int mi_attention_heads_image(const void *q_dev, const void *k_dev, const void *v_dev, void *img_dev, int64_t n_img, int32_t B, int32_t heads,
                             int32_t Tq, int32_t Tk, int32_t Tq_pitch, int32_t Tk_pitch, int32_t dtype, void *stream);

int mi_attention_image(const float *q_dev, const float *k_dev, const float *v_dev, void *img_dev, int64_t n_img, int32_t B,
                       int32_t heads, int32_t Tq, int32_t Tk, int64_t q_batch_stride, int64_t kv_batch_stride, int32_t dtype,
                       void *stream);

int mi_gn_gelu(float *x_dev, int32_t B, int32_t C, int32_t C_alloc, int32_t D1, int32_t D2, int32_t row_mode, const float *stats_dev,
               const float *w_dev, const float *b_dev, void *stream);

int32_t mi_gram_order(int32_t h);
int mi_gn_gelu_gram(float *x_dev, int32_t B, int32_t h, int32_t C_alloc, int32_t D1, int32_t D2, int32_t pitch, int32_t row_mode,
                    const float *stats_dev, const float *w_dev, const float *b_dev, double *gram_dev, int32_t slots, void *stream);
int mi_dconv_gn_gelu_gram(float *x_dev, int32_t B, int32_t h, int32_t C_alloc, int32_t D1, int32_t D2, int32_t pitch, int32_t row_mode,
                          const float *stats_dev, const float *w_dev, const float *b_dev, double *gram_dev, int32_t slots, void *stream);
int mi_gram_finalize(double *gram_dev, int32_t rows, int32_t h, int32_t slots, const double *wt_dev, const double *ct_dev, double sum_b,
                     double sum_bsq, double cols, double count, float eps, float *stats_out_dev, void *stream);

int mi_lstm_seq(const float *gx_dev, const float *whh_host, int32_t N, int32_t H, int32_t W, float *out_dev, int32_t mode, void *stream);

int mi_layernorm_cf(const float *x_dev, int32_t B, int32_t C, int32_t T, const float *w_dev, const float *b_dev,
                    const float *add_dev, float *y_dev, void *stream);


int mi_token_norm(int32_t mode, const float *x_dev, int32_t B, int32_t C, int32_t T, const float *w_dev, const float *b_dev,
                  const float *pe_dev, const float *gstat_dev, float *y_dev, float *ostat_dev, void *img_dev, int64_t img_n,
                  int32_t img_dtype, void *stream);

int mi_local_attn(const float *qkc_dev, int32_t B, int32_t C, int32_t T, int32_t ld, float *out_dev, int32_t ld_o, void *stream);

int mi_group_norm_apply(const float *x_dev, int32_t B, int32_t Cin, int32_t G, int32_t in_pitch, int32_t in_len, int32_t off,
                        const float *w_dev, const float *b_dev, int32_t glu, int32_t gelu, const float *scale_dev, const float *res_dev,
                        int32_t res_pitch, float *y_dev, int32_t Cout, int32_t out_len, int32_t out_pitch, int32_t chan_div,
                        double *stats_ws_dev, float *stats_out_dev, void *stream);

int mi_blstm_unfold(const float *x_dev, int32_t B, int32_t C, int32_t T, int32_t F, int32_t W, int32_t S, float *frames_dev, void *stream);
int mi_blstm_restitch(const float *frames_dev, int32_t B, int32_t C, int32_t T, int32_t F, int32_t W, int32_t S, const float *skip_dev,
                      float *y_dev, void *stream);

int mi_row_affine_pitch(const float *x_dev, int32_t B, int32_t C, int32_t L, int32_t out_pitch, const float *norm_dev, float *y_dev,
                        void *stream);


int mi_dconv_row(const float *x_dev, float *y_dev, int32_t B, int32_t C, int32_t Fr, int32_t T, const float *weights_host, int32_t variant,
                 void *stream);

int mi_dconv_time_layer(const float *x_dev, float *y_dev, int32_t B, int32_t C, int32_t Lv, int32_t Lp, int32_t dil,
                        const float *weights_host, float *hbuf_dev, double *stats_dev, double *gram_dev, float *st_dev, void *stream);

void mi_debug_set_post_launch_hook(void (*hook)(void *stream));

enum mi_conv_route {
    MI_ROUTE_TABLE = 0,
    MI_ROUTE_DMA = 1,
    MI_ROUTE_DMATAP = 2,
    MI_ROUTE_DMAROW = 3,
    MI_ROUTE_X6 = 4,
    MI_ROUTE_HALF = 5,
    MI_ROUTE_TAP_HALF = 6,
    MI_ROUTE_TAP_X6 = 7,
    MI_ROUTE_ROWS_X6 = 8,
    MI_ROUTE_HALF_IMG = 9,
    MI_ROUTE_HALF_IMG256 = 10,
    MI_ROUTE_TIME_X6 = 11
};

int mi_debug_last_conv_route(void);

int mi_debug_last_conv_tile(void);

int mi_debug_conv_staged(void);

int64_t mi_debug_conv_route_launches(int32_t route, int32_t epi);

int mi_debug_conv_route(const struct mi_conv_desc *desc, int *tile);

int mi_debug_switches(char *buf, int32_t n);

const char *mi_last_error(void);
const char *mi_version(void);

#ifdef __cplusplus
}
#endif
#endif
```

Before: 2421.

## Route dilated dconv, rewrite and channel convs onto split-weight x6 kernels

```diff
diff --git a/demucs_amd/_lib.py b/demucs_amd/_lib.py
--- a/demucs_amd/_lib.py
+++ b/demucs_amd/_lib.py
@@ -43,7 +43,7 @@
         ("wtap", C.c_void_p), ("ntaps", C.c_int32), ("tap_k2", C.c_int32), ("tap_pad1", C.c_int32), ("tap_pad2", C.c_int32),
         ("tap_dil1", C.c_int32), ("tap_dil2", C.c_int32), ("yh_pq", C.c_int64),
         ("dma_rows", C.c_int32), ("dma_rows_pad", C.c_int32),
-        ("dma_time", C.c_int32), ("dma_time_pad", C.c_int32),
+        ("dma_time", C.c_int32), ("dma_dil", C.c_int32),
     ]
 
 
diff --git a/demucs_amd/csrc/api.hip b/demucs_amd/csrc/api.hip
--- a/demucs_amd/csrc/api.hip
+++ b/demucs_amd/csrc/api.hip
@@ -119,7 +119,7 @@
 }
 constexpr size_t kConvSlack = 128;
 int g_conv_staged = 0;
-static bool conv_reads_slack(int route) { return route == MI_ROUTE_DMATAP || route == MI_ROUTE_TAP_X6 || route == MI_ROUTE_TIME_X6; }
+static bool conv_reads_slack(int route) { return route == MI_ROUTE_DMATAP || route == MI_ROUTE_TAP_X6 || route == MI_ROUTE_TIME_X6 || route == MI_ROUTE_DIL_X6; }
 static bool conv_owns_slack(const float *x, size_t bytes) {
     hipDeviceptr_t base = nullptr;
     size_t size = 0;
@@ -781,7 +781,7 @@
 }
 
 int mi_conv_pack_split(const float *wt_dev, int32_t Kpad, int32_t Mpad, int32_t tile_m, void *wx_dev, void *stream) {
-    MI_REQUIRE(wt_dev && wx_dev && Kpad > 0 && Mpad > 0 && (conv_x6_supported(tile_m) || tile_m == 192), "mi_conv_pack_split: bad argument");
+    MI_REQUIRE(wt_dev && wx_dev && Kpad > 0 && Mpad > 0 && (conv_x6_image_tile(tile_m) || tile_m == 192), "mi_conv_pack_split: bad argument");
     MI_REQUIRE(tile_m != 192 || Mpad % 192 == 0, "mi_conv_pack_split: tile_m 192 needs Mpad %% 192 == 0 (Mpad %d)", Mpad);
     return launch_pack_split(wt_dev, Kpad, Mpad, tile_m == 192 ? 96 : tile_m, wx_dev, (hipStream_t)stream);
 }
diff --git a/demucs_amd/csrc/conv_route.hip b/demucs_amd/csrc/conv_route.hip
--- a/demucs_amd/csrc/conv_route.hip
+++ b/demucs_amd/csrc/conv_route.hip
@@ -25,7 +25,7 @@
     const int dil = d.tap_dil2 ? d.tap_dil2 : 1;
     const bool kind = (d.epi == MI_EPI_GLU && (tile == 96 || tile == 128) && (d.ntaps == 9 || d.ntaps == 3) && dil == 1) ||
                       (d.epi == MI_EPI_BIAS_STATS && (tile == 32 || tile == 64) && d.ntaps == 3 && (dil == 1 || dil == 2) && d.flags == 0);
-    return !off && !d.half && (split ? has_image && d.epi == MI_EPI_GLU : !has_image) && kind && d.tap_k2 == 3 && d.Mpad % tile == 0 &&
+    return !off && !d.half && (split ? has_image && (d.epi == MI_EPI_GLU || d.dma_dil) : !has_image) && kind && d.tap_k2 == 3 && d.Mpad % tile == 0 &&
            d.K % d.ntaps == 0 && d.S1 == 1 && d.S2 == 1 && d.O1 == d.D1 && d.O2 == ld && ld % 4 == 0 && d.tap_pad2 == dil &&
            d.tap_pad1 == (d.ntaps / 3 - 1) / 2 && !(d.flags & (MI_FLAG_IMG | MI_FLAG_IMG4)) && d.x_bstride == (int64_t)(d.K / d.ntaps) * d.D1 * ld;
 }
@@ -139,7 +139,8 @@
         const bool filled = !(sw.small_tile && under_filled(d, 192));
         return filled && conv_x6_tile192(d.epi, d.epi == MI_EPI_LINEAR ? lf : 0, plain, ntaps) ? 192 : 96;
     };
-    if (!plain && !sw.x6_plain_only && dmatap_eligible(d, tile, image, true)) return {MI_ROUTE_TAP_X6, split_tile(d.ntaps), plain};
+    if (!plain && !sw.x6_plain_only && dmatap_eligible(d, tile, image, true))
+        return d.epi == MI_EPI_BIAS_STATS ? ConvRoute{MI_ROUTE_DIL_X6, tile, plain} : ConvRoute{MI_ROUTE_TAP_X6, split_tile(d.ntaps), plain};
     if (!sw.x6_plain_only && dmarow_eligible(d, tile, plain, image, true)) return {MI_ROUTE_ROWS_X6, split_tile(kRowTaps), plain};
     if (!sw.x6_plain_only && dmatime_eligible(d, tile, plain, image))
         return {MI_ROUTE_TIME_X6, split_tile(d.epi == MI_EPI_CONVTR ? kTimeTr : kTimeEnc), plain};
diff --git a/demucs_amd/csrc/engine_core.h b/demucs_amd/csrc/engine_core.h
--- a/demucs_amd/csrc/engine_core.h
+++ b/demucs_amd/csrc/engine_core.h
@@ -84,6 +84,7 @@
     SPLIT_DEFAULT,
     SPLIT_ROWS,
     SPLIT_TIME,
+    SPLIT_REST,
 };
 
 struct WeightTable {
diff --git a/demucs_amd/csrc/engine_core.hip b/demucs_amd/csrc/engine_core.hip
--- a/demucs_amd/csrc/engine_core.hip
+++ b/demucs_amd/csrc/engine_core.hip
@@ -89,10 +89,13 @@
     if (!prof.on) return launch_conv(d, st);
     const int route = conv_route(d).route;
     const int tile = d.tile_m && d.tile_m != 192 ? d.tile_m : conv_pick_tile(d.M), ti = tile == 32 ? 0 : tile == 64 ? 1 : tile == 96 ? 2 : 3;
-    const bool tap_x6 = route == MI_ROUTE_TAP_X6, rows_x6 = route == MI_ROUTE_ROWS_X6, time_x6 = route == MI_ROUTE_TIME_X6;
+    const int lf = d.flags & (MI_FLAG_GELU | MI_FLAG_SCALE | MI_FLAG_RES | MI_FLAG_LN | MI_FLAG_STATS);
+    const bool tap_x6 = route == MI_ROUTE_TAP_X6, rows_x6 = route == MI_ROUTE_ROWS_X6;
+    const bool native_row = route == MI_ROUTE_TIME_X6 || route == MI_ROUTE_DIL_X6 ||
+                            (route == MI_ROUTE_X6 && conv_x6_own_symbol(d.epi, d.epi == MI_EPI_LINEAR ? lf : 0, d.plain));
     const int cls = tap_x6    ? 105 + (d.ntaps == 9 ? 2 : 0) + (tile == 128 ? 1 : 0)
                     : rows_x6 ? 109 + (d.epi == MI_EPI_CONVTR ? 4 : d.epi == MI_EPI_GLU ? 2 : 0) + (tile == 128 ? 1 : 0)
-                              : (route >= MI_ROUTE_X6 && !time_x6 ? 48 : 0) + d.epi * 8 + ti * 2 + (d.plain ? 1 : 0);
+                              : (route >= MI_ROUTE_X6 && !native_row ? 48 : 0) + d.epi * 8 + ti * 2 + (d.plain ? 1 : 0);
     const double N = (double)d.B * d.O1 * d.O2;
     const double in_bytes = 4.0 * (double)d.B * (double)d.x_bstride;
     double out_rows = d.M;
@@ -115,10 +118,10 @@
 
 int EngineCore::pack_split(PackedConv *pc, SplitScope scope) {
     const Switches &sw = switches();
-    const bool in_default = scope == SPLIT_DEFAULT || scope == SPLIT_TIME || (scope == SPLIT_ROWS && !sw.no_dma_rows);
+    const bool in_default = scope == SPLIT_DEFAULT || scope == SPLIT_TIME || scope == SPLIT_REST || (scope == SPLIT_ROWS && !sw.no_dma_rows);
     const bool want = sw.x6_scope == 2 || (sw.x6_scope == 1 && in_default && cfg.dtype == MI_DTYPE_F32);
-    if (!want || !conv_x6_supported(pc->tile)) return MI_OK;
-    const bool t192 = pc->M % 192 == 0 && pc->Mpad == pc->M;
+    if (!want || !(scope == SPLIT_REST ? conv_x6_image_tile(pc->tile) : conv_x6_supported(pc->tile))) return MI_OK;
+    const bool t192 = pc->M % 192 == 0 && pc->Mpad == pc->M && !(scope == SPLIT_REST && pc->tile == 128);
     MI_TRY(weights.alloc(&pc->wx, (size_t)6 * pc->Kpad * pc->Mpad));
     MI_TRY(launch_pack_split(pc->wt, pc->Kpad, pc->Mpad, t192 ? 96 : pc->tile, pc->wx, nullptr));
     MI_HIP(hipStreamSynchronize(nullptr));
@@ -248,7 +251,7 @@
         MI_TRY(wt.get(p + ".4.weight", 2 * C, &g2w));
         MI_TRY(wt.get(p + ".4.bias", 2 * C, &g2b));
         MI_TRY(wt.get(p + ".6.scale", C, &ls));
-        MI_TRY(pack_conv(w0, b0, h, 3 * C, false, &l.conv3));
+        MI_TRY(pack_conv(w0, b0, h, 3 * C, false, &l.conv3, 0, comp == 8 && C >= 192 ? SPLIT_REST : SPLIT_OPT_IN));
         const int dil = 1 << d;
         MI_TRY(make_ktab(Gather{C, 1, 3, 1, dil, 0, dil, chan_stride, D2}, l.conv3.Kpad, &l.ktab3));
         const int hp = round_up(h, 16);
@@ -329,6 +332,7 @@
         d.epi = MI_EPI_BIAS_STATS; d.y = hidden; d.y_bstride = (int64_t)hp * P; d.y_cstride = P; d.stats = stats;
         if (dconv_tap_dma) {
             d.ntaps = 3; d.tap_k2 = 3; d.tap_pad1 = 0; d.tap_pad2 = 1 << dlayer; d.tap_dil2 = 1 << dlayer;
+            if (d.wx && !d.half) d.dma_dil = 1;
         }
         MI_TRY(conv(d, st));
         MI_TRY(launch_finalize_stats(stats, rows, cnt_row * h, 1e-5f, 0, st1, nullptr, st));
diff --git a/demucs_amd/csrc/gemm_conv.h b/demucs_amd/csrc/gemm_conv.h
--- a/demucs_amd/csrc/gemm_conv.h
+++ b/demucs_amd/csrc/gemm_conv.h
@@ -80,7 +80,7 @@
     int32_t dma_rows;
     int32_t dma_rows_pad;
     int32_t dma_time;
-    int32_t dma_time_pad;
+    int32_t dma_dil;
 } mi_conv_desc;
 
 #ifdef __cplusplus
diff --git a/demucs_amd/csrc/gemm_conv.hip b/demucs_amd/csrc/gemm_conv.hip
--- a/demucs_amd/csrc/gemm_conv.hip
+++ b/demucs_amd/csrc/gemm_conv.hip
@@ -216,6 +216,7 @@
         case MI_ROUTE_TAP_X6: return launch_conv_tap_x6(d, r.tile, image_tile, st);
         case MI_ROUTE_ROWS_X6: return launch_conv_rows_x6(d, r.tile, image_tile, st);
         case MI_ROUTE_TIME_X6: return launch_conv_time_x6(d, r.tile, image_tile, st);
+        case MI_ROUTE_DIL_X6: return launch_conv_dil_x6(d, r.tile, st);
         case MI_ROUTE_X6: return launch_conv_x6(d, r.tile, image_tile, r.plain, st);
         case MI_ROUTE_DMATAP:
             return d.epi == MI_EPI_GLU ? launch_dmatap<MI_EPI_GLU>(d, r.tile, st) : launch_dmatap<MI_EPI_BIAS_STATS>(d, r.tile, st);
diff --git a/demucs_amd/csrc/gemm_x6.hip b/demucs_amd/csrc/gemm_x6.hip
--- a/demucs_amd/csrc/gemm_x6.hip
+++ b/demucs_amd/csrc/gemm_x6.hip
@@ -27,12 +27,14 @@
     return MI_OK;
 }
 
-template <int WM, int WN, int TM, int TN, int EPI, int LFLAGS, bool PLAIN, bool HALF_IMG, int NT>
+template <int WM, int WN, int TM, int TN, int EPI, int LFLAGS, bool PLAIN, bool HALF_IMG, int NT, int DIL = 1>
 __device__ __forceinline__ void conv_x6_body(const mi_conv_desc &d, const int N, const int MT, const int Gm) {
     constexpr int BM = WM * TM * 32;
     constexpr bool RAW = PLAIN || NT != 0;
     constexpr bool ROWS = NT == kRowTaps;
-    static_assert(NT <= 0 || (!PLAIN && EPI == MI_EPI_GLU), "tap loader: GLU rewrite convs");
+    static_assert(NT <= 0 || (!PLAIN && ((EPI == MI_EPI_GLU && DIL == 1) || (EPI == MI_EPI_BIAS_STATS && NT == 3 && (DIL == 1 || DIL == 2)))),
+                  "tap loader: GLU rewrite convs (dilation 1), k = 3 convs with row statistics (dilation 1 or 2)");
+    static_assert(DIL == 1 || NT == 3, "DIL: the k = 3 tap loader");
     static_assert(!ROWS || (!PLAIN && (EPI == MI_EPI_LINEAR || EPI == MI_EPI_CONVTR || EPI == MI_EPI_GLU)),
                   "row-tap loader: encoder / transposed convs, 1 x 1 + GLU rewrites");
     static_assert(NT != kTimeTr || (!PLAIN && EPI == MI_EPI_CONVTR), "time-axis two-tap loader: transposed convs");
@@ -75,7 +77,7 @@
     const float *bp = lc.valid ? xcol + (size_t)(8 * bh) * w.P : d.sink + MI_SINK_FLOATS;
     const size_t b_row = lc.valid ? (size_t)w.P : 0, b_step = lc.valid ? (size_t)BK * w.P : 0;
     float breg[8];
-    BLoader<NT> L(d, w, N, w.P);
+    BLoader<NT, DIL> L(d, w, N, w.P);
     constexpr bool OWN_STAGE = NT == kTimeEnc;
 #define MI_BRAW_DMA(kt, rs) L.issue(d, (kt), braw + (rs) * (BK * BN) + (OWN_STAGE ? 0 : 4 * w.wave) * BN)
 #define MI_BRAW_FIX(kt, rs) L.fix(d, (kt), braw + (rs) * (BK * BN) + (OWN_STAGE ? 0 : 4 * w.wave) * BN)
@@ -224,6 +226,21 @@
     conv_x6_body<WM, WN, TM, TN, MI_EPI_LINEAR, MI_FLAG_GELU, false, HALF_IMG, kTimeEnc>(d, N, MT, Gm);
 }
 
+template <int WM, int WN, int TM, int TN, int DIL>
+__global__ __launch_bounds__(256, 2) void conv_dil_x6_kernel(const mi_conv_desc d, const int N, const int MT, const int Gm) {
+    conv_x6_body<WM, WN, TM, TN, MI_EPI_BIAS_STATS, 0, false, false, 3, DIL>(d, N, MT, Gm);
+}
+
+template <int WM, int WN, int TM, int TN, int LFLAGS, bool HALF_IMG>
+__global__ __launch_bounds__(256, 2) void conv_chan_x6_kernel(const mi_conv_desc d, const int N, const int MT, const int Gm) {
+    conv_x6_body<WM, WN, TM, TN, MI_EPI_LINEAR, LFLAGS, true, HALF_IMG, 0>(d, N, MT, Gm);
+}
+
+template <int WM, int WN, int TM, int TN, bool HALF_IMG>
+__global__ __launch_bounds__(256, 2) void conv_glu_x6_kernel(const mi_conv_desc d, const int N, const int MT, const int Gm) {
+    conv_x6_body<WM, WN, TM, TN, MI_EPI_GLU, 0, true, HALF_IMG, 0>(d, N, MT, Gm);
+}
+
 template <int WM, int WN, int TM, int TN, int EPI, int LFLAGS, bool PLAIN, bool HALF_IMG = false, int NTAPS = 0>
 static int launch_cfg_x6(const mi_conv_desc &d, hipStream_t st) {
     constexpr int BM = WM * TM * 32;
@@ -234,6 +251,8 @@
     else if constexpr (NTAPS == kRowTaps) MI_LAUNCH_TILES((conv_rows_x6_kernel<WM, WN, TM, TN, EPI, LFLAGS, HALF_IMG>), d, g, Gm, st);
     else if constexpr (NTAPS == kTimeTr) MI_LAUNCH_TILES((conv_time_tr_x6_kernel<WM, WN, TM, TN, HALF_IMG>), d, g, Gm, st);
     else if constexpr (NTAPS == kTimeEnc) MI_LAUNCH_TILES((conv_time_enc_x6_kernel<WM, WN, TM, TN, HALF_IMG>), d, g, Gm, st);
+    else if constexpr (conv_x6_own_symbol(EPI, LFLAGS, PLAIN) == 1) MI_LAUNCH_TILES((conv_chan_x6_kernel<WM, WN, TM, TN, LFLAGS, HALF_IMG>), d, g, Gm, st);
+    else if constexpr (conv_x6_own_symbol(EPI, LFLAGS, PLAIN) == 2) MI_LAUNCH_TILES((conv_glu_x6_kernel<WM, WN, TM, TN, HALF_IMG>), d, g, Gm, st);
     else MI_LAUNCH_TILES((conv_gemm_x6_kernel<WM, WN, TM, TN, EPI, LFLAGS, PLAIN, HALF_IMG>), d, g, Gm, st);
     return MI_OK;
 }
@@ -292,6 +311,22 @@
     return launch_tile_x6<MI_EPI_LINEAR, MI_FLAG_GELU, false, kTimeEnc>(d, tile, image_tile, st);
 }
 
+int launch_conv_dil_x6(const mi_conv_desc &d, int tile, hipStream_t st) {
+    MI_REQUIRE(d.wx && ((uintptr_t)d.wx & 15) == 0, "conv dil x6: split weight image missing or misaligned");
+    const int dil = d.tap_dil2 ? d.tap_dil2 : 1;
+    MI_REQUIRE(d.epi == MI_EPI_BIAS_STATS && d.ntaps == 3 && (tile == 32 || tile == 64) && (dil == 1 || dil == 2),
+               "conv dil x6: BIAS_STATS layer with 3 taps, dilation 1 or 2, on a 32- or 64-row tile (epi %d, tile %d, ntaps %d, dilation %d)", d.epi,
+               tile, d.ntaps, dil);
+    ConvGeom g;
+    MI_TRY(conv_geom(d, "conv dil x6", tile, tile, g));
+    const int Gm = pick_m_groups(g.MT, (size_t)d.Kpad * d.Mpad * 6);
+    if (tile == 64 && dil == 2) MI_LAUNCH_TILES((conv_dil_x6_kernel<1, 4, 2, 1, 2>), d, g, Gm, st);
+    else if (tile == 64) MI_LAUNCH_TILES((conv_dil_x6_kernel<1, 4, 2, 1, 1>), d, g, Gm, st);
+    else if (dil == 2) MI_LAUNCH_TILES((conv_dil_x6_kernel<1, 4, 1, 1, 2>), d, g, Gm, st);
+    else MI_LAUNCH_TILES((conv_dil_x6_kernel<1, 4, 1, 1, 1>), d, g, Gm, st);
+    return MI_OK;
+}
+
 int launch_conv_x6(const mi_conv_desc &d, int tile, int image_tile, bool plain, hipStream_t st) {
     MI_REQUIRE(d.wx && ((uintptr_t)d.wx & 15) == 0, "conv x6: split weight image missing or misaligned");
     return dispatch_epilogue(d, [&](auto epi, auto lflags) {
diff --git a/demucs_amd/csrc/kernels.h b/demucs_amd/csrc/kernels.h
--- a/demucs_amd/csrc/kernels.h
+++ b/demucs_amd/csrc/kernels.h
@@ -139,6 +139,10 @@
 };
 const Switches &switches();
 constexpr bool conv_x6_supported(int tile) { return tile == 128 || tile == 96 || tile == 64; }
+constexpr bool conv_x6_image_tile(int tile) { return conv_x6_supported(tile) || tile == 32; }
+constexpr int conv_x6_own_symbol(int epi, int lflags, bool plain) {
+    return !plain ? 0 : epi == MI_EPI_LINEAR && (lflags == 0 || lflags == MI_FLAG_RES) ? 1 : epi == MI_EPI_GLU ? 2 : 0;
+}
 constexpr int kRowTaps = -1;
 constexpr int kTimeTr = -2;
 constexpr int kTimeEnc = -3;
@@ -147,12 +151,13 @@
     if (ntaps == kTimeTr) return epi == MI_EPI_CONVTR;
     if (ntaps == kTimeEnc) return epi == MI_EPI_LINEAR && lflags == MI_FLAG_GELU;
     if (ntaps == kRowTaps) return (epi == MI_EPI_LINEAR && lflags == MI_FLAG_GELU) || epi == MI_EPI_CONVTR || epi == MI_EPI_GLU;
-    return plain && epi == MI_EPI_LINEAR && lflags == MI_FLAG_LN;
+    return plain && ((epi == MI_EPI_LINEAR && lflags == MI_FLAG_LN) || epi == MI_EPI_GLU);
 }
 int launch_conv_x6(const mi_conv_desc &d, int tile, int image_tile, bool plain, hipStream_t st);
 int launch_conv_tap_x6(const mi_conv_desc &d, int tile, int image_tile, hipStream_t st);
 int launch_conv_rows_x6(const mi_conv_desc &d, int tile, int image_tile, hipStream_t st);
 int launch_conv_time_x6(const mi_conv_desc &d, int tile, int image_tile, hipStream_t st);
+int launch_conv_dil_x6(const mi_conv_desc &d, int tile, hipStream_t st);
 int launch_pack_split(const float *wt, int Kpad, int Mpad, int tile_m, void *wx, hipStream_t st);
 
 int launch_conv_half(const mi_conv_desc &d, const ConvRoute &r, hipStream_t st);
diff --git a/demucs_amd/csrc/model.hip b/demucs_amd/csrc/model.hip
--- a/demucs_amd/csrc/model.hip
+++ b/demucs_amd/csrc/model.hip
@@ -64,7 +64,7 @@
         MI_TRY(pack_conv(w, b, C, Cin * 8, false, &e.conv, 0, i > 0 ? SPLIT_ROWS : SPLIT_OPT_IN));
         if (i) MI_TRY(pack_enc_tap(w, Cin, &e.conv));
         MI_TRY(make_ktab(Gather{Cin, 8, 1, 1, 1, 2, 0, (int64_t)kFr[i] * T, T}, e.conv.Kpad, &e.ktab_conv));
-        MI_TRY(pack_conv(rw, rb, 2 * C, C, true, &e.rewrite, 0, i >= 2 ? SPLIT_ROWS : SPLIT_OPT_IN));
+        MI_TRY(pack_conv(rw, rb, 2 * C, C, true, &e.rewrite, 0, i >= 2 ? SPLIT_ROWS : SPLIT_REST));
         MI_TRY(make_ktab(Gather{C, 1, 1, 1, 1, 0, 0, (int64_t)kFr[i + 1] * T, T}, e.rewrite.Kpad, &e.ktab_rw));
         MI_TRY(load_dconv(wt, p, C, (int64_t)kFr[i + 1] * T, T, true, &e.dconv));
 
@@ -78,7 +78,7 @@
         MI_TRY(pack_conv(w, b, C, Cint * 8, false, &te.conv, 0, i > 0 ? SPLIT_TIME : SPLIT_OPT_IN));
         if (i) MI_TRY(pack_enc_tap(w, Cint, &te.conv));
         MI_TRY(make_ktab(Gather{Cint, 1, 8, 1, 1, 0, 2, (int64_t)Lp[i], Lp[i]}, te.conv.Kpad, &te.ktab_conv));
-        MI_TRY(pack_conv(rw, rb, 2 * C, C, true, &te.rewrite, 0, i >= 2 ? SPLIT_ROWS : SPLIT_OPT_IN));
+        MI_TRY(pack_conv(rw, rb, 2 * C, C, true, &te.rewrite, 0, i >= 2 ? SPLIT_ROWS : SPLIT_REST));
         MI_TRY(make_ktab(Gather{C, 1, 1, 1, 1, 0, 0, (int64_t)Lp[i + 1], Lp[i + 1]}, te.rewrite.Kpad, &te.ktab_rw));
         MI_TRY(load_dconv(wt, pt, C, (int64_t)Lp[i + 1], Lp[i + 1], false, &te.dconv));
     }
@@ -127,7 +127,7 @@
             const float *w, *b;
             MI_TRY(wt.get(std::string(names[i]) + ".weight", (int64_t)M * K, &w));
             MI_TRY(wt.get(std::string(names[i]) + ".bias", M, &b));
-            MI_TRY(pack_conv(w, b, M, K, false, &chan[i]));
+            MI_TRY(pack_conv(w, b, M, K, false, &chan[i], 0, SPLIT_REST));
             MI_TRY(make_ktab(Gather{K, 1, 1, 1, 1, 0, 0, (int64_t)P, P}, chan[i].Kpad, &chan_ktab[i]));
         }
         for (int br = 0; br < 2; ++br) {
diff --git a/include/demucs_amd.h b/include/demucs_amd.h
--- a/include/demucs_amd.h
+++ b/include/demucs_amd.h
@@ -437,7 +437,8 @@
     MI_ROUTE_ROWS_X6 = 8,
     MI_ROUTE_HALF_IMG = 9,
     MI_ROUTE_HALF_IMG256 = 10,
-    MI_ROUTE_TIME_X6 = 11
+    MI_ROUTE_TIME_X6 = 11,
+    MI_ROUTE_DIL_X6 = 12
 };
 
 int mi_debug_last_conv_route(void);
```

Result: no change. 2439 (median of 6 runs) (+0.8%).
